# facebookresearch/momentum

Measured on NVIDIA H100. Metric: GN iterations/sec (batched 72-joint IK), higher is better.
Workload: dtype f32

## Files before the change

momentum_b200/csrc/ik_capi.cu:

```cuda
#include "../../include/momentum_b200.h"

#include <cuda_runtime.h>
#include <nvtx3/nvToolsExt.h>

#include <algorithm>
#include <cfloat>
#include <cmath>
#include <cstdio>
#include <cstdlib>
#include <cstring>
#include <memory>
#include <string>
#include <vector>

#include "ik_chol_sched.h"
#include "ik_fused.cuh"
#include "ik_jtj_tc.cuh"
#include "ik_kernels.cuh"
#include "ik_plan.h"

using namespace mb2;

namespace {

thread_local std::string g_lastError;

int fail(int code, const std::string& msg) {
  g_lastError = msg;
  return code;
}
#define MB2_CUDA(expr)                                                                                  \
  do {                                                                                                  \
    cudaError_t _e = (expr);                                                                            \
    if (_e != cudaSuccess) return fail(MB2_ERR_CUDA, std::string(#expr) + ": " + cudaGetErrorString(_e)); \
  } while (0)
#define MB2_CHECK(cond, msg)                                   \
  do {                                                         \
    if (!(cond)) return fail(MB2_ERR_INVALID_ARGUMENT, (msg)); \
  } while (0)

template <class T>
struct DeviceBuffer {
  T* p{nullptr};
  size_t n{0};
  ~DeviceBuffer() { release(); }
  void release() {
    if (p) cudaFree(p);
    p = nullptr;
    n = 0;
  }
  cudaError_t resize(size_t count) {
    if (count <= n && p) return cudaSuccess;
    release();
    if (count == 0) return cudaSuccess;
    cudaError_t e = cudaMalloc(&p, count * sizeof(T));
    if (e == cudaSuccess) n = count;
    return e;
  }
  cudaError_t upload(const std::vector<T>& v, cudaStream_t s) {
    cudaError_t e = resize(std::max<size_t>(v.size(), 1));
    if (e != cudaSuccess || v.empty()) return e;
    return cudaMemcpyAsync(p, v.data(), v.size() * sizeof(T), cudaMemcpyHostToDevice, s);
  }
};

int roundUp(int v, int m) { return (v + m - 1) / m * m; }

int usableDevices();

struct DeviceGuard {
  int prev{-1};
  bool switched{false};
  cudaError_t err{cudaSuccess};
  explicit DeviceGuard(int device) {
    err = cudaGetDevice(&prev);
    if (err == cudaSuccess && prev != device) { err = cudaSetDevice(device); switched = err == cudaSuccess; }
  }
  ~DeviceGuard() { if (switched) cudaSetDevice(prev); }
  DeviceGuard(const DeviceGuard&) = delete;
  DeviceGuard& operator=(const DeviceGuard&) = delete;
};
#define MB2_DEVICE_GUARD(device)                                                                                      \
  if (usableDevices() <= 0) return fail(MB2_ERR_CUDA, "no usable sm_90 CUDA device: momentum_b200 has no CPU fallback"); \
  DeviceGuard _guard(device);                                                                                         \
  MB2_CUDA(_guard.err)

struct NvtxRange {
  explicit NvtxRange(const char* name) { nvtxRangePushA(name); }
  ~NvtxRange() { nvtxRangePop(); }
};

}

struct mb2_character {
  int device{0};
  HostCharacter host;
  DeviceBuffer<int32_t> parent, ptOuter, ptInner, levelStart, levelJoints;
  DeviceBuffer<float> offset, prerot, ptVals, ptOffsets;
  uint64_t limitsVersion{0};
};

struct DeviceSchedule {
  CholSchedule host;
  CholSchedDev dev{};
  DeviceBuffer<int32_t> blob;
  GramPlan gram;
  DeviceBuffer<int32_t> gBlob;
  int32_t gBlobInts{0}, gOffsets[8]{};
  DeviceBuffer<int32_t> fBlob;
  FusedBlobLayout fLayout{};
  FusedConfig fConfig{};
};

struct mb2_solver_function {
  const mb2_character* ch{nullptr};
  int B{0};
  cudaStream_t stream{nullptr};
  HostFunction host;
  bool planDirty{true};
  int planMode{0};
  bool planSchedDense{false};
  bool planAlignRows{false};
  uint64_t planLimitsVersion{~0ull};
  Plan plan;
  int ldJ{32};
  DeviceBuffer<EfDesc> dEfs;
  DeviceBuffer<UnitDesc> dUnits;
  DeviceBuffer<CellDesc> dCells;
  DeviceBuffer<ContribDesc> dContribs;
  DeviceBuffer<float> dLimitData;
  DeviceBuffer<int32_t> dEnabledList, dIdentity, dDeviceCols;
  DeviceBuffer<float> dTargets, dWeights, dJ, dTheta, dState, dH, dTargetStage;
  DeviceBuffer<double> dErrors;
  std::unique_ptr<DeviceSchedule> sched;
  FunctionTables tables() const;
};

struct PhaseEvent {
  cudaEvent_t start, stop;
  int phase;
};

struct mb2_solver {
  mb2_solver_function* fn{nullptr};
  mb2_gauss_newton_options opt{};
  DeviceBuffer<float> dH, dDelta, dThetaOrig, dTheta0, dScale, dGradDotDelta, dThetaStage, dGrad, dTiles, dRadius, dRSaved;
  DeviceBuffer<double> dLastErrors, dTrialErrors, dHistory;
  DeviceBuffer<int32_t> dActive, dIterations, dStatus, dSearching, dActiveCount, dWorkCounter, dQrChunks;
  DeviceBuffer<unsigned long long> dPhaseCycles;
  bool lastFused{false}, lastGramChol{false};
  int lastFusedGroups{0};
  cudaEvent_t fusedStart{nullptr}, fusedStop{nullptr};
  double fusedMs{0};
  int* hActiveCount{nullptr};
  char* hResults{nullptr};
  size_t hResultsBytes{0};
  bool resultsStaged{false};
  uint64_t totalIterations{0}, kernelLaunches{0};
  bool profiling{false};
  bool inKernelProfile{false};
  std::vector<PhaseEvent> events;
  double phaseMs[4]{0, 0, 0, 0};
  uint64_t phaseLaunches[4]{0, 0, 0, 0};
  size_t historyStride{0};
  ~mb2_solver() {
    if (hActiveCount) cudaFreeHost(hActiveCount);
    if (hResults) cudaFreeHost(hResults);
    if (fusedStart) cudaEventDestroy(fusedStart);
    if (fusedStop) cudaEventDestroy(fusedStop);
    for (auto& e : events) { cudaEventDestroy(e.start); cudaEventDestroy(e.stop); }
  }
};

FunctionTables mb2_solver_function::tables() const {
  FunctionTables T{};
  const HostCharacter& h = ch->host;
  T.numJoints = h.numJoints;
  T.numParams = h.numParams;
  T.parent = ch->parent.p;
  T.offset = ch->offset.p;
  T.prerot = ch->prerot.p;
  T.ptOuter = ch->ptOuter.p;
  T.ptInner = ch->ptInner.p;
  T.ptVals = ch->ptVals.p;
  T.ptOffsets = ch->ptOffsets.p;
  T.numLevels = int(h.levelStart.size()) - 1;
  T.levelStart = ch->levelStart.p;
  T.levelJoints = ch->levelJoints.p;
  T.numEf = int(plan.efs.size());
  T.numUnits = int(plan.units.size());
  T.numCells = int(plan.cells.size());
  T.efs = dEfs.p;
  T.units = dUnits.p;
  T.cells = dCells.p;
  T.contribs = dContribs.p;
  T.limitData = dLimitData.p;
  T.targetStride = host.targetStride;
  T.recStride = plan.recStride;
  T.numRows = plan.numRows;
  T.ldJ = ldJ;
  T.numCols = plan.numCols;
  T.weightsPerInstance = host.weightsPerInstance ? 1 : 0;
  T.numWeights = host.numWeights;
  T.ptNnz = int(h.ptInner.size());
  T.numContribs = int(plan.contribs.size());
  T.numLimitData = int(plan.limitData.size());
  const bool strips = planMode == 2 && planAlignRows && sched;
  T.stripMode = strips ? 1 : 0;
  T.residOff = strips ? sched->gram.residOff : 0;
  T.jacobianStride = strips ? size_t(sched->gram.stride) : size_t(plan.numCols + 1) * ldJ;
  return T;
}

namespace {

bool g_deviceChecked = false;
int g_usableDevices = 0;
}
namespace {
int usableDevices() {
  if (!g_deviceChecked) {
    int n = 0;
    if (cudaGetDeviceCount(&n) != cudaSuccess) { n = 0; cudaGetLastError(); }
    int ok = 0;
    for (int d = 0; d < n; ++d) {
      int major = 0;
      if (cudaDeviceGetAttribute(&major, cudaDevAttrComputeCapabilityMajor, d) == cudaSuccess && major == 9) ++ok;
    }
    g_usableDevices = ok;
    g_deviceChecked = true;
  }
  return g_usableDevices;
}

int requireDevice(int device) {
  if (usableDevices() <= 0) return fail(MB2_ERR_CUDA, "no usable sm_90 CUDA device: momentum_b200 has no CPU fallback");
  MB2_CUDA(cudaSetDevice(device));
  MB2_CUDA(initKernelAttributes());
  return MB2_OK;
}

int ensureTargets(mb2_solver_function* f) {
  const size_t need = size_t(f->B) * std::max(f->host.targetStride, 1);
  if (f->dTargets.n < need) {
    DeviceBuffer<float> old;
    std::swap(old.p, f->dTargets.p);
    std::swap(old.n, f->dTargets.n);
    MB2_CUDA(f->dTargets.resize(need));
    MB2_CUDA(cudaMemsetAsync(f->dTargets.p, 0, need * sizeof(float), f->stream));
    MB2_CUDA(cudaStreamSynchronize(f->stream));
    (void)old;
  }
  return MB2_OK;
}

int uploadWeights(mb2_solver_function* f) {
  if (!f->host.weightsPerInstance) {
    std::vector<float> w = f->host.weights;
    if (w.empty()) w.push_back(0.f);
    MB2_CUDA(f->dWeights.upload(w, f->stream));
  }
  return MB2_OK;
}

int buildFusedBlob(mb2_solver_function* f, DeviceSchedule& ds, const std::vector<int32_t>& gramBlob, const std::vector<int32_t>& schedBlob, cudaStream_t s) {
  std::vector<int32_t> blob;
  auto add = [&](const void* data, size_t bytes) {
    const int32_t off = int32_t(blob.size());
    const size_t words = (bytes + 3) / 4;
    blob.resize(blob.size() + words, 0);
    if (bytes) std::memcpy(blob.data() + off, data, bytes);
    while (blob.size() % 4) blob.push_back(0);
    return off;
  };
  const HostCharacter& h = f->ch->host;
  const Plan& p = f->plan;
  FusedBlobLayout& L = ds.fLayout;
  L.parent = add(h.parent.data(), h.parent.size() * 4);
  L.offset = add(h.offset.data(), h.offset.size() * 4);
  L.prerot = add(h.prerot.data(), h.prerot.size() * 4);
  L.ptOuter = add(h.ptOuter.data(), h.ptOuter.size() * 4);
  L.ptInner = add(h.ptInner.data(), h.ptInner.size() * 4);
  L.ptVals = add(h.ptVals.data(), h.ptVals.size() * 4);
  L.ptOffsets = add(h.ptOffsets.data(), h.ptOffsets.size() * 4);
  L.levelStart = add(h.levelStart.data(), h.levelStart.size() * 4);
  L.levelJoints = add(h.levelJoints.data(), h.levelJoints.size() * 4);
  L.efs = add(p.efs.data(), p.efs.size() * sizeof(EfDesc));
  L.units = add(p.units.data(), p.units.size() * sizeof(UnitDesc));
  L.cells = add(p.cells.data(), p.cells.size() * sizeof(CellDesc));
  L.contribs = add(p.contribs.data(), p.contribs.size() * sizeof(ContribDesc));
  L.limitData = add(p.limitData.data(), p.limitData.size() * 4);
  L.cols = add(p.deviceCols.data(), p.deviceCols.size() * 4);
  L.gram = add(gramBlob.data(), gramBlob.size() * 4);
  L.sched = add(schedBlob.data(), schedBlob.size() * 4);
  if (blob.empty()) blob.push_back(0);
  while (blob.size() % 4) blob.push_back(0);
  L.words = int32_t(blob.size());
  MB2_CUDA(ds.fBlob.upload(blob, s));
  return MB2_OK;
}

int ensurePlan(mb2_solver_function* f, int mode, bool schedDense = false, bool alignRows = false) {
  bool allEnabled = true;
  for (uint8_t e : f->host.enabled) allEnabled = allEnabled && e;
  if (allEnabled && mode == 1) mode = 0;
  if (mode != 2) alignRows = false;
  if (!f->planDirty && f->planLimitsVersion == f->ch->limitsVersion && f->planMode == mode && (mode != 2 || (f->planSchedDense == schedDense && f->planAlignRows == alignRows)))
    return MB2_OK;
  MB2_DEVICE_GUARD(f->ch->device);
  cudaStream_t s = f->stream;
  f->sched.reset();
  std::unique_ptr<DeviceSchedule> ds;
  std::string err;
  if (mode == 2) {
    ds = std::make_unique<DeviceSchedule>();
    err = planSolverPath(f->ch->host, f->host.efs, f->host.enabled, schedDense, alignRows, f->plan, ds->host, ds->gram);
  } else {
    err = buildPlan(f->ch->host, f->host.efs, f->host.enabled, mode != 0, f->plan);
  }
  if (!err.empty()) return fail(MB2_ERR_INVALID_ARGUMENT, err);
  if (ds) {
    std::vector<int32_t> sblob, gblob;
    CholSchedDev hostView;
    makeScheduleBlob(ds->host, sblob, hostView);
    MB2_CUDA(ds->blob.upload(sblob, s));
    ds->dev = rebaseSchedule(hostView, ds->blob.p);
    if (alignRows) {
      makeGramBlob(ds->gram, ds->host, gblob, ds->gOffsets);
      ds->gBlobInts = int32_t(gblob.size());
      MB2_CUDA(ds->gBlob.upload(gblob, s));
      const int rc = buildFusedBlob(f, *ds, gblob, sblob, s);
      if (rc != MB2_OK) return rc;
    }
    f->sched = std::move(ds);
  }
  f->planMode = mode;
  f->planSchedDense = schedDense;
  f->planAlignRows = alignRows;
  MB2_CUDA(f->dEfs.upload(f->plan.efs, s));
  MB2_CUDA(f->dUnits.upload(f->plan.units, s));
  MB2_CUDA(f->dCells.upload(f->plan.cells, s));
  MB2_CUDA(f->dContribs.upload(f->plan.contribs, s));
  MB2_CUDA(f->dLimitData.upload(f->plan.limitData, s));
  MB2_CUDA(f->dEnabledList.upload(f->plan.enabledList, s));
  MB2_CUDA(f->dDeviceCols.upload(f->plan.deviceCols, s));
  std::vector<int32_t> ident(f->ch->host.numParams);
  for (size_t i = 0; i < ident.size(); ++i) ident[i] = int32_t(i);
  MB2_CUDA(f->dIdentity.upload(ident, s));
  f->ldJ = std::max(32, roundUp(f->plan.numRows, 32));
  const bool stripLayout = mode == 2 && alignRows;
  const size_t jElems = stripLayout ? size_t(f->B) * size_t(f->sched->gram.stride) : size_t(f->B) * (f->plan.numCols + 1) * f->ldJ;
  MB2_CUDA(f->dJ.resize(jElems));
  MB2_CUDA(cudaMemsetAsync(f->dJ.p, 0, jElems * sizeof(float), s));
  MB2_CUDA(f->dErrors.resize(f->B));
  MB2_CUDA(f->dTheta.resize(size_t(f->B) * f->ch->host.numParams));
  int rc = ensureTargets(f);
  if (rc != MB2_OK) return rc;
  rc = uploadWeights(f);
  if (rc != MB2_OK) return rc;
  if (stripLayout) {
    int dev = 0, optin = 0;
    MB2_CUDA(cudaGetDevice(&dev));
    MB2_CUDA(cudaDeviceGetAttribute(&optin, cudaDevAttrMaxSharedMemoryPerBlockOptin, dev));
    f->sched->fConfig = fusedConfigure(f->tables(), f->sched->fLayout, f->sched->dev, f->sched->gram.stride, int(f->sched->gram.tileOrder.size()) / kGramWarps, optin);
  }
  MB2_CUDA(cudaStreamSynchronize(s));
  f->planDirty = false;
  f->planLimitsVersion = f->ch->limitsVersion;
  return MB2_OK;
}

SweepArgs sweepArgs(mb2_solver_function* f, const float* theta, const int32_t* active) {
  SweepArgs a{};
  a.T = f->tables();
  a.batch = f->B;
  a.theta = theta;
  a.ldTheta = f->ch->host.numParams;
  a.targets = f->dTargets.p;
  a.cweights = f->dWeights.p;
  a.jacobian = f->dJ.p;
  a.errors = f->dErrors.p;
  a.active = active;
  a.stateOut = nullptr;
  return a;
}

int addBlock(mb2_solver_function* f, const std::string& buildError, const HostErrorFunction& ef, int32_t* outIndex) {
  if (!buildError.empty()) return fail(MB2_ERR_INVALID_ARGUMENT, buildError);
  const std::string err = f->host.add(ef, outIndex);
  if (!err.empty()) return fail(MB2_ERR_UNSUPPORTED, err);
  f->planDirty = true;
  return MB2_OK;
}

void bitsToEnabled(const uint64_t* bits, int n, std::vector<uint8_t>& out) {
  out.assign(n, 0);
  for (int i = 0; i < n; ++i) out[i] = (bits[i >> 6] >> (i & 63)) & 1ull ? 1 : 0;
}

void recordPhaseStart(mb2_solver* s, int phase, cudaStream_t st) {
  s->kernelLaunches++;
  if (!s->profiling) return;
  PhaseEvent e;
  cudaEventCreate(&e.start);
  cudaEventCreate(&e.stop);
  e.phase = phase;
  cudaEventRecord(e.start, st);
  s->events.push_back(e);
}
void recordPhaseStop(mb2_solver* s, cudaStream_t st) {
  if (!s->profiling) return;
  cudaEventRecord(s->events.back().stop, st);
}

__global__ void initSolveStateKernel(int batch, int32_t* active, int32_t* iterations, int32_t* status, double* lastErrors, double* errors) {
  const int b = blockIdx.x * blockDim.x + threadIdx.x;
  if (b >= batch) return;
  active[b] = 1;
  iterations[b] = 0;
  status[b] = 0;
  lastErrors[b] = DBL_MAX;
  errors[b] = DBL_MAX;
}
__global__ void initLineSearchKernel(int batch, const int32_t* active, int32_t* searching, float* scale) {
  const int b = blockIdx.x * blockDim.x + threadIdx.x;
  if (b >= batch) return;
  searching[b] = active[b];
  scale[b] = 1.f;
}
__global__ void finalizeKernel(int batch, int n, float* theta, const float* theta0, int32_t* status) {
  const int b = blockIdx.x;
  __shared__ int bad;
  if (threadIdx.x == 0) bad = 0;
  __syncthreads();
  for (int i = threadIdx.x; i < n; i += blockDim.x)
    if (!isfinite(theta[size_t(b) * n + i])) bad = 1;
  __syncthreads();
  if (bad) {
    for (int i = threadIdx.x; i < n; i += blockDim.x) theta[size_t(b) * n + i] = theta0[size_t(b) * n + i];
    if (threadIdx.x == 0) status[b] = MB2_INSTANCE_NON_FINITE;
  }
}

int resolveJtjMode(const mb2_solver_function* f, int requested, int ns) {
  if (requested == MB2_JTJ_FP32_SIMT) return MB2_JTJ_FP32_SIMT;
  const bool ok = jtjTensorSupported(ns, f->plan.numCols, f->ldJ);
  if (requested == MB2_JTJ_AUTO) return ok ? MB2_JTJ_TF32X3 : MB2_JTJ_FP32_SIMT;
  return ok ? requested : -1;
}

int runJtJ(mb2_solver_function* f, int mode, int ns, float* H, int ldH, size_t hStride, const int32_t* active, cudaStream_t st, float* g = nullptr, int ldG = 0) {
  JtJArgs a{};
  a.batch = f->B;
  a.jacobian = f->dJ.p;
  a.numCols = f->plan.numCols;
  a.ldJ = f->ldJ;
  a.kRows = roundUp(std::max(f->plan.numRows, 1), 4);
  a.ns = ns;
  a.H = H;
  a.ldH = ldH;
  a.hStride = hStride;
  a.active = active;
  a.g = g;
  a.ldG = ldG;
  if (mode == MB2_JTJ_FP32_SIMT) { MB2_CUDA(launchJtJSimt(a, st)); }
  else { MB2_CUDA(launchJtJTensor(a, mode == MB2_JTJ_TF32X3 ? 3 : 1, st)); }
  return MB2_OK;
}

}

extern "C" {

const char* mb2_last_error(void) { return g_lastError.c_str(); }
int mb2_device_count(void) { return usableDevices(); }

void mb2_default_gauss_newton_options(mb2_gauss_newton_options* o) {
  if (!o) return;
  std::memset(o, 0, sizeof(*o));
  o->min_iterations = 1;
  o->max_iterations = 2;
  o->threshold = 1.0f;
  o->verbose = 0;
  o->regularization = 0.05f;
  o->do_line_search = 0;
  o->use_block_jtj = 0;
  o->target_rows_per_chunk = ~0ull;
  o->subset_line_search = 0;
  o->jtj_mode = MB2_JTJ_AUTO;
  o->store_error_history = 0;
  o->cholesky_mode = MB2_CHOLESKY_AUTO;
  o->fused_mode = MB2_FUSED_AUTO;
  o->linear_solver = MB2_LINEAR_SOLVER_CHOLESKY;
  o->trust_region_radius = 1.0f;
}

int mb2_character_create(int device, int32_t J, const int32_t* parents, const float* offsets, const float* prerot, int32_t n,
                         const int32_t* outer, const int32_t* inner, const float* vals, const float* ptoffsets, mb2_character** out) {
  MB2_CHECK(out != nullptr, "null argument");
  auto c = std::make_unique<mb2_character>();
  HostCharacter& h = c->host;
  const std::string err = makeCharacter(J, parents, offsets, prerot, n, outer, inner, vals, ptoffsets, h);
  if (!err.empty()) return fail(MB2_ERR_INVALID_ARGUMENT, err);
  MB2_DEVICE_GUARD(device);
  int rc = requireDevice(device);
  if (rc != MB2_OK) return rc;
  c->device = device;
  MB2_CUDA(c->parent.upload(h.parent, nullptr));
  MB2_CUDA(c->offset.upload(h.offset, nullptr));
  MB2_CUDA(c->prerot.upload(h.prerot, nullptr));
  MB2_CUDA(c->ptOuter.upload(h.ptOuter, nullptr));
  MB2_CUDA(c->ptInner.upload(h.ptInner, nullptr));
  MB2_CUDA(c->ptVals.upload(h.ptVals, nullptr));
  MB2_CUDA(c->ptOffsets.upload(h.ptOffsets, nullptr));
  MB2_CUDA(c->levelStart.upload(h.levelStart, nullptr));
  MB2_CUDA(c->levelJoints.upload(h.levelJoints, nullptr));
  MB2_CUDA(cudaStreamSynchronize(nullptr));
  *out = c.release();
  return MB2_OK;
}

int mb2_character_set_parameter_limits(mb2_character* c, int32_t count, const mb2_parameter_limit* limits) {
  MB2_CHECK(c != nullptr, "invalid limits");
  const std::string err = setParameterLimits(c->host, count, limits);
  if (!err.empty()) return fail(MB2_ERR_INVALID_ARGUMENT, err);
  c->limitsVersion++;
  return MB2_OK;
}

void mb2_character_destroy(mb2_character* c) { delete c; }

int mb2_solver_function_create(const mb2_character* c, int32_t batch, mb2_solver_function** out) {
  MB2_CHECK(c != nullptr && out != nullptr, "null argument");
  MB2_CHECK(batch > 0, "batch must be positive");
  MB2_DEVICE_GUARD(c->device);
  int rc = requireDevice(c->device);
  if (rc != MB2_OK) return rc;
  auto f = std::make_unique<mb2_solver_function>();
  f->ch = c;
  f->B = batch;
  f->host.enabled.assign(c->host.numParams, 1);
  MB2_CUDA(cudaStreamCreateWithFlags(&f->stream, cudaStreamNonBlocking));
  *out = f.release();
  return MB2_OK;
}

void mb2_solver_function_destroy(mb2_solver_function* f) {
  if (!f) return;
  if (f->stream) cudaStreamDestroy(f->stream);
  delete f;
}

int mb2_character_clone(const mb2_character* c, int device, mb2_character** out) {
  MB2_CHECK(c != nullptr && out != nullptr, "null argument");
  const HostCharacter& h = c->host;
  mb2_character* copy = nullptr;
  int rc = mb2_character_create(device, h.numJoints, h.parent.data(), h.offset.data(), h.prerot.data(), h.numParams, h.ptOuter.data(), h.ptInner.data(), h.ptVals.data(),
                                h.ptOffsets.data(), &copy);
  if (rc != MB2_OK) return rc;
  copy->host.limits = h.limits;
  copy->limitsVersion = 1;
  *out = copy;
  return MB2_OK;
}
int mb2_solver_function_clone(const mb2_solver_function* f, const mb2_character* c, int32_t batch, mb2_solver_function** out) {
  MB2_CHECK(f != nullptr && c != nullptr && out != nullptr, "null argument");
  MB2_CHECK(c->host.numJoints == f->ch->host.numJoints && c->host.numParams == f->ch->host.numParams, "clone target character has a different shape");
  MB2_CHECK(!f->host.weightsPerInstance, "a function with per-instance constraint weights cannot be cloned (set them on the clone)");
  mb2_solver_function* g = nullptr;
  int rc = mb2_solver_function_create(c, batch, &g);
  if (rc != MB2_OK) return rc;
  g->host = f->host;
  g->planDirty = true;
  *out = g;
  return MB2_OK;
}
int mb2_character_device(const mb2_character* c) { return c ? c->device : -1; }
const mb2_character* mb2_solver_function_character(const mb2_solver_function* f) { return f ? f->ch : nullptr; }
int32_t mb2_solver_function_num_error_functions(const mb2_solver_function* f) { return f ? int32_t(f->host.efs.size()) : 0; }
int32_t mb2_solver_function_target_size(const mb2_solver_function* f, int32_t index) {
  return (f && index >= 0 && index < int32_t(f->host.efs.size())) ? f->host.efs[index].targetSize : -1;
}

int32_t mb2_solver_function_num_parameters(const mb2_solver_function* f) { return f ? f->ch->host.numParams : 0; }
int32_t mb2_solver_function_batch(const mb2_solver_function* f) { return f ? f->B : 0; }
int32_t mb2_solver_function_actual_parameters(const mb2_solver_function* f) { return f ? f->host.actualParameters() : 0; }
int32_t mb2_solver_function_jacobian_rows(const mb2_solver_function* f) { return f ? f->host.jacobianRows(f->ch->host) : 0; }
int32_t mb2_solver_function_jacobian_stride(const mb2_solver_function* f) { return f ? f->host.jacobianStride(f->ch->host) : 0; }

int mb2_add_position_error_function(mb2_solver_function* f, float weight, float alpha, float c, int32_t nc, const int32_t* parents,
                                    const float* offsets, const float* weights, int32_t* outIndex) {
  MB2_CHECK(f != nullptr, "null solver function");
  HostErrorFunction ef;
  return addBlock(f, positionErrorFunction(f->ch->host, weight, alpha, c, nc, parents, offsets, weights, ef), ef, outIndex);
}

int mb2_add_position_error_function_instanced(mb2_solver_function* f, float weight, float alpha, float c, int32_t nc, const int32_t* parents, const float* weights,
                                              int32_t* outIndex) {
  MB2_CHECK(f != nullptr, "null solver function");
  HostErrorFunction ef;
  return addBlock(f, instancedPositionErrorFunction(f->ch->host, weight, alpha, c, nc, parents, weights, ef), ef, outIndex);
}

int mb2_add_plane_error_function(mb2_solver_function* f, float weight, float alpha, float c, int32_t above, int32_t nc, const int32_t* parents,
                                 const float* offsets, const float* weights, int32_t* outIndex) {
  MB2_CHECK(f != nullptr, "null solver function");
  HostErrorFunction ef;
  return addBlock(f, planeErrorFunction(f->ch->host, weight, alpha, c, above, nc, parents, offsets, weights, ef), ef, outIndex);
}

int mb2_add_model_parameters_error_function(mb2_solver_function* f, float weight, const float* targetWeights, int32_t* outIndex) {
  MB2_CHECK(f != nullptr, "null solver function");
  HostErrorFunction ef;
  return addBlock(f, modelParametersErrorFunction(f->ch->host, weight, targetWeights, ef), ef, outIndex);
}

int mb2_add_orientation_error_function(mb2_solver_function* f, float weight, float alpha, float c, int32_t rotDiff, int32_t nc,
                                       const int32_t* parents, const float* offsets, const float* weights, int32_t* outIndex) {
  MB2_CHECK(f != nullptr, "null solver function");
  HostErrorFunction ef;
  return addBlock(f, orientationErrorFunction(f->ch->host, weight, alpha, c, rotDiff, nc, parents, offsets, weights, ef), ef, outIndex);
}

int mb2_add_state_error_function(mb2_solver_function* f, float weight, int32_t rotationErrorType, float posWgt, float rotWgt,
                                 const float* posW, const float* rotW, int32_t* outIndex) {
  MB2_CHECK(f != nullptr, "null solver function");
  HostErrorFunction ef;
  return addBlock(f, stateErrorFunction(f->ch->host, weight, rotationErrorType, posWgt, rotWgt, posW, rotW, ef), ef, outIndex);
}

int mb2_add_limit_error_function(mb2_solver_function* f, float weight, float alpha, float c, int32_t* outIndex) {
  MB2_CHECK(f != nullptr, "null solver function");
  HostErrorFunction ef;
  return addBlock(f, limitErrorFunction(weight, alpha, c, ef), ef, outIndex);
}

int mb2_set_error_function_weight(mb2_solver_function* f, int32_t index, float weight) {
  MB2_CHECK(f != nullptr && index >= 0 && index < int(f->host.efs.size()), "error function index out of range");
  f->host.efs[index].weight = weight;
  f->planDirty = true;
  return MB2_OK;
}

static int setTargetsImpl(mb2_solver_function* f, int32_t index, const float* targets, bool deviceSrc, cudaStream_t st) {
  MB2_CHECK(f != nullptr && index >= 0 && index < int(f->host.efs.size()) && targets, "invalid targets");
  const HostErrorFunction& ef = f->host.efs[index];
  if (ef.targetSize == 0 && ef.kind != 4) return MB2_OK;
  MB2_CHECK(ef.targetSize > 0, "this error function has no per-instance targets");
  MB2_DEVICE_GUARD(f->ch->device);
  int rc = ensureTargets(f);
  if (rc != MB2_OK) return rc;
  float* dst = f->dTargets.p + ef.targetOff;
  const float* packed = targets;
  if (!deviceSrc) {
    MB2_CUDA(f->dTargetStage.resize(size_t(f->B) * ef.targetSize));
    MB2_CUDA(cudaMemcpyAsync(f->dTargetStage.p, targets, size_t(f->B) * ef.targetSize * sizeof(float), cudaMemcpyHostToDevice, st));
    packed = f->dTargetStage.p;
  }
  MB2_CUDA(launchScatterTargets(packed, dst, ef.targetSize, f->host.targetStride, f->B, st));
  if (ef.kind == 1 || ef.kind == 2) MB2_CUDA(launchNormalizeQuats(dst, 0, f->host.targetStride, ef.numConstraints(), f->B, st));
  return MB2_OK;
}
int mb2_set_targets(mb2_solver_function* f, int32_t index, const float* targets) {
  if (!f) return fail(MB2_ERR_INVALID_ARGUMENT, "null solver function");
  int rc = setTargetsImpl(f, index, targets, false, f->stream);
  if (rc != MB2_OK) return rc;
  MB2_CUDA(cudaStreamSynchronize(f->stream));
  return MB2_OK;
}
int mb2_set_targets_device(mb2_solver_function* f, int32_t index, const float* targets, void* stream) {
  if (!f) return fail(MB2_ERR_INVALID_ARGUMENT, "null solver function");
  return setTargetsImpl(f, index, targets, true, stream ? (cudaStream_t)stream : f->stream);
}

int mb2_set_constraint_weights(mb2_solver_function* f, int32_t index, const float* weights, int32_t perInstance) {
  MB2_CHECK(f != nullptr && index >= 0 && index < int(f->host.efs.size()) && weights, "invalid constraint weights");
  HostErrorFunction& ef = f->host.efs[index];
  MB2_CHECK(ef.kind <= 2 || ef.kind == 5, "constraint weights apply to Position/Orientation/Plane error functions");
  MB2_DEVICE_GUARD(f->ch->device);
  const int nc = ef.numConstraints();
  if (!perInstance) {
    MB2_CHECK(!f->host.weightsPerInstance, "solver function already uses per-instance constraint weights");
    ef.weights.assign(weights, weights + nc);
    std::copy(weights, weights + nc, f->host.weights.begin() + ef.weightOff);
    return uploadWeights(f);
  }
  if (!f->host.weightsPerInstance) {
    std::vector<float> all(size_t(f->B) * f->host.numWeights);
    for (int b = 0; b < f->B; ++b) std::copy(f->host.weights.begin(), f->host.weights.end(), all.begin() + size_t(b) * f->host.numWeights);
    f->dWeights.release();
    MB2_CUDA(f->dWeights.upload(all, f->stream));
    f->host.weightsPerInstance = true;
  }
  MB2_CUDA(cudaMemcpy2DAsync(f->dWeights.p + ef.weightOff, size_t(f->host.numWeights) * sizeof(float), weights, size_t(nc) * sizeof(float),
                             size_t(nc) * sizeof(float), f->B, cudaMemcpyHostToDevice, f->stream));
  MB2_CUDA(cudaStreamSynchronize(f->stream));
  return MB2_OK;
}

int mb2_set_constraint_weights_device(mb2_solver_function* f, int32_t index, const float* weights_device, void* stream) {
  MB2_CHECK(f != nullptr && index >= 0 && index < int(f->host.efs.size()) && weights_device, "invalid constraint weights");
  HostErrorFunction& ef = f->host.efs[index];
  MB2_CHECK(ef.kind <= 2 || ef.kind == 5, "constraint weights apply to Position/Orientation/Plane error functions");
  MB2_DEVICE_GUARD(f->ch->device);
  const int nc = ef.numConstraints();
  if (!f->host.weightsPerInstance) {
    std::vector<float> all(size_t(f->B) * f->host.numWeights);
    for (int b = 0; b < f->B; ++b) std::copy(f->host.weights.begin(), f->host.weights.end(), all.begin() + size_t(b) * f->host.numWeights);
    f->dWeights.release();
    MB2_CUDA(f->dWeights.upload(all, f->stream));
    MB2_CUDA(cudaStreamSynchronize(f->stream));
    f->host.weightsPerInstance = true;
    f->planDirty = true;
  }
  cudaStream_t st = stream ? (cudaStream_t)stream : f->stream;
  if (nc > 0)
    MB2_CUDA(cudaMemcpy2DAsync(f->dWeights.p + ef.weightOff, size_t(f->host.numWeights) * sizeof(float), weights_device, size_t(nc) * sizeof(float), size_t(nc) * sizeof(float), f->B,
                               cudaMemcpyDeviceToDevice, st));
  return MB2_OK;
}

int mb2_solver_function_set_enabled_parameters(mb2_solver_function* f, const uint64_t* bits) {
  MB2_CHECK(f != nullptr && bits != nullptr, "null argument");
  bitsToEnabled(bits, f->ch->host.numParams, f->host.enabled);
  f->planDirty = true;
  return MB2_OK;
}

int mb2_solver_function_get_error(mb2_solver_function* f, const float* params, double* errors) {
  MB2_CHECK(f != nullptr && params && errors, "null argument");
  MB2_DEVICE_GUARD(f->ch->device);
  int rc = ensurePlan(f, f->planMode, f->planSchedDense, f->planAlignRows);
  if (rc != MB2_OK) return rc;
  const size_t n = f->ch->host.numParams;
  MB2_CUDA(cudaMemcpyAsync(f->dTheta.p, params, size_t(f->B) * n * sizeof(float), cudaMemcpyHostToDevice, f->stream));
  MB2_CUDA(launchSweep(sweepArgs(f, f->dTheta.p, nullptr), false, f->stream));
  MB2_CUDA(cudaMemcpyAsync(errors, f->dErrors.p, size_t(f->B) * sizeof(double), cudaMemcpyDeviceToHost, f->stream));
  MB2_CUDA(cudaStreamSynchronize(f->stream));
  return MB2_OK;
}

int mb2_solver_function_get_jacobian(mb2_solver_function* f, const float* params, float* jac, float* residual, double* errors, int32_t* actualRows) {
  MB2_CHECK(f != nullptr && params, "null argument");
  MB2_DEVICE_GUARD(f->ch->device);
  int rc = ensurePlan(f, 0);
  if (rc != MB2_OK) return rc;
  const size_t n = f->ch->host.numParams;
  const int rows = mb2_solver_function_jacobian_rows(f);
  MB2_CUDA(cudaMemcpyAsync(f->dTheta.p, params, size_t(f->B) * n * sizeof(float), cudaMemcpyHostToDevice, f->stream));
  MB2_CUDA(launchSweep(sweepArgs(f, f->dTheta.p, nullptr), true, f->stream));
  for (int b = 0; b < f->B && rows > 0; ++b) {
    const float* Jb = f->dJ.p + size_t(b) * (n + 1) * f->ldJ;
    if (jac)
      MB2_CUDA(cudaMemcpy2DAsync(jac + size_t(b) * n * rows, size_t(rows) * sizeof(float), Jb, size_t(f->ldJ) * sizeof(float), size_t(rows) * sizeof(float), n,
                                 cudaMemcpyDeviceToHost, f->stream));
    if (residual)
      MB2_CUDA(cudaMemcpyAsync(residual + size_t(b) * rows, Jb + n * f->ldJ, size_t(rows) * sizeof(float), cudaMemcpyDeviceToHost, f->stream));
  }
  if (errors) MB2_CUDA(cudaMemcpyAsync(errors, f->dErrors.p, size_t(f->B) * sizeof(double), cudaMemcpyDeviceToHost, f->stream));
  MB2_CUDA(cudaStreamSynchronize(f->stream));
  if (actualRows) *actualRows = rows;
  return MB2_OK;
}

int mb2_solver_function_get_jacobian_device(mb2_solver_function* f, const float* params_device, const float** jacobian_device, int32_t* ld, void* stream) {
  MB2_CHECK(f != nullptr && params_device && jacobian_device, "null argument");
  MB2_DEVICE_GUARD(f->ch->device);
  int rc = ensurePlan(f, 0);
  if (rc != MB2_OK) return rc;
  cudaStream_t st = stream ? (cudaStream_t)stream : f->stream;
  MB2_CUDA(launchSweep(sweepArgs(f, params_device, nullptr), true, st));
  *jacobian_device = f->dJ.p;
  if (ld) *ld = f->ldJ;
  return MB2_OK;
}

int mb2_solver_function_get_jtjr(mb2_solver_function* f, const float* params, int32_t jtjMode, float* jtj, float* jtr, double* errors) {
  MB2_CHECK(f != nullptr && params, "null argument");
  MB2_DEVICE_GUARD(f->ch->device);
  int rc = ensurePlan(f, 0);
  if (rc != MB2_OK) return rc;
  const size_t n = f->ch->host.numParams;
  const int ap = f->plan.actualParameters;
  MB2_CHECK(ap > 0, "no enabled parameters");
  const int mode = resolveJtjMode(f, jtjMode, ap);
  if (mode < 0) return fail(MB2_ERR_UNSUPPORTED, "tensor-core JtJ does not support this shape");
  const int ldH = roundUp(ap + 1, 16);
  const size_t hElems = size_t(f->B) * (ap + 1) * ldH;
  MB2_CUDA(f->dH.resize(hElems));
  MB2_CUDA(cudaMemcpyAsync(f->dTheta.p, params, size_t(f->B) * n * sizeof(float), cudaMemcpyHostToDevice, f->stream));
  MB2_CUDA(launchSweep(sweepArgs(f, f->dTheta.p, nullptr), true, f->stream));
  MB2_CUDA(cudaMemsetAsync(f->dH.p, 0, hElems * sizeof(float), f->stream));
  rc = runJtJ(f, mode, ap, f->dH.p, ldH, size_t(ap + 1) * ldH, nullptr, f->stream);
  if (rc != MB2_OK) return rc;
  std::vector<float> h(hElems);
  MB2_CUDA(cudaMemcpyAsync(h.data(), f->dH.p, hElems * sizeof(float), cudaMemcpyDeviceToHost, f->stream));
  if (errors) MB2_CUDA(cudaMemcpyAsync(errors, f->dErrors.p, size_t(f->B) * sizeof(double), cudaMemcpyDeviceToHost, f->stream));
  MB2_CUDA(cudaStreamSynchronize(f->stream));
  for (int b = 0; b < f->B; ++b) {
    const float* Hb = h.data() + size_t(b) * (ap + 1) * ldH;
    for (int j = 0; j < ap; ++j) {
      if (jtj) for (int i = j; i < ap; ++i) jtj[(size_t(b) * ap + i) * ap + j] = Hb[size_t(j) * ldH + i];
      if (jtr) jtr[size_t(b) * ap + j] = Hb[size_t(j) * ldH + ap];
    }
  }
  return MB2_OK;
}

int mb2_solver_function_get_skeleton_state(mb2_solver_function* f, const float* params, float* state) {
  MB2_CHECK(f != nullptr && params && state, "null argument");
  MB2_DEVICE_GUARD(f->ch->device);
  int rc = ensurePlan(f, f->planMode, f->planSchedDense, f->planAlignRows);
  if (rc != MB2_OK) return rc;
  const size_t n = f->ch->host.numParams;
  const size_t sz = size_t(f->B) * f->ch->host.numJoints * 8;
  MB2_CUDA(f->dState.resize(sz));
  MB2_CUDA(cudaMemcpyAsync(f->dTheta.p, params, size_t(f->B) * n * sizeof(float), cudaMemcpyHostToDevice, f->stream));
  SweepArgs a = sweepArgs(f, f->dTheta.p, nullptr);
  a.stateOut = f->dState.p;
  MB2_CUDA(launchSweep(a, false, f->stream));
  MB2_CUDA(cudaMemcpyAsync(state, f->dState.p, sz * sizeof(float), cudaMemcpyDeviceToHost, f->stream));
  MB2_CUDA(cudaStreamSynchronize(f->stream));
  return MB2_OK;
}

int mb2_solver_create(mb2_solver_function* f, const mb2_gauss_newton_options* opt, mb2_solver** out) {
  MB2_CHECK(f != nullptr && out != nullptr, "null argument");
  auto s = std::make_unique<mb2_solver>();
  s->fn = f;
  if (opt) s->opt = *opt; else mb2_default_gauss_newton_options(&s->opt);
  MB2_DEVICE_GUARD(f->ch->device);
  MB2_CUDA(cudaMallocHost(&s->hActiveCount, sizeof(int)));
  *out = s.release();
  return MB2_OK;
}
void mb2_solver_destroy(mb2_solver* s) { delete s; }
int mb2_solver_set_options(mb2_solver* s, const mb2_gauss_newton_options* opt) {
  MB2_CHECK(s != nullptr && opt != nullptr, "null argument");
  s->opt = *opt;
  return MB2_OK;
}
int mb2_solver_set_enabled_parameters(mb2_solver* s, const uint64_t* bits) {
  MB2_CHECK(s != nullptr, "null solver");
  return mb2_solver_function_set_enabled_parameters(s->fn, bits);
}
int mb2_solver_set_profiling(mb2_solver* s, int32_t enabled) {
  MB2_CHECK(s != nullptr, "null solver");
  s->profiling = enabled != 0;
  s->inKernelProfile = enabled >= 2;
  return MB2_OK;
}

int mb2_solver_solve_device(mb2_solver* s, float* theta, void* cudaStream) {
  MB2_CHECK(s != nullptr && theta != nullptr, "null argument");
  mb2_solver_function* f = s->fn;
  MB2_DEVICE_GUARD(f->ch->device);
  NvtxRange nvtxSolve("mb2::SolverT::solve");
  const mb2_gauss_newton_options& o = s->opt;
  int cholMode = resolveCholeskyMode(o.cholesky_mode, f->host.enabled);
  const bool useTr = o.linear_solver == MB2_LINEAR_SOLVER_TRUST_REGION_QR;
  const bool useQr = o.linear_solver == MB2_LINEAR_SOLVER_QR || useTr;
  if (useTr && !(o.trust_region_radius > 0.f)) return fail(MB2_ERR_INVALID_ARGUMENT, "trust_region_radius must be positive");
  if (useQr) {
    if (o.jtj_mode == MB2_JTJ_SPARSE_TILES || o.cholesky_mode >= 2 || o.fused_mode >= MB2_FUSED_PERSISTENT)
      return fail(MB2_ERR_UNSUPPORTED, "the QR step works on the dense Jacobian: it excludes the tile-sparse Gram, the tile Cholesky and the fused kernels");
    cholMode = 1;
  }
  bool useGram = cholMode >= 2 && (o.jtj_mode == MB2_JTJ_AUTO || o.jtj_mode == MB2_JTJ_SPARSE_TILES);
  if (o.jtj_mode == MB2_JTJ_SPARSE_TILES && cholMode < 2) return fail(MB2_ERR_UNSUPPORTED, "MB2_JTJ_SPARSE_TILES needs the tile-scheduled Cholesky");
  int rc = ensurePlan(f, cholMode >= 2 ? 2 : 1, cholMode == 2, useGram);
  if (rc != MB2_OK) return rc;
  bool useSchedule = cholMode >= 2;
  if (useSchedule && choleskyScheduledSmemBytes(f->plan.numCols, f->sched->host.nPad, f->sched->host.numTiles, f->sched->dev.blobInts) > size_t(200 * 1024)) {
    if (o.cholesky_mode >= 2) return fail(MB2_ERR_UNSUPPORTED, "tile schedule does not fit in shared memory for this system");
    useSchedule = false;
    useGram = false;
    rc = ensurePlan(f, 1);
    if (rc != MB2_OK) return rc;
  }
  cudaStream_t st = cudaStream ? (cudaStream_t)cudaStream : f->stream;
  const int B = f->B, n = f->ch->host.numParams;
  const int ns = f->plan.numCols;
  const int maxIt = int(std::min<uint64_t>(o.max_iterations, 1u << 30));
  const int minIt = int(std::min<uint64_t>(o.min_iterations, 1u << 30));
  MB2_CHECK(ns > 0, "no enabled parameters");
  if (useGram && gramTilesSmemBytes(size_t(f->sched->gram.stride), f->sched->gBlobInts) > size_t(200 * 1024)) {
    if (o.jtj_mode == MB2_JTJ_SPARSE_TILES) return fail(MB2_ERR_UNSUPPORTED, "Jacobian strips do not fit in shared memory for this system");
    useGram = false;
    rc = ensurePlan(f, 2, cholMode == 2, false);
    if (rc != MB2_OK) return rc;
  }
  s->lastFused = false;
  {
    const bool eligible = useGram && useSchedule && o.do_line_search == 0 && f->sched->fConfig.groups >= 1 && f->sched->fBlob.p != nullptr;
    if (o.fused_mode == MB2_FUSED_PERSISTENT && !eligible)
      return fail(MB2_ERR_UNSUPPORTED, "the fused kernel needs the tile-sparse Gram + tile-scheduled Cholesky path, no line search, and a plan that fits in shared memory");
    int smCount = 0;
    if (eligible && o.fused_mode == MB2_FUSED_AUTO) {
      int dev0 = 0;
      MB2_CUDA(cudaGetDevice(&dev0));
      MB2_CUDA(cudaDeviceGetAttribute(&smCount, cudaDevAttrMultiProcessorCount, dev0));
    }
    const bool oneWave = eligible && o.fused_mode == MB2_FUSED_AUTO && B <= f->sched->fConfig.groups * smCount;
    if ((o.fused_mode == MB2_FUSED_PERSISTENT || oneWave) && eligible) {
      const DeviceSchedule& ds = *f->sched;
      MB2_CUDA(s->dIterations.resize(B));
      MB2_CUDA(s->dStatus.resize(B));
      MB2_CUDA(s->dWorkCounter.resize(1));
      MB2_CUDA(cudaMemsetAsync(s->dWorkCounter.p, 0, sizeof(int32_t), st));
      if (o.store_error_history) {
        MB2_CUDA(s->dHistory.resize(size_t(B) * std::max(maxIt, 1)));
        MB2_CUDA(cudaMemsetAsync(s->dHistory.p, 0, size_t(B) * std::max(maxIt, 1) * sizeof(double), st));
        s->historyStride = size_t(std::max(maxIt, 1));
      }
      FusedArgs fa{};
      fa.batch = B;
      fa.T = f->tables();
      fa.blob = ds.fBlob.p;
      fa.L = ds.fLayout;
      fa.S = ds.dev;
      fa.schedGlobal = ds.dev.blob;
      for (int k = 0; k < 8; ++k) fa.gramOff[k] = ds.gOffsets[k];
      fa.numStrips = ds.gram.numStrips;
      fa.stripStride = ds.gram.stride;
      fa.residOff = ds.gram.residOff;
      fa.numOrder = int32_t(ds.gram.tileOrder.size());
      fa.regularization = o.regularization;
      fa.threshold = o.threshold;
      fa.minIterations = minIt;
      fa.maxIterations = maxIt;
      fa.theta = theta;
      fa.ldTheta = n;
      fa.targets = f->dTargets.p;
      fa.cweights = f->dWeights.p;
      fa.errors = f->dErrors.p;
      fa.iterations = s->dIterations.p;
      fa.status = s->dStatus.p;
      fa.history = o.store_error_history ? s->dHistory.p : nullptr;
      fa.workCounter = s->dWorkCounter.p;
      fa.phaseCycles = nullptr;
      if (s->profiling) {
        MB2_CUDA(s->dPhaseCycles.resize(16));
        MB2_CUDA(cudaMemsetAsync(s->dPhaseCycles.p, 0, 16 * sizeof(unsigned long long), st));
        fa.phaseCycles = s->inKernelProfile ? s->dPhaseCycles.p : nullptr;
        if (!s->fusedStart) { MB2_CUDA(cudaEventCreate(&s->fusedStart)); MB2_CUDA(cudaEventCreate(&s->fusedStop)); }
        MB2_CUDA(cudaEventRecord(s->fusedStart, st));
      }
      int dev = 0, sms = 0;
      MB2_CUDA(cudaGetDevice(&dev));
      MB2_CUDA(cudaDeviceGetAttribute(&sms, cudaDevAttrMultiProcessorCount, dev));
      {
        NvtxRange nvtxIt("mb2::fusedSolveKernel (GaussNewtonSolverT::doIteration x maxIterations)");
        MB2_CUDA(launchFusedSolve(fa, ds.fConfig, sms, s->inKernelProfile, st));
      }
      if (s->profiling) MB2_CUDA(cudaEventRecord(s->fusedStop, st));
      for (auto& e : s->events) { cudaEventDestroy(e.start); cudaEventDestroy(e.stop); }
      s->events.clear();
      s->kernelLaunches = 1;
      s->lastFused = true;
      s->lastFusedGroups = ds.fConfig.groups;
      return MB2_OK;
    }
  }
  bool useGramChol = false;
  if (useGram && useSchedule) {
    const DeviceSchedule& ds = *f->sched;
    const int rounds = std::max(int(ds.gram.tileOrder.size()) / kGramWarps, 1);
    const bool fits = gramCholeskySmemBytes(size_t(ds.gram.stride), ds.gBlobInts, ns, ds.host.nPad, ds.host.numTiles, ds.dev.blobInts) <= size_t(200 * 1024) && rounds <= kGramCholMaxRounds;
    if (o.fused_mode == MB2_FUSED_GRAM_CHOLESKY && !fits) return fail(MB2_ERR_UNSUPPORTED, "Gram + Cholesky fusion: strips / tiles of this plan do not fit in shared memory, or too many tiles per warp");
    useGramChol = fits && (o.fused_mode == MB2_FUSED_AUTO || o.fused_mode == MB2_FUSED_GRAM_CHOLESKY);
  } else if (o.fused_mode == MB2_FUSED_GRAM_CHOLESKY) {
    return fail(MB2_ERR_UNSUPPORTED, "Gram + Cholesky fusion needs the tile-sparse Gram + tile-scheduled Cholesky path");
  }
  s->lastGramChol = useGramChol;
  if (useGramChol && s->profiling) {
    MB2_CUDA(s->dPhaseCycles.resize(16));
    MB2_CUDA(cudaMemsetAsync(s->dPhaseCycles.p, 0, 16 * sizeof(unsigned long long), st));
  }
  const int mode = useGram ? MB2_JTJ_SPARSE_TILES : resolveJtjMode(f, o.jtj_mode == MB2_JTJ_SPARSE_TILES ? MB2_JTJ_AUTO : o.jtj_mode, ns);
  if (mode < 0) return fail(MB2_ERR_UNSUPPORTED, "tensor-core JtJ does not support this shape");
  const int ldH = roundUp(ns + 1, 16);
  const size_t hStride = size_t(ns + 1) * ldH;
  if (!useGram && !useQr) MB2_CUDA(s->dH.resize(size_t(B) * hStride));
  int qrMaxRows = 0, qrChunks = 0;
  if (useQr) {
    qrMaxRows = qrMaxChunkRows(ns, size_t(200 * 1024));
    if (qrMaxRows < 8) return fail(MB2_ERR_UNSUPPORTED, "the QR step keeps R in shared memory: too many enabled parameters for this kernel");
    if (useTr) {
      qrMaxRows = std::min(qrMaxRows, std::max(8, ns / 2));
      if (trQrSmemFloats(ns, n, f->ch->host.numJoints, qrMaxRows) * sizeof(float) > size_t(220 * 1024))
        return fail(MB2_ERR_UNSUPPORTED, "the trust-region QR kernel keeps R and the damping rows in shared memory: too many enabled parameters / joints");
    }
    std::vector<int32_t> starts{0};
    int r0 = 0, widest = 0;
    for (const auto& ef : f->host.efs) {
      if (!(ef.weight > 0.f)) continue;
      const int size = jacobianBlockSize(f->ch->host, ef);
      for (int done = 0; done < size; done += qrMaxRows) { const int p = std::min(qrMaxRows, size - done); starts.push_back(r0 + done + p); widest = std::max(widest, p); }
      r0 += size;
    }
    qrChunks = int(starts.size()) - 1;
    qrMaxRows = std::max(widest, 1);
    MB2_CUDA(s->dQrChunks.upload(starts, st));
    if (useTr) {
      MB2_CUDA(s->dRadius.upload(std::vector<float>(size_t(B), o.trust_region_radius), st));
      MB2_CUDA(s->dRSaved.resize(size_t(B) * ((size_t(ns) * (ns + 1) / 2 + 3) & ~size_t(3))));
    }
  }
  float* Hbuf = s->dH.p;
  const size_t tilesStride = useGram ? size_t(f->sched->host.numTiles) * 256 + f->sched->host.nPad : 0;
  if (useGram && !(o.fused_mode == MB2_FUSED_AUTO || o.fused_mode == MB2_FUSED_GRAM_CHOLESKY)) MB2_CUDA(s->dTiles.resize(size_t(B) * tilesStride));
  const int ldG = cholGradientLd(ns);
  MB2_CUDA(s->dGrad.resize(size_t(B) * ldG));
  MB2_CUDA(s->dDelta.resize(size_t(B) * ns));
  MB2_CUDA(s->dTheta0.resize(size_t(B) * n));
  MB2_CUDA(s->dLastErrors.resize(B));
  MB2_CUDA(s->dActive.resize(B));
  MB2_CUDA(s->dIterations.resize(B));
  MB2_CUDA(s->dStatus.resize(B));
  MB2_CUDA(s->dActiveCount.resize(1));
  const bool lineSearch = o.do_line_search != 0 && !useTr;
  if (lineSearch) {
    MB2_CUDA(s->dThetaOrig.resize(size_t(B) * n));
    MB2_CUDA(s->dTrialErrors.resize(B));
    MB2_CUDA(s->dScale.resize(B));
    MB2_CUDA(s->dSearching.resize(B));
    MB2_CUDA(s->dGradDotDelta.resize(B));
  }
  if (o.store_error_history) {
    MB2_CUDA(s->dHistory.resize(size_t(B) * std::max(maxIt, 1)));
    MB2_CUDA(cudaMemsetAsync(s->dHistory.p, 0, size_t(B) * std::max(maxIt, 1) * sizeof(double), st));
    s->historyStride = size_t(std::max(maxIt, 1));
  }
  for (auto& e : s->events) { cudaEventDestroy(e.start); cudaEventDestroy(e.stop); }
  s->events.clear();
  s->kernelLaunches = 0;

  initSolveStateKernel<<<(B + 127) / 128, 128, 0, st>>>(B, s->dActive.p, s->dIterations.p, s->dStatus.p, s->dLastErrors.p, f->dErrors.p);
  MB2_CUDA(cudaGetLastError());
  MB2_CUDA(cudaMemcpyAsync(s->dTheta0.p, theta, size_t(B) * n * sizeof(float), cudaMemcpyDeviceToDevice, st));

  static const bool cholProfile = getenv("MB2_CHOL_PROFILE") != nullptr;
  constexpr int kPollEvery = 4;
  for (int it = 0; it < maxIt; ++it) {
    MB2_CUDA(cudaMemsetAsync(s->dActiveCount.p, 0, sizeof(int), st));
    recordPhaseStart(s, 0, st);
    MB2_CUDA(launchSweep(sweepArgs(f, theta, s->dActive.p), true, st));
    recordPhaseStop(s, st);
    GramArgs g{};
    if (!useGramChol && !useQr) recordPhaseStart(s, 1, st);
    if (useQr) {
    } else if (useGram) {
      const DeviceSchedule& ds = *f->sched;
      g.batch = B;
      g.strips = f->dJ.p;
      g.stripStride = size_t(ds.gram.stride);
      g.residOff = ds.gram.residOff;
      g.active = s->dActive.p;
      g.numStrips = ds.gram.numStrips;
      g.numTiles = ds.host.numTiles;
      g.numTileCols = ds.host.numTileCols;
      g.nPad = ds.host.nPad;
      g.numOrder = int32_t(ds.gram.tileOrder.size());
      g.blob = ds.gBlob.p;
      g.blobInts = ds.gBlobInts;
      g.offTileOrder = ds.gOffsets[0]; g.offTilePairStart = ds.gOffsets[1]; g.offPairA = ds.gOffsets[2]; g.offPairB = ds.gOffsets[3];
      g.offColStripStart = ds.gOffsets[4]; g.offColStrip = ds.gOffsets[5]; g.offStripRow = ds.gOffsets[6]; g.offTileInfo = ds.gOffsets[7];
      g.regularization = o.regularization;
      g.out = s->dTiles.p;
      g.outStride = tilesStride;
      if (!useGramChol) {
        if (s->dTiles.n < size_t(B) * tilesStride) MB2_CUDA(s->dTiles.resize(size_t(B) * tilesStride));
        g.out = s->dTiles.p;
        MB2_CUDA(launchGramTiles(g, st));
      }
    } else {
      rc = runJtJ(f, mode, ns, Hbuf, ldH, hStride, s->dActive.p, st, s->dGrad.p, ldG);
      if (rc != MB2_OK) return rc;
    }
    if (!useGramChol && !useQr) recordPhaseStop(s, st);
    CholArgs c{};
    c.batch = B;
    c.H = Hbuf;
    c.ns = ns;
    c.ldH = ldH;
    c.hStride = hStride;
    c.regularization = o.regularization;
    c.cols = f->dDeviceCols.p;
    c.theta = theta;
    c.ldTheta = n;
    c.delta = s->dDelta.p;
    c.applyUpdate = lineSearch ? 0 : 1;
    c.errors = f->dErrors.p;
    c.lastErrors = s->dLastErrors.p;
    c.active = s->dActive.p;
    c.iterations = s->dIterations.p;
    c.status = s->dStatus.p;
    c.history = o.store_error_history ? s->dHistory.p : nullptr;
    c.iteration = it;
    c.minIterations = minIt;
    c.maxIterations = maxIt;
    c.threshold = o.threshold;
    c.activeCount = s->dActiveCount.p;
    c.bookkeeping = lineSearch ? 0 : 1;
    c.gradDotDelta = lineSearch ? s->dGradDotDelta.p : nullptr;
    c.g = s->dGrad.p;
    c.ldG = ldG;
    c.tilesIn = useGram ? s->dTiles.p : nullptr;
    c.tilesStride = tilesStride;
    c.profile = (it == 0 && cholProfile) ? 1 : 0;
    recordPhaseStart(s, 2, st);
    if (useQr) {
      QrArgs q{};
      q.c = c;
      q.jacobian = f->dJ.p;
      q.numCols = f->plan.numCols;
      q.ldJ = f->ldJ;
      q.chunkStart = s->dQrChunks.p;
      q.numChunks = qrChunks;
      if (useTr) {
        TrQrArgs t{};
        t.q = q;
        t.T = f->tables();
        t.targets = f->dTargets.p;
        t.cweights = f->dWeights.p;
        t.radius = s->dRadius.p;
        t.rSaved = s->dRSaved.p;
        t.maxRadius = 10.f;
        t.maxChunkRows = qrMaxRows;
        MB2_CUDA(launchTrustRegionQr(t, st));
      } else {
        MB2_CUDA(launchQrSolve(q, qrMaxRows, st));
      }
    } else if (useGramChol) {
      GramCholArgs gc{};
      gc.g = g;
      gc.c = c;
      gc.c.tilesIn = nullptr;
      gc.phaseCycles = s->inKernelProfile ? s->dPhaseCycles.p : nullptr;
      MB2_CUDA(launchGramCholesky(gc, f->sched->dev, s->inKernelProfile, st));
    } else if (useSchedule) MB2_CUDA(launchCholeskyScheduled(c, f->sched->dev, st));
    else MB2_CUDA(launchCholesky(c, st));
    recordPhaseStop(s, st);
    if (lineSearch) {
      MB2_CUDA(cudaMemcpyAsync(s->dThetaOrig.p, theta, size_t(B) * n * sizeof(float), cudaMemcpyDeviceToDevice, st));
      initLineSearchKernel<<<(B + 127) / 128, 128, 0, st>>>(B, s->dActive.p, s->dSearching.p, s->dScale.p);
      MB2_CUDA(cudaGetLastError());
      for (int step = 0; step < 10; ++step) {
        MB2_CUDA(launchTrialUpdate(B, s->dThetaOrig.p, n, s->dDelta.p, ns, f->dDeviceCols.p, s->dScale.p, theta, s->dSearching.p, st));
        SweepArgs ea = sweepArgs(f, theta, s->dSearching.p);
        ea.errors = s->dTrialErrors.p;
        recordPhaseStart(s, 3, st);
        MB2_CUDA(launchSweep(ea, false, st));
        recordPhaseStop(s, st);
        LineSearchArgs la{};
        la.batch = B; la.ns = ns; la.numParams = n; la.ldTheta = n;
        la.errors = f->dErrors.p;
        la.trialErrors = s->dTrialErrors.p;
        la.gradDotDelta = s->dGradDotDelta.p;
        la.scale = s->dScale.p;
        la.searching = s->dSearching.p;
        la.step = step;
        la.subsetVariant = o.subset_line_search;
        la.active = s->dActive.p;
        MB2_CUDA(launchLineSearchStep(la, st));
        s->kernelLaunches += 2;
      }
      BookkeepingArgs ba{};
      ba.batch = B;
      ba.errors = f->dErrors.p; ba.lastErrors = s->dLastErrors.p; ba.active = s->dActive.p; ba.iterations = s->dIterations.p;
      ba.status = s->dStatus.p; ba.history = o.store_error_history ? s->dHistory.p : nullptr;
      ba.theta = theta; ba.ldTheta = n; ba.numParams = n;
      ba.iteration = it; ba.minIterations = minIt; ba.maxIterations = maxIt; ba.threshold = o.threshold; ba.activeCount = s->dActiveCount.p;
      MB2_CUDA(launchBookkeeping(ba, st));
      s->kernelLaunches += 1;
    }
    if (it + 1 < maxIt && it >= minIt && (it - minIt) % kPollEvery == kPollEvery - 1) {
      MB2_CUDA(cudaMemcpyAsync(s->hActiveCount, s->dActiveCount.p, sizeof(int), cudaMemcpyDeviceToHost, st));
      MB2_CUDA(cudaStreamSynchronize(st));
      if (*s->hActiveCount == 0) break;
    }
  }
  finalizeKernel<<<B, 128, 0, st>>>(B, n, theta, s->dTheta0.p, s->dStatus.p);
  MB2_CUDA(cudaGetLastError());
  s->kernelLaunches += 2;
  return MB2_OK;
}

static void collectProfile(mb2_solver* s) {
  if (s->profiling && s->lastFused && s->fusedStart) {
    float ms = 0.f;
    s->fusedMs = cudaEventElapsedTime(&ms, s->fusedStart, s->fusedStop) == cudaSuccess ? double(ms) : 0.0;
  }
  if (s->profiling) {
    for (int k = 0; k < 4; ++k) { s->phaseMs[k] = 0; s->phaseLaunches[k] = 0; }
    for (auto& e : s->events) {
      float ms = 0.f;
      if (cudaEventElapsedTime(&ms, e.start, e.stop) == cudaSuccess) { s->phaseMs[e.phase] += ms; s->phaseLaunches[e.phase]++; }
    }
  }
}

int mb2_solver_get_results(mb2_solver* s, double* errors, int32_t* iterations, int32_t* status) {
  MB2_CHECK(s != nullptr, "null solver");
  mb2_solver_function* f = s->fn;
  const int B = f->B;
  MB2_DEVICE_GUARD(f->ch->device);
  MB2_CUDA(cudaDeviceSynchronize());
  if (errors) MB2_CUDA(cudaMemcpy(errors, f->dErrors.p, size_t(B) * sizeof(double), cudaMemcpyDeviceToHost));
  std::vector<int32_t> its(B);
  MB2_CUDA(cudaMemcpy(its.data(), s->dIterations.p, size_t(B) * sizeof(int32_t), cudaMemcpyDeviceToHost));
  s->totalIterations = 0;
  for (int v : its) s->totalIterations += uint64_t(v);
  if (iterations) std::copy(its.begin(), its.end(), iterations);
  if (status) MB2_CUDA(cudaMemcpy(status, s->dStatus.p, size_t(B) * sizeof(int32_t), cudaMemcpyDeviceToHost));
  collectProfile(s);
  return MB2_OK;
}

int mb2_solver_solve_async(mb2_solver* s, float* params) {
  MB2_CHECK(s != nullptr && params != nullptr, "null argument");
  mb2_solver_function* f = s->fn;
  MB2_DEVICE_GUARD(f->ch->device);
  const size_t B = size_t(f->B);
  const size_t bytes = B * f->ch->host.numParams * sizeof(float);
  MB2_CUDA(s->dThetaStage.resize(B * f->ch->host.numParams));
  MB2_CUDA(cudaMemcpyAsync(s->dThetaStage.p, params, bytes, cudaMemcpyHostToDevice, f->stream));
  s->resultsStaged = false;
  int rc = mb2_solver_solve_device(s, s->dThetaStage.p, f->stream);
  if (rc != MB2_OK) return rc;
  MB2_CUDA(cudaMemcpyAsync(params, s->dThetaStage.p, bytes, cudaMemcpyDeviceToHost, f->stream));
  const size_t need = B * (sizeof(double) + 2 * sizeof(int32_t));
  if (s->hResultsBytes < need) {
    if (s->hResults) cudaFreeHost(s->hResults);
    s->hResults = nullptr;
    s->hResultsBytes = 0;
    MB2_CUDA(cudaMallocHost(reinterpret_cast<void**>(&s->hResults), need));
    s->hResultsBytes = need;
  }
  MB2_CUDA(cudaMemcpyAsync(s->hResults, f->dErrors.p, B * sizeof(double), cudaMemcpyDeviceToHost, f->stream));
  MB2_CUDA(cudaMemcpyAsync(s->hResults + B * sizeof(double), s->dIterations.p, B * sizeof(int32_t), cudaMemcpyDeviceToHost, f->stream));
  MB2_CUDA(cudaMemcpyAsync(s->hResults + B * (sizeof(double) + sizeof(int32_t)), s->dStatus.p, B * sizeof(int32_t), cudaMemcpyDeviceToHost, f->stream));
  s->resultsStaged = true;
  return MB2_OK;
}

int mb2_solver_wait(mb2_solver* s, double* errors, int32_t* iterations, int32_t* status) {
  MB2_CHECK(s != nullptr, "null solver");
  MB2_DEVICE_GUARD(s->fn->ch->device);
  MB2_CUDA(cudaStreamSynchronize(s->fn->stream));
  if (!s->resultsStaged) return mb2_solver_get_results(s, errors, iterations, status);
  const size_t B = size_t(s->fn->B);
  const int32_t* its = reinterpret_cast<const int32_t*>(s->hResults + B * sizeof(double));
  if (errors) std::memcpy(errors, s->hResults, B * sizeof(double));
  s->totalIterations = 0;
  for (size_t b = 0; b < B; ++b) s->totalIterations += uint64_t(its[b]);
  if (iterations) std::memcpy(iterations, its, B * sizeof(int32_t));
  if (status) std::memcpy(status, s->hResults + B * (sizeof(double) + sizeof(int32_t)), B * sizeof(int32_t));
  s->resultsStaged = false;
  collectProfile(s);
  return MB2_OK;
}

int mb2_solver_solve(mb2_solver* s, float* params, double* errors, int32_t* iterations, int32_t* status) {
  const int rc = mb2_solver_solve_async(s, params);
  if (rc != MB2_OK) return rc;
  return mb2_solver_wait(s, errors, iterations, status);
}

int mb2_solver_get_error_history(mb2_solver* s, double* history) {
  MB2_CHECK(s != nullptr && history != nullptr, "null argument");
  MB2_CHECK(s->opt.store_error_history && s->dHistory.p, "error history was not stored (set store_error_history)");
  MB2_CUDA(cudaMemcpy(history, s->dHistory.p, size_t(s->fn->B) * s->historyStride * sizeof(double), cudaMemcpyDeviceToHost));
  return MB2_OK;
}

int mb2_solver_get_counters(mb2_solver* s, uint64_t* totalIterations, uint64_t* kernelLaunches) {
  MB2_CHECK(s != nullptr, "null solver");
  if (totalIterations) *totalIterations = s->totalIterations;
  if (kernelLaunches) *kernelLaunches = s->kernelLaunches;
  return MB2_OK;
}

int mb2_solver_get_plan_stats(mb2_solver* s, int64_t stats[12]) {
  MB2_CHECK(s != nullptr && stats != nullptr, "null argument");
  const mb2_solver_function* f = s->fn;
  int64_t nnz = 0;
  for (const CellDesc& c : f->plan.cells) nnz += f->plan.units[c.unit].numRows;
  const bool tiles = f->planMode == 2 && f->sched;
  stats[0] = nnz;
  stats[1] = f->plan.numCols;
  stats[2] = f->ldJ;
  stats[3] = f->planMode == 0 ? int64_t(f->plan.enabledList.size()) : int64_t(f->plan.numCols);
  stats[4] = tiles ? f->sched->host.numTiles : 0;
  stats[5] = tiles ? f->sched->host.tileOps : 0;
  stats[6] = tiles ? f->sched->host.numLevels : 0;
  stats[7] = f->plan.numRows;
  const bool gram = tiles && f->planAlignRows;
  stats[8] = gram ? f->sched->gram.stride : 0;
  stats[9] = gram ? f->sched->gram.macs : 0;
  stats[10] = gram ? int64_t(f->sched->gram.pairA.size()) : 0;
  stats[11] = gram ? f->sched->fConfig.groups : 0;
  return MB2_OK;
}

int mb2_solver_get_fused_profile(mb2_solver* s, int32_t* fused, int32_t* groups, double* kernelMs, uint64_t phaseCycles[12]) {
  MB2_CHECK(s != nullptr, "null solver");
  if (fused) *fused = s->lastFused ? 1 : (s->lastGramChol ? 2 : 0);
  if (groups) *groups = s->lastFused ? s->lastFusedGroups : 0;
  if (kernelMs) *kernelMs = s->lastFused ? s->fusedMs : (s->lastGramChol ? s->phaseMs[2] : 0.0);
  if (phaseCycles) {
    for (int k = 0; k < 12; ++k) phaseCycles[k] = 0;
    if ((s->lastFused || s->lastGramChol) && s->profiling && s->dPhaseCycles.p) {
      MB2_DEVICE_GUARD(s->fn->ch->device);
      unsigned long long h[12];
      MB2_CUDA(cudaMemcpy(h, s->dPhaseCycles.p, sizeof(h), cudaMemcpyDeviceToHost));
      if (s->lastFused) {
        for (int k = 0; k < 12; ++k) phaseCycles[k] = h[k];
      } else {
        phaseCycles[0] = h[0];
        for (int k = 1; k < 8; ++k) phaseCycles[4 + k] = h[k];
      }
    }
  }
  return MB2_OK;
}

int mb2_solver_get_phase_times(mb2_solver* s, double ms[4], uint64_t launches[4]) {
  MB2_CHECK(s != nullptr, "null solver");
  for (int k = 0; k < 4; ++k) {
    if (ms) ms[k] = s->phaseMs[k];
    if (launches) launches[k] = s->phaseLaunches[k];
  }
  return MB2_OK;
}

}
```

momentum_b200/csrc/ik_chol_sched.cpp:

```cpp
#include "ik_chol_sched.h"

#include "ik_chol_sched.cuh"

#include <algorithm>
#include <cstdio>
#include <cstdlib>
#include <map>
#include <set>
#include <tuple>

namespace mb2 {

namespace {

struct BitRows {
  int n, words;
  std::vector<uint64_t> b;
  BitRows(int n_) : n(n_), words((n_ + 63) / 64), b(size_t(n_) * ((n_ + 63) / 64), 0) {}
  uint64_t* row(int i) { return b.data() + size_t(i) * words; }
  const uint64_t* row(int i) const { return b.data() + size_t(i) * words; }
  void set(int i, int j) { row(i)[j >> 6] |= 1ull << (j & 63); }
  void clear(int i, int j) { row(i)[j >> 6] &= ~(1ull << (j & 63)); }
  bool test(int i, int j) const { return (row(i)[j >> 6] >> (j & 63)) & 1ull; }
  int count(int i) const {
    int c = 0;
    for (int w = 0; w < words; ++w) c += __builtin_popcountll(row(i)[w]);
    return c;
  }
};

std::vector<int> minimumDegreeOrder(BitRows& adj, const std::vector<int>* priority) {
  const int n = adj.n;
  std::vector<int> order;
  order.reserve(n);
  std::vector<uint8_t> done(n, 0);
  std::vector<int> degree(n);
  for (int i = 0; i < n; ++i) degree[i] = adj.count(i);
  int last = -1;
  for (int step = 0; step < n; ++step) {
    int best = -1;
    for (int i = 0; i < n; ++i) {
      if (done[i]) continue;
      if (best < 0 || degree[i] < degree[best]) { best = i; continue; }
      if (degree[i] != degree[best]) continue;
      const int pi = priority ? (*priority)[i] : 0, pb = priority ? (*priority)[best] : 0;
      if (pi > pb) best = i;
      else if (pi == pb && last >= 0 && adj.test(last, i) && !adj.test(last, best)) best = i;
    }
    std::vector<int> nb;
    for (int j = 0; j < n; ++j)
      if (!done[j] && j != best && adj.test(best, j)) nb.push_back(j);
    for (int u : nb) {
      uint64_t* ru = adj.row(u);
      const uint64_t* rv = adj.row(best);
      for (int w = 0; w < adj.words; ++w) ru[w] |= rv[w];
      adj.clear(u, u);
      adj.clear(u, best);
    }
    for (int u : nb) {
      int c = 0;
      for (int j : nb) c += (j != u) ? 1 : 0;
      (void)c;
      int d = 0;
      const uint64_t* ru = adj.row(u);
      for (int j = 0; j < n; ++j)
        if (!done[j] && j != best && ((ru[j >> 6] >> (j & 63)) & 1ull)) ++d;
      degree[u] = d;
    }
    done[best] = 1;
    order.push_back(best);
    last = best;
  }
  return order;
}

}

std::string buildCholSchedule(int n, const std::vector<std::vector<int>>& cliques, bool forceDense, CholSchedule& out, const std::vector<int>* priority) {
  out = CholSchedule();
  if (n <= 0) return "empty system";
  out.n = n;
  out.nParams = n;

  std::vector<int> order(n);
  BitRows pattern(n);
  for (int i = 0; i < n; ++i) pattern.set(i, i);
  if (forceDense) {
    for (int i = 0; i < n; ++i) order[i] = i;
  } else {
    for (const auto& c : cliques)
      for (int a : c) {
        if (a < 0 || a >= n) continue;
        for (int b : c)
          if (b >= 0 && b < n) pattern.set(a, b);
      }
    BitRows work = pattern;
    for (int i = 0; i < n; ++i) work.clear(i, i);
    if (priority != nullptr && int(priority->size()) != n) return "priority must have one entry per column";
    order = minimumDegreeOrder(work, priority);
  }
  std::vector<int> slot(n);
  {
    std::vector<int> rank(n);
    for (int i = 0; i < n; ++i) rank[order[i]] = i;
    BitRows F(n);
    for (int a = 0; a < n; ++a)
      for (int b = 0; b < n; ++b)
        if (a != b && (forceDense || pattern.test(a, b))) { const int i = rank[a], j = rank[b]; if (i > j) F.set(i, j); }
    std::vector<int> parent(n, -1), cnt(n, 0);
    std::vector<std::vector<int>> col(n);
    for (int j = 0; j < n; ++j) {
      for (int i = j + 1; i < n; ++i) if (F.test(i, j)) col[j].push_back(i);
      cnt[j] = int(col[j].size());
      if (!col[j].empty()) {
        const int pj = col[j][0];
        parent[j] = pj;
        for (size_t k = 1; k < col[j].size(); ++k) F.set(col[j][k], pj);
      }
    }
    int fill = 0, start = 0;
    int padded = 0;
    auto closeTile = [&]() { if (fill != 0) { padded += kCholTile - fill; fill = 0; } };
    auto flushSupernode = [&](int first, int lastExcl) {
      const int sz = lastExcl - first;
      if (sz <= kCholTile) {
        if (fill + sz > kCholTile) closeTile();
      } else {
        closeTile();
        const int head = sz % kCholTile;
        for (int j = first; j < first + head; ++j) { slot[j] = padded++; fill = (fill + 1) % kCholTile; }
        closeTile();
        first += head;
      }
      for (int j = first; j < lastExcl; ++j) { slot[j] = padded++; fill = (fill + 1) % kCholTile; }
    };
    for (int j = 1; j <= n; ++j) {
      const bool joins = j < n && parent[j - 1] == j && cnt[j - 1] == cnt[j] + 1;
      if (!joins) { flushSupernode(start, j); start = j; }
    }
    (void)fill;
    const int T0 = (padded + kCholTile - 1) / kCholTile;
    out.numTileCols = T0;
    out.nPad = T0 * kCholTile;
  }
  const int T = out.numTileCols;
  if (T > 512) return "system too large for the tile schedule";
  out.perm.assign(out.nPad, int16_t(-1));
  std::vector<int> pos(n);
  for (int i = 0; i < n; ++i) { out.perm[slot[i]] = int16_t(order[i]); pos[order[i]] = slot[i]; }

  std::vector<std::vector<uint8_t>> S(T, std::vector<uint8_t>(T, 0));
  for (int I = 0; I < T; ++I) S[I][I] = 1;
  if (forceDense) {
    for (int I = 0; I < T; ++I) for (int J = 0; J <= I; ++J) S[I][J] = 1;
  } else {
    for (int a = 0; a < n; ++a)
      for (int b = 0; b < n; ++b)
        if (pattern.test(a, b)) {
          const int I = pos[a] / kCholTile, J = pos[b] / kCholTile;
          if (I >= J) S[I][J] = 1;
        }
    for (int K = 0; K < T; ++K) {
      std::vector<int> st;
      for (int I = K + 1; I < T; ++I) if (S[I][K]) st.push_back(I);
      for (size_t a = 0; a < st.size(); ++a)
        for (size_t b = 0; b <= a; ++b) S[st[a]][st[b]] = 1;
    }
  }
  std::vector<std::vector<int>> tileId(T, std::vector<int>(T, -1));
  out.diagTile.assign(T, -1);
  for (int J = 0; J < T; ++J)
    for (int I = J; I < T; ++I)
      if (S[I][J]) {
        tileId[I][J] = int(out.tileRow.size());
        out.tileRow.push_back(int16_t(I));
        out.tileCol.push_back(int16_t(J));
        if (I == J) out.diagTile[J] = tileId[I][J];
      }
  out.numTiles = int(out.tileRow.size());
  out.tileIdTable.assign(size_t(T) * T, int16_t(-1));
  for (int I = 0; I < T; ++I) for (int J = 0; J <= I; ++J) out.tileIdTable[size_t(I) * T + J] = int16_t(tileId[I][J]);
  out.pos.resize(n);
  for (int i = 0; i < n; ++i) out.pos[i] = int16_t(pos[i]);
  std::vector<int> level(T, 0);
  std::vector<std::vector<int>> st(T);
  for (int K = 0; K < T; ++K) {
    for (int I = K + 1; I < T; ++I) if (S[I][K]) st[K].push_back(I);
    if (!st[K].empty()) level[st[K][0]] = std::max(level[st[K][0]], level[K] + 1);
  }
  int numLevels = 0;
  for (int K = 0; K < T; ++K) numLevels = std::max(numLevels, level[K] + 1);
  out.numLevels = numLevels;

  out.levelColStart.assign(1, 0);
  out.levelPanelStart.assign(1, 0);
  out.levelTaskStart.assign(1, 0);
  out.levelVTaskStart.assign(1, 0);
  out.taskPairStart.assign(1, 0);
  out.vtaskSrcStart.assign(1, 0);
  for (int L = 0; L < numLevels; ++L) {
    std::map<int, std::vector<std::pair<int, int>>> tasks;
    std::map<int, std::vector<std::pair<int, int>>> vtasks;
    for (int K = 0; K < T; ++K) {
      if (level[K] != L) continue;
      out.levelCols.push_back(K);
      for (int I : st[K]) {
        out.panelTile.push_back(tileId[I][K]);
        out.panelDiag.push_back(out.diagTile[K]);
        out.panelRow.push_back(I);
        vtasks[I].push_back({tileId[I][K], K});
      }
      for (size_t a = 0; a < st[K].size(); ++a)
        for (size_t b = 0; b <= a; ++b) {
          const int I = st[K][a], J = st[K][b];
          tasks[tileId[I][J]].push_back({tileId[I][K], tileId[J][K]});
          out.tileOps++;
        }
    }
    for (auto& kv : tasks) {
      out.taskDst.push_back(kv.first);
      for (auto& pr : kv.second) { out.pairA.push_back(pr.first); out.pairB.push_back(pr.second); }
      out.taskPairStart.push_back(int(out.pairA.size()));
    }
    for (auto& kv : vtasks) {
      out.vtaskRow.push_back(kv.first);
      for (auto& pr : kv.second) { out.vsrcTile.push_back(pr.first); out.vsrcCol.push_back(pr.second); }
      out.vtaskSrcStart.push_back(int(out.vsrcTile.size()));
    }
    out.levelColStart.push_back(int(out.levelCols.size()));
    out.levelPanelStart.push_back(int(out.panelTile.size()));
    out.levelTaskStart.push_back(int(out.taskDst.size()));
    out.levelVTaskStart.push_back(int(out.vtaskRow.size()));
  }
  for (int W : {8, 16}) {
    std::vector<int32_t>& start = W == 8 ? out.levelOrderStart8 : out.levelOrderStart16;
    std::vector<int32_t>& order = W == 8 ? out.taskOrder8 : out.taskOrder16;
    start.assign(1, 0);
    for (int L = 0; L < numLevels; ++L) {
      std::vector<int> ids;
      for (int t = out.levelTaskStart[L]; t < out.levelTaskStart[L + 1]; ++t) ids.push_back(t);
      std::stable_sort(ids.begin(), ids.end(), [&](int a, int b) { return out.taskPairStart[a + 1] - out.taskPairStart[a] > out.taskPairStart[b + 1] - out.taskPairStart[b]; });
      std::vector<std::vector<int>> ofWarp(W);
      std::vector<int64_t> load(W, 0);
      for (int t : ids) {
        int w = 0;
        for (int k = 1; k < W; ++k) if (load[k] < load[w]) w = k;
        ofWarp[w].push_back(t);
        load[w] += 2 * (out.taskPairStart[t + 1] - out.taskPairStart[t]) + 1;
      }
      size_t rounds = 0;
      for (const auto& v : ofWarp) rounds = std::max(rounds, v.size());
      const size_t base = order.size();
      order.resize(base + rounds * W, -1);
      for (int w = 0; w < W; ++w)
        for (size_t r = 0; r < ofWarp[w].size(); ++r) order[base + r * W + w] = ofWarp[w][r];
      start.push_back(int32_t(order.size()));
    }
  }
  out.colPanelStart.assign(1, 0);
  for (int K = 0; K < T; ++K) {
    for (int I : st[K]) { out.colPanelTile.push_back(tileId[I][K]); out.colPanelRow.push_back(I); }
    out.colPanelStart.push_back(int(out.colPanelTile.size()));
  }
  for (int K = 0; K < T; ++K) { const int64_t r = T - 1 - K; out.denseTileOps += r * (r + 1) / 2; }
  out.order = order;
  if (getenv("MB2_SCHED_DUMP") != nullptr) {
    fprintf(stderr, "chol schedule: n %d nPad %d tile columns %d tiles %d levels %d tile ops %lld (dense %lld)\n", n, out.nPad, T, out.numTiles, numLevels, (long long)out.tileOps, (long long)out.denseTileOps);
    for (int L = 0; L < numLevels; ++L) {
      int maxPairs = 0, pairs = 0;
      for (int t = out.levelTaskStart[L]; t < out.levelTaskStart[L + 1]; ++t) { const int p = out.taskPairStart[t + 1] - out.taskPairStart[t]; pairs += p; maxPairs = std::max(maxPairs, p); }
      fprintf(stderr, "  level %d: %d diagonal tiles, %d panel tiles, %d update tasks (%d pairs, longest %d), %d vector tasks; columns:", L, out.levelColStart[L + 1] - out.levelColStart[L],
              out.levelPanelStart[L + 1] - out.levelPanelStart[L], out.levelTaskStart[L + 1] - out.levelTaskStart[L], pairs, maxPairs, out.levelVTaskStart[L + 1] - out.levelVTaskStart[L]);
      for (int ci = out.levelColStart[L]; ci < out.levelColStart[L + 1]; ++ci) fprintf(stderr, " %d(%d)", out.levelCols[ci], int(st[out.levelCols[ci]].size()));
      fprintf(stderr, "\n");
    }
  }
  return "";
}

std::string buildGramPlan(const CholSchedule& s, const std::vector<int32_t>& cellRow0, const std::vector<int32_t>& cellRows, const std::vector<int32_t>& cellCol,
                          int numRows, GramPlan& out) {
  out = GramPlan();
  out.numTiles = s.numTiles;
  out.numTileCols = s.numTileCols;
  const int T = s.numTileCols;
  std::map<std::pair<int, int>, int> stripId;
  for (size_t i = 0; i < cellCol.size(); ++i) {
    const int d = cellCol[i];
    if (d < 0 || d >= s.n || s.pos[d] < 0) return "Jacobian cell in a column outside the schedule";
    const int K = s.pos[d] >> 4;
    for (int q = cellRow0[i] >> 2; q <= (cellRow0[i] + cellRows[i] - 1) >> 2; ++q) stripId[{q, K}] = 0;
  }
  int next = 0;
  for (auto& kv : stripId) kv.second = next++;
  out.numStrips = next;
  out.stripCoord.resize(size_t(next) * 2);
  std::vector<std::vector<int>> ofCol(T);
  for (const auto& kv : stripId) {
    const int q = kv.first.first, K = kv.first.second;
    out.stripCoord[2 * kv.second] = 4 * q;
    out.stripCoord[2 * kv.second + 1] = s.perm[16 * K];
    ofCol[K].push_back(kv.second);
  }
  std::map<int, std::set<int>> colsOfUnit;
  std::map<int, int> rowsOfUnit;
  for (size_t i = 0; i < cellCol.size(); ++i) { colsOfUnit[cellRow0[i]].insert(s.pos[cellCol[i]] >> 4); rowsOfUnit[cellRow0[i]] = cellRows[i]; }
  std::set<std::tuple<int, int, int>> quadPairs;
  for (const auto& kv : colsOfUnit) {
    const int r0 = kv.first, r1 = r0 + rowsOfUnit[r0] - 1;
    for (int q = r0 >> 2; q <= r1 >> 2; ++q)
      for (int I : kv.second)
        for (int J : kv.second)
          if (I >= J) quadPairs.insert(std::make_tuple(q, I, J));
  }
  std::vector<std::vector<std::pair<int, int>>> pairs(s.numTiles);
  for (const auto& qp : quadPairs) {
    const int q = std::get<0>(qp), I = std::get<1>(qp), J = std::get<2>(qp);
    const int t = s.tileIdTable[size_t(I) * T + J];
    if (t < 0) return "Gram plan: a Jacobian row couples two tile columns whose tile is not in the schedule";
    pairs[t].push_back({stripId[{q, I}], stripId[{q, J}]});
  }
  out.residOff = out.numStrips * 64;
  out.stride = (out.residOff + ((numRows + 3) & ~3) + 63) / 64 * 64;
  const int zeroStrip = out.stride / 64;
  out.tilePairStart.assign(s.numTiles + 1, 0);
  for (int t = 0; t < s.numTiles; ++t) {
    out.macs += int64_t(pairs[t].size()) * 16 * 16 * 4;
    if (pairs[t].size() % 2) pairs[t].push_back({zeroStrip, zeroStrip});
    out.tilePairStart[t + 1] = out.tilePairStart[t] + int(pairs[t].size());
    for (const auto& pr : pairs[t]) { out.pairA.push_back(pr.first); out.pairB.push_back(pr.second); }
  }
  out.tileQuadStart.assign(s.numTiles + 1, 0);
  for (int t = 0; t < s.numTiles; ++t) {
    out.tileQuadStart[t + 1] = out.tileQuadStart[t] + (out.tilePairStart[t + 1] - out.tilePairStart[t]) / 2;
    for (int p = out.tilePairStart[t]; p < out.tilePairStart[t + 1]; p += 2) {
      out.quad.push_back(out.pairA[p] * 64); out.quad.push_back(out.pairB[p] * 64);
      out.quad.push_back(out.pairA[p + 1] * 64); out.quad.push_back(out.pairB[p + 1] * 64);
    }
  }
  {
    std::vector<int> byLoad(s.numTiles);
    for (int t = 0; t < s.numTiles; ++t) byLoad[t] = t;
    std::stable_sort(byLoad.begin(), byLoad.end(), [&](int a, int b) { return pairs[a].size() > pairs[b].size(); });
    std::vector<std::vector<int>> ofWarp(kGramWarps);
    std::vector<int64_t> load(kGramWarps, 0);
    for (int t : byLoad) {
      int w = 0;
      for (int k = 1; k < kGramWarps; ++k) if (load[k] < load[w]) w = k;
      ofWarp[w].push_back(t);
      load[w] += int64_t(pairs[t].size()) / 2 + 2;
    }
    size_t rounds = 0;
    for (const auto& v : ofWarp) rounds = std::max(rounds, v.size());
    out.tileOrder.assign(rounds * kGramWarps, -1);
    for (int w = 0; w < kGramWarps; ++w)
      for (size_t r = 0; r < ofWarp[w].size(); ++r) out.tileOrder[r * kGramWarps + w] = ofWarp[w][r];
  }
  std::map<int, int> stripsOfQuad;
  for (const auto& kv : stripId) ++stripsOfQuad[kv.first.first];
  out.cellStripOff.resize(cellCol.size());
  out.cellQuadStride.resize(cellCol.size());
  for (size_t i = 0; i < cellCol.size(); ++i) {
    const int d = cellCol[i], K = s.pos[d] >> 4, q0 = cellRow0[i] >> 2;
    out.cellStripOff[i] = uint32_t(stripId[{q0, K}]) * 64u + uint32_t(d - s.perm[16 * K]) * 4u;
    out.cellQuadStride[i] = uint16_t(stripsOfQuad[q0]);
    for (int q = q0 + 1; q <= (cellRow0[i] + cellRows[i] - 1) >> 2; ++q)
      if (stripsOfQuad[q] != stripsOfQuad[q0] || stripId[{q, K}] != stripId[{q0, K}] + (q - q0) * stripsOfQuad[q0]) return "Gram plan: row quads of one unit are not laid out uniformly";
  }
  out.colStripStart.assign(T + 1, 0);
  for (int K = 0; K < T; ++K) {
    out.colStripStart[K + 1] = out.colStripStart[K] + int(ofCol[K].size());
    out.colStrip.insert(out.colStrip.end(), ofCol[K].begin(), ofCol[K].end());
  }
  return "";
}

void makeGramBlob(const GramPlan& g, const CholSchedule& s, std::vector<int32_t>& blob, int32_t offsets[8]) {
  blob.clear();
  int k = 0;
  auto add = [&](const std::vector<int32_t>& v) { offsets[k++] = int32_t(blob.size()); blob.insert(blob.end(), v.begin(), v.end()); while (blob.size() % 4) blob.push_back(0); };
  add(g.tileOrder); add(g.tileQuadStart); add(g.quad); add(std::vector<int32_t>()); add(g.colStripStart); add(g.colStrip);
  std::vector<int32_t> stripRow(g.numStrips), info(s.numTiles);
  for (int i = 0; i < g.numStrips; ++i) stripRow[i] = g.stripCoord[2 * i];
  auto validOf = [&](int K) { int v = 0; while (v < kCholTile && s.perm[16 * K + v] >= 0) ++v; return v; };
  for (int t = 0; t < s.numTiles; ++t) info[t] = validOf(s.tileRow[t]) | (validOf(s.tileCol[t]) << 8) | ((s.tileRow[t] == s.tileCol[t] ? 1 : 0) << 16);
  add(stripRow); add(info);
  if (blob.empty()) blob.push_back(0);
}

void layoutDeviceColumns(CholSchedule& s, std::vector<int32_t>& deviceColumnOrder) {
  deviceColumnOrder.clear();
  s.nParams = s.n;
  for (int K = 0; K < s.numTileCols; ++K) {
    while (deviceColumnOrder.size() % 4 != 0) deviceColumnOrder.push_back(-1);
    for (int j = 0; j < kCholTile; ++j) {
      int16_t& p = s.perm[16 * K + j];
      if (p < 0) continue;
      const int dev = int(deviceColumnOrder.size());
      deviceColumnOrder.push_back(p);
      p = int16_t(dev);
    }
  }
  s.n = int32_t(deviceColumnOrder.size());
  s.pos.assign(s.n, int16_t(-1));
  for (int slot = 0; slot < s.nPad; ++slot) if (s.perm[slot] >= 0) s.pos[s.perm[slot]] = int16_t(slot);
  s.order.assign(deviceColumnOrder.begin(), deviceColumnOrder.end());
}

}

namespace mb2 {

void makeScheduleBlob(const CholSchedule& s, std::vector<int32_t>& blob, CholSchedDev& dev) {
  blob.clear();
  std::vector<size_t> offs;
  auto add16 = [&](const std::vector<int16_t>& v) { offs.push_back(blob.size()); for (int16_t x : v) blob.push_back(int32_t(x)); while (blob.size() % 4) blob.push_back(0); };
  auto add32 = [&](const std::vector<int32_t>& v) { offs.push_back(blob.size()); blob.insert(blob.end(), v.begin(), v.end()); while (blob.size() % 4) blob.push_back(0); };
  add16(s.perm); add16(s.pos); add16(s.tileIdTable); add16(s.tileRow); add16(s.tileCol);
  add32(s.diagTile); add32(s.levelColStart); add32(s.levelCols); add32(s.levelPanelStart); add32(s.panelTile); add32(s.panelDiag);
  add32(s.levelTaskStart); add32(s.taskDst); add32(s.taskPairStart); add32(s.pairA); add32(s.pairB); add32(s.levelVTaskStart); add32(s.vtaskRow);
  add32(s.vtaskSrcStart); add32(s.vsrcTile); add32(s.vsrcCol); add32(s.colPanelStart); add32(s.colPanelTile); add32(s.colPanelRow);
  add32(s.levelOrderStart8); add32(s.taskOrder8); add32(s.levelOrderStart16); add32(s.taskOrder16);
  {
    std::vector<int32_t> info(size_t(s.numTiles) * 3, 0);
    auto validOf = [&](int K) { int v = 0; while (v < kCholTile && s.perm[16 * K + v] >= 0) ++v; return v; };
    for (int t = 0; t < s.numTiles; ++t) {
      const int I = s.tileRow[t], J = s.tileCol[t];
      const int vI = validOf(I), vJ = validOf(J);
      info[3 * t] = vI > 0 ? s.perm[16 * I] : 0;
      info[3 * t + 1] = vJ > 0 ? s.perm[16 * J] : 0;
      info[3 * t + 2] = vI | (vJ << 8) | ((I == J ? 1 : 0) << 16);
    }
    add32(info);
  }
  if (blob.empty()) blob.push_back(0);
  dev = CholSchedDev();
  dev.n = s.n; dev.nPad = s.nPad; dev.numTileCols = s.numTileCols; dev.numTiles = s.numTiles; dev.numLevels = s.numLevels;
  const int32_t* b = blob.data();
  dev.blob = b;
  dev.blobInts = int32_t(blob.size());
  int k = 0;
  dev.perm = b + offs[k++]; dev.pos = b + offs[k++]; dev.tileIdTable = b + offs[k++]; dev.tileRow = b + offs[k++]; dev.tileCol = b + offs[k++];
  dev.diagTile = b + offs[k++]; dev.levelColStart = b + offs[k++]; dev.levelCols = b + offs[k++]; dev.levelPanelStart = b + offs[k++];
  dev.panelTile = b + offs[k++]; dev.panelDiag = b + offs[k++]; dev.levelTaskStart = b + offs[k++]; dev.taskDst = b + offs[k++];
  dev.taskPairStart = b + offs[k++]; dev.pairA = b + offs[k++]; dev.pairB = b + offs[k++]; dev.levelVTaskStart = b + offs[k++]; dev.vtaskRow = b + offs[k++];
  dev.vtaskSrcStart = b + offs[k++]; dev.vsrcTile = b + offs[k++]; dev.vsrcCol = b + offs[k++]; dev.colPanelStart = b + offs[k++];
  dev.colPanelTile = b + offs[k++]; dev.colPanelRow = b + offs[k++];
  dev.levelOrderStart8 = b + offs[k++]; dev.taskOrder8 = b + offs[k++]; dev.levelOrderStart16 = b + offs[k++]; dev.taskOrder16 = b + offs[k++];
  dev.tileInfo = b + offs[k++];
}

}
```

momentum_b200/csrc/ik_chol_sched.cuh:

```cuda
#pragma once

#include <cmath>
#include <cstring>

#include "ik_types.h"

#include <vector_types.h>

namespace mb2 {

struct CholSchedDev {
  int32_t n, nPad, numTileCols, numTiles, numLevels;
  const int32_t* blob;
  int32_t blobInts;
  const int32_t* perm;
  const int32_t* pos;
  const int32_t* tileIdTable;
  const int32_t* tileRow;
  const int32_t* tileCol;
  const int32_t* diagTile;
  const int32_t* levelColStart;
  const int32_t* levelCols;
  const int32_t* levelPanelStart;
  const int32_t* panelTile;
  const int32_t* panelDiag;
  const int32_t* levelTaskStart;
  const int32_t* taskDst;
  const int32_t* taskPairStart;
  const int32_t* pairA;
  const int32_t* pairB;
  const int32_t* levelVTaskStart;
  const int32_t* vtaskRow;
  const int32_t* vtaskSrcStart;
  const int32_t* vsrcTile;
  const int32_t* vsrcCol;
  const int32_t* colPanelStart;
  const int32_t* colPanelTile;
  const int32_t* colPanelRow;
  const int32_t* levelOrderStart8;
  const int32_t* taskOrder8;
  const int32_t* levelOrderStart16;
  const int32_t* taskOrder16;
  const int32_t* tileInfo;
};
MB2_HD CholSchedDev rebaseSchedule(const CholSchedDev& S, const int32_t* newBlob) {
  CholSchedDev R = S;
  const int32_t* o = S.blob;
  R.blob = newBlob;
#define MB2_RB(f) R.f = newBlob + (S.f - o);
  MB2_RB(perm) MB2_RB(pos) MB2_RB(tileIdTable) MB2_RB(tileRow) MB2_RB(tileCol) MB2_RB(diagTile) MB2_RB(levelColStart) MB2_RB(levelCols)
  MB2_RB(levelPanelStart) MB2_RB(panelTile) MB2_RB(panelDiag) MB2_RB(levelTaskStart) MB2_RB(taskDst) MB2_RB(taskPairStart) MB2_RB(pairA) MB2_RB(pairB)
  MB2_RB(levelVTaskStart) MB2_RB(vtaskRow) MB2_RB(vtaskSrcStart) MB2_RB(vsrcTile) MB2_RB(vsrcCol) MB2_RB(colPanelStart) MB2_RB(colPanelTile)
  MB2_RB(colPanelRow) MB2_RB(levelOrderStart8) MB2_RB(taskOrder8) MB2_RB(levelOrderStart16) MB2_RB(taskOrder16) MB2_RB(tileInfo)
#undef MB2_RB
  return R;
}

MB2_HD int tileSlotOffset(int lane) { return (lane ^ (lane >> 3)) << 2; }
MB2_HD int tileIdx(int r, int c) {
  const int lane = ((r & 7) << 2) | ((c & 7) >> 1);
  return ((c >> 3) << 7) + ((lane ^ (lane >> 3)) << 2) + (((r >> 3) << 1) | (c & 1));
}
MB2_HD int fragRow(int lane, int e) { return (lane >> 2) + 8 * (e >> 1); }
MB2_HD int fragCol(int lane, int h, int e) { return 8 * h + 2 * (lane & 3) + (e & 1); }
MB2_HD void tileLoadFrag(const float* tile, int lane, float d[2][4]) {
  const int so = tileSlotOffset(lane);
#if defined(__CUDA_ARCH__)
  const float4 v0 = *reinterpret_cast<const float4*>(tile + so), v1 = *reinterpret_cast<const float4*>(tile + 128 + so);
  d[0][0] = v0.x; d[0][1] = v0.y; d[0][2] = v0.z; d[0][3] = v0.w; d[1][0] = v1.x; d[1][1] = v1.y; d[1][2] = v1.z; d[1][3] = v1.w;
#else
  for (int h = 0; h < 2; ++h) for (int e = 0; e < 4; ++e) d[h][e] = tile[128 * h + so + e];
#endif
}
MB2_HD void tileStoreFrag(float* tile, int lane, const float d[2][4]) {
  const int so = tileSlotOffset(lane);
#if defined(__CUDA_ARCH__)
  *reinterpret_cast<float4*>(tile + so) = make_float4(d[0][0], d[0][1], d[0][2], d[0][3]);
  *reinterpret_cast<float4*>(tile + 128 + so) = make_float4(d[1][0], d[1][1], d[1][2], d[1][3]);
#else
  for (int h = 0; h < 2; ++h) for (int e = 0; e < 4; ++e) tile[128 * h + so + e] = d[h][e];
#endif
}

MB2_HD float cholPadElement(float v, int info, int r, int c) {
  const int vI = info & 0xFF, vJ = (info >> 8) & 0xFF, diag = (info >> 16) & 1;
  if (r < vI && c < vJ) return v;
  return (diag && r == c) ? 1.f : 0.f;
}
MB2_HD int tmaBoxIdx(int c, int r) { return c * 16 + ((((r >> 2) ^ ((c >> 1) & 3)) << 2) | (r & 3)); }
MB2_HD void cholConvertBox(float* tile, int info, int lane) {
  float v[2][4];
#pragma unroll
  for (int h = 0; h < 2; ++h)
#pragma unroll
    for (int e = 0; e < 4; ++e) {
      const int r = fragRow(lane, e), c = fragCol(lane, h, e);
      const bool mirror = ((info >> 16) & 1) != 0 && c > r;
      v[h][e] = cholPadElement(tile[mirror ? tmaBoxIdx(r, c) : tmaBoxIdx(c, r)], info, r, c);
    }
#if defined(__CUDA_ARCH__)
  __syncwarp();
#endif
  tileStoreFrag(tile, lane, v);
}

MB2_HD float tf32High(float x) {
#if defined(__CUDA_ARCH__)
  return __uint_as_float((__float_as_uint(x) + 0x1000u) & 0xFFFFE000u);
#else
  uint32_t u;
  std::memcpy(&u, &x, 4);
  u = (u + 0x1000u) & 0xFFFFE000u;
  float r;
  std::memcpy(&r, &u, 4);
  return r;
#endif
}
#if defined(__CUDA_ARCH__)
__device__ __forceinline__ void mmaTf32K8(float d[4], float a0, float a1, float a2, float a3, float b0, float b1) {
  asm volatile("mma.sync.aligned.m16n8k8.row.col.f32.tf32.tf32.f32 {%0, %1, %2, %3}, {%4, %5, %6, %7}, {%8, %9}, {%0, %1, %2, %3};"
               : "+f"(d[0]), "+f"(d[1]), "+f"(d[2]), "+f"(d[3])
               : "r"(__float_as_uint(a0)), "r"(__float_as_uint(a1)), "r"(__float_as_uint(a2)), "r"(__float_as_uint(a3)), "r"(__float_as_uint(b0)),
                 "r"(__float_as_uint(b1)));
}
__device__ __forceinline__ void mma3xTf32Step(float d[2][4], float small[2][4], float a0, float a1, float a2, float a3, float b00, float b01, float b10, float b11) {
  const float a0h = tf32High(a0), a1h = tf32High(a1), a2h = tf32High(a2), a3h = tf32High(a3);
  const float b00h = tf32High(b00), b01h = tf32High(b01), b10h = tf32High(b10), b11h = tf32High(b11);
  const float a0l = a0 - a0h, a1l = a1 - a1h, a2l = a2 - a2h, a3l = a3 - a3h;
  const float b00l = b00 - b00h, b01l = b01 - b01h, b10l = b10 - b10h, b11l = b11 - b11h;
  mmaTf32K8(small[0], a0l, a1l, a2l, a3l, b00h, b01h); mmaTf32K8(small[1], a0l, a1l, a2l, a3l, b10h, b11h);
  mmaTf32K8(small[0], a0h, a1h, a2h, a3h, b00l, b01l); mmaTf32K8(small[1], a0h, a1h, a2h, a3h, b10l, b11l);
  float t0[4] = {0.f, 0.f, 0.f, 0.f}, t1[4] = {0.f, 0.f, 0.f, 0.f};
  mmaTf32K8(t0, a0h, a1h, a2h, a3h, b00h, b01h); mmaTf32K8(t1, a0h, a1h, a2h, a3h, b10h, b11h);
#pragma unroll
  for (int e = 0; e < 4; ++e) { d[0][e] += t0[e]; d[1][e] += t1[e]; }
}
#endif
MB2_HD void mma3xEmulate(float& d, float& small, const float av[8], const float bv[8]) {
  float lo = 0.f, mid = 0.f, hi = 0.f;
  for (int k = 0; k < 8; ++k) {
    const float ah = tf32High(av[k]), bh = tf32High(bv[k]), al = av[k] - ah, bl = bv[k] - bh;
    lo += al * bh; mid += ah * bl; hi += ah * bh;
  }
  small += lo + mid;
  d += hi;
}

MB2_HD void gramTilePairs(const float* strips, int oa0, int ob0, int oa1, int ob1, int lane, float d[2][4], float small[2][4]) {
  const float* A0 = strips + oa0;
  const float* B0 = strips + ob0;
  const float* A1 = strips + oa1;
  const float* B1 = strips + ob1;
#if defined(__CUDA_ARCH__)
  mma3xTf32Step(d, small, A0[lane], A0[32 + lane], A1[lane], A1[32 + lane], B0[lane], B1[lane], B0[32 + lane], B1[32 + lane]);
#else
  for (int h = 0; h < 2; ++h)
    for (int e = 0; e < 4; ++e) {
      const int r = fragRow(lane, e), c = fragCol(lane, h, e);
      float av[8], bv[8];
      for (int k = 0; k < 8; ++k) { av[k] = k < 4 ? A0[4 * r + k] : A1[4 * r + k - 4]; bv[k] = k < 4 ? B0[4 * c + k] : B1[4 * c + k - 4]; }
      mma3xEmulate(d[h][e], small[h][e], av, bv);
    }
#endif
}
MB2_HD void gramTileAccumulate(const float* strips, const int32_t* quads, int q0, int q1, int lane, float d[2][4]) {
  float small[2][4] = {{0.f, 0.f, 0.f, 0.f}, {0.f, 0.f, 0.f, 0.f}};
  for (int q = q0; q < q1; ++q) {
#if defined(__CUDA_ARCH__)
    const int4 o = *reinterpret_cast<const int4*>(quads + 4 * q);
    gramTilePairs(strips, o.x, o.y, o.z, o.w, lane, d, small);
#else
    gramTilePairs(strips, quads[4 * q], quads[4 * q + 1], quads[4 * q + 2], quads[4 * q + 3], lane, d, small);
#endif
  }
#pragma unroll
  for (int h = 0; h < 2; ++h)
#pragma unroll
    for (int e = 0; e < 4; ++e) d[h][e] += small[h][e];
}
MB2_HD void gramTileStore(float* tile, const float d[2][4], int info, float lambda, int lane) {
  const int vI = info & 0xFF, vJ = (info >> 8) & 0xFF, diag = (info >> 16) & 1;
  if (vI == 16 && vJ == 16 && !diag) { tileStoreFrag(tile, lane, d); return; }
  float v[2][4];
#pragma unroll
  for (int h = 0; h < 2; ++h)
#pragma unroll
    for (int e = 0; e < 4; ++e) {
      const int r = fragRow(lane, e), c = fragCol(lane, h, e);
      v[h][e] = cholPadElement((diag && r == c) ? d[h][e] + lambda : d[h][e], info, r, c);
    }
  tileStoreFrag(tile, lane, v);
}
MB2_HD float gramVectorEntry(const float* strips, const float* resid, const int32_t* colStrip, const int32_t* stripRow, int s0, int s1, int hl) {
  float g0 = 0.f, g1 = 0.f;
  for (int k = s0; k < s1; ++k) {
    const int sidx = colStrip[k];
    const float4 sv = *reinterpret_cast<const float4*>(strips + size_t(sidx) * 64 + 4 * hl);
    const float4 rv = *reinterpret_cast<const float4*>(resid + stripRow[sidx]);
    g0 += sv.x * rv.x + sv.y * rv.y;
    g1 += sv.z * rv.z + sv.w * rv.w;
  }
  return g0 + g1;
}

MB2_HD void tileLoadRow(const float* tile, int r, float* a) {
#pragma unroll
  for (int j = 0; j < 16; j += 2) {
    const float2 v = *reinterpret_cast<const float2*>(tile + tileIdx(r, j));
    a[j] = v.x; a[j + 1] = v.y;
  }
}
MB2_HD void tileStoreRow(float* tile, int r, const float* a) {
#pragma unroll
  for (int j = 0; j < 16; j += 2) {
    float2 v;
    v.x = a[j]; v.y = a[j + 1];
    *reinterpret_cast<float2*>(tile + tileIdx(r, j)) = v;
  }
}

MB2_HD void cholDiagTile(float* tile, float* y16, int lane, float fallback, int* fail) {
#if defined(__CUDA_ARCH__)
  const int hl = lane & 15;
  const bool isE = lane >= 16;
  float v[16];
#pragma unroll
  for (int k = 0; k < 16; ++k) v[k] = isE ? (k == hl ? 1.f : 0.f) : tile[tileIdx(k, hl)];
  float z = isE ? 0.f : y16[hl], rdSelf = 0.f;
  __syncwarp();
#pragma unroll
  for (int k = 0; k < 16; ++k) {
    float* blk = tile + 32 * (k & 1);
    if (!isE) { blk[hl] = v[k]; blk[16 + hl] = z; }
    __syncwarp();
    float c[16];
#pragma unroll
    for (int g4 = (k >> 2); g4 < 4; ++g4) {
      const float4 q = *reinterpret_cast<const float4*>(blk + 4 * g4);
      c[4 * g4] = q.x; c[4 * g4 + 1] = q.y; c[4 * g4 + 2] = q.z; c[4 * g4 + 3] = q.w;
    }
    float piv = c[k];
    const float zk = blk[16 + k];
    if (!(piv > 0.f)) { piv = fallback; if (lane == k) *fail = 1; }
    float inv;
    asm("rcp.approx.ftz.f32 %0, %1;" : "=f"(inv) : "f"(piv));
    const float rdk = rsqrtf(piv);
    if (lane == k) rdSelf = rdk;
    const float m = v[k] * inv;
    const float tm = (!isE && hl > k) ? m : 0.f;
#pragma unroll
    for (int j = k + 1; j < 16; ++j) v[j] -= m * c[j];
    z -= tm * zk;
    v[k] *= rdk;
  }
  __syncwarp();
  if (!isE) y16[hl] = z * rdSelf;
  else {
#pragma unroll
    for (int i = 0; i < 16; ++i) tile[tileIdx(i, hl)] = v[i];
  }
#else
  if (lane != 0) return;
  float A[16][16], E[16][16], z[16], rd[16];
  for (int l = 0; l < 16; ++l) { for (int k = 0; k < 16; ++k) { A[l][k] = tile[tileIdx(k, l)]; E[k][l] = (k == l) ? 1.f : 0.f; } z[l] = y16[l]; }
  for (int k = 0; k < 16; ++k) {
    float piv = A[k][k];
    if (!(piv > 0.f)) { piv = fallback; *fail = 1; }
    const float inv = 1.f / piv;
    rd[k] = 1.f / sqrtf(piv);
    const float zk = z[k];
    float c[16];
    for (int j = 0; j < 16; ++j) c[j] = A[j][k];
    for (int l = 0; l < 16; ++l) {
      const float m = c[l] * inv;
      for (int j = k + 1; j < 16; ++j) A[l][j] -= m * c[j];
      if (l > k) z[l] -= m * zk;
    }
    for (int l = 0; l < 16; ++l) {
      const float m = E[k][l] * inv;
      for (int j = k + 1; j < 16; ++j) E[j][l] -= m * c[j];
      E[k][l] *= rd[k];
    }
  }
  for (int l = 0; l < 16; ++l) {
    y16[l] = z[l] * rd[l];
    for (int i = 0; i < 16; ++i) tile[tileIdx(i, l)] = E[i][l];
  }
#endif
}

MB2_HD void tileProduct(const float* TA, const float* TB, int lane, float d[2][4], float small[2][4]) {
#if defined(__CUDA_ARCH__)
  const int so = tileSlotOffset(lane);
  const float4 a0 = *reinterpret_cast<const float4*>(TA + so), a1 = *reinterpret_cast<const float4*>(TA + 128 + so);
  const float4 b0 = *reinterpret_cast<const float4*>(TB + so), b1 = *reinterpret_cast<const float4*>(TB + 128 + so);
  mma3xTf32Step(d, small, a0.x, a0.z, a0.y, a0.w, b0.x, b0.y, b0.z, b0.w);
  mma3xTf32Step(d, small, a1.x, a1.z, a1.y, a1.w, b1.x, b1.y, b1.z, b1.w);
#else
  for (int h = 0; h < 2; ++h)
    for (int e = 0; e < 4; ++e) {
      const int r = fragRow(lane, e), c = fragCol(lane, h, e);
      for (int ks = 0; ks < 2; ++ks) {
        float av[8], bv[8];
        for (int k = 0; k < 8; ++k) { av[k] = TA[tileIdx(r, 8 * ks + k)]; bv[k] = TB[tileIdx(c, 8 * ks + k)]; }
        mma3xEmulate(d[h][e], small[h][e], av, bv);
      }
    }
#endif
}

MB2_HD void cholPanelProduct(const float* tile, const float* diagW, int lane, float out[2][4]) {
  float small[2][4];
#pragma unroll
  for (int h = 0; h < 2; ++h)
#pragma unroll
    for (int e = 0; e < 4; ++e) { out[h][e] = 0.f; small[h][e] = 0.f; }
  tileProduct(tile, diagW, lane, out, small);
#pragma unroll
  for (int h = 0; h < 2; ++h)
#pragma unroll
    for (int e = 0; e < 4; ++e) out[h][e] += small[h][e];
}
MB2_HD void cholPanelStore(float* tile, int lane, const float out[2][4]) { tileStoreFrag(tile, lane, out); }

MB2_HD void cholUpdateTask(float* tiles, const CholSchedDev& S, int task, int lane) {
  float d[2][4], small[2][4];
#pragma unroll
  for (int h = 0; h < 2; ++h)
#pragma unroll
    for (int e = 0; e < 4; ++e) { d[h][e] = 0.f; small[h][e] = 0.f; }
  for (int p = S.taskPairStart[task]; p < S.taskPairStart[task + 1]; ++p)
    tileProduct(tiles + size_t(S.pairA[p]) * 256, tiles + size_t(S.pairB[p]) * 256, lane, d, small);
  float* D = tiles + size_t(S.taskDst[task]) * 256;
  float v[2][4];
  tileLoadFrag(D, lane, v);
#pragma unroll
  for (int h = 0; h < 2; ++h)
#pragma unroll
    for (int e = 0; e < 4; ++e) v[h][e] -= d[h][e] + small[h][e];
  tileStoreFrag(D, lane, v);
}

MB2_HD void cholVectorTask(const float* tiles, float* y, const CholSchedDev& S, int vtask, int hl) {
  float s0 = 0.f, s1 = 0.f, s2 = 0.f, s3 = 0.f;
  for (int p = S.vtaskSrcStart[vtask]; p < S.vtaskSrcStart[vtask + 1]; ++p) {
    float t[16];
    tileLoadRow(tiles + size_t(S.vsrcTile[p]) * 256, hl, t);
    const float* yk = y + S.vsrcCol[p] * 16;
#pragma unroll
    for (int c = 0; c < 16; c += 4) { s0 += t[c] * yk[c]; s1 += t[c + 1] * yk[c + 1]; s2 += t[c + 2] * yk[c + 2]; s3 += t[c + 3] * yk[c + 3]; }
  }
  y[S.vtaskRow[vtask] * 16 + hl] -= (s0 + s1) + (s2 + s3);
}

MB2_HD void cholBackwardColumn(const float* tiles, float* y, const CholSchedDev& S, int K, int lane) {
#if defined(__CUDA_ARCH__)
  const int g = lane >> 2, t = lane & 3, so = tileSlotOffset(lane);
  float c0 = 0.f, c1 = 0.f, c2 = 0.f, c3 = 0.f;
  for (int p = S.colPanelStart[K]; p < S.colPanelStart[K + 1]; ++p) {
    const float* T = tiles + size_t(S.colPanelTile[p]) * 256;
    const float* yi = y + S.colPanelRow[p] * 16;
    const float4 v0 = *reinterpret_cast<const float4*>(T + so), v1 = *reinterpret_cast<const float4*>(T + 128 + so);
    const float ya = yi[g], yb = yi[g + 8];
    c0 = fmaf(v0.x, ya, fmaf(v0.z, yb, c0)); c1 = fmaf(v0.y, ya, fmaf(v0.w, yb, c1));
    c2 = fmaf(v1.x, ya, fmaf(v1.z, yb, c2)); c3 = fmaf(v1.y, ya, fmaf(v1.w, yb, c3));
  }
#pragma unroll
  for (int o = 4; o < 32; o <<= 1) {
    c0 += __shfl_xor_sync(0xffffffffu, c0, o); c1 += __shfl_xor_sync(0xffffffffu, c1, o);
    c2 += __shfl_xor_sync(0xffffffffu, c2, o); c3 += __shfl_xor_sync(0xffffffffu, c3, o);
  }
  float* yk = y + K * 16;
  if (g == 0) { yk[2 * t] -= c0; yk[2 * t + 1] -= c1; yk[8 + 2 * t] -= c2; yk[9 + 2 * t] -= c3; }
  __syncwarp();
  const float* W = tiles + size_t(S.diagTile[K]) * 256;
  const float4 w0 = *reinterpret_cast<const float4*>(W + so), w1 = *reinterpret_cast<const float4*>(W + 128 + so);
  const float sa = yk[g], sb = yk[g + 8];
  float x0 = fmaf(w0.x, sa, w0.z * sb), x1 = fmaf(w0.y, sa, w0.w * sb), x2 = fmaf(w1.x, sa, w1.z * sb), x3 = fmaf(w1.y, sa, w1.w * sb);
#pragma unroll
  for (int o = 4; o < 32; o <<= 1) {
    x0 += __shfl_xor_sync(0xffffffffu, x0, o); x1 += __shfl_xor_sync(0xffffffffu, x1, o);
    x2 += __shfl_xor_sync(0xffffffffu, x2, o); x3 += __shfl_xor_sync(0xffffffffu, x3, o);
  }
  __syncwarp();
  if (g == 0) { yk[2 * t] = x0; yk[2 * t + 1] = x1; yk[8 + 2 * t] = x2; yk[9 + 2 * t] = x3; }
#else
  if (lane != 0) return;
  float s[16];
  for (int c = 0; c < 16; ++c) s[c] = 0.f;
  for (int p = S.colPanelStart[K]; p < S.colPanelStart[K + 1]; ++p) {
    const float* T = tiles + size_t(S.colPanelTile[p]) * 256;
    const float* yi = y + S.colPanelRow[p] * 16;
    for (int c = 0; c < 16; ++c) for (int r = 0; r < 16; ++r) s[c] += T[tileIdx(r, c)] * yi[r];
  }
  float* yk = y + K * 16;
  for (int c = 0; c < 16; ++c) s[c] = yk[c] - s[c];
  const float* W = tiles + size_t(S.diagTile[K]) * 256;
  for (int c = 0; c < 16; ++c) {
    float x = 0.f;
    for (int r = 0; r < 16; ++r) x += W[tileIdx(r, c)] * s[r];
    yk[c] = x;
  }
#endif
}

}
```

momentum_b200/csrc/ik_chol_sched.h:

```cpp
#pragma once

#include <cstdint>
#include <string>
#include <vector>

namespace mb2 {

constexpr int kCholTile = 16;

struct CholSchedule {
  int32_t n{0}, nPad{0}, numTileCols{0}, numTiles{0}, numLevels{0};
  int32_t nParams{0};
  std::vector<int16_t> perm;
  std::vector<int16_t> pos;
  std::vector<int16_t> tileIdTable;
  std::vector<int16_t> tileRow, tileCol;
  std::vector<int32_t> diagTile;
  std::vector<int32_t> levelColStart, levelCols;
  std::vector<int32_t> levelPanelStart, panelTile, panelDiag, panelRow;
  std::vector<int32_t> levelTaskStart, taskDst, taskPairStart, pairA, pairB;
  std::vector<int32_t> levelOrderStart8, taskOrder8, levelOrderStart16, taskOrder16;
  std::vector<int32_t> levelVTaskStart, vtaskRow, vtaskSrcStart, vsrcTile, vsrcCol;
  std::vector<int32_t> colPanelStart, colPanelTile, colPanelRow;
  std::vector<int> order;
  int64_t tileOps{0};
  int64_t denseTileOps{0};
};

std::string buildCholSchedule(int n, const std::vector<std::vector<int>>& cliques, bool forceDense, CholSchedule& out, const std::vector<int>* priority = nullptr);
void layoutDeviceColumns(CholSchedule& s, std::vector<int32_t>& deviceColumnOrder);

inline int cholSchedLdH(int n) { return (n + 1 + 15) / 16 * 16; }
constexpr int kGramWarps = 8;
constexpr int kGramCholMaxRounds = 8;
struct GramPlan {
  int32_t numStrips{0}, numTiles{0}, numTileCols{0};
  std::vector<int32_t> stripCoord;
  std::vector<int32_t> tileOrder;
  std::vector<int32_t> tilePairStart;
  std::vector<int32_t> pairA, pairB;
  std::vector<int32_t> tileQuadStart;
  std::vector<int32_t> quad;
  std::vector<int32_t> colStripStart;
  std::vector<int32_t> colStrip;
  std::vector<uint32_t> cellStripOff;
  std::vector<uint16_t> cellQuadStride;
  int32_t residOff{0};
  int32_t stride{0};
  int64_t macs{0};
};
std::string buildGramPlan(const CholSchedule& s, const std::vector<int32_t>& cellRow0, const std::vector<int32_t>& cellRows, const std::vector<int32_t>& cellCol,
                          int numRows, GramPlan& out);

void makeGramBlob(const GramPlan& g, const CholSchedule& s, std::vector<int32_t>& blob, int32_t offsets[8]);

struct CholSchedDev;
void makeScheduleBlob(const CholSchedule& s, std::vector<int32_t>& blob, CholSchedDev& dev);

}
```

momentum_b200/csrc/ik_kernels.cu:

```cuda
#include "ik_kernels.cuh"

#include <algorithm>
#include <cstdio>
#include <type_traits>

#include "ik_chol.cuh"
#include "ik_chol_sched.h"
#include "ik_jtj_tc.cuh"
#include "ik_ptx.cuh"
#include "ik_device.cuh"

namespace mb2 {

__device__ __forceinline__ double warpSum(double v) {
  for (int o = 16; o > 0; o >>= 1) v += __shfl_xor_sync(0xffffffffu, v, o);
  return v;
}

size_t sweepSmemPerInstance(const FunctionTables& T, int warpsPerInstance) {
  const size_t nPad = (T.numParams + 3) & ~3;
  const size_t jp = warpsPerInstance > 1 ? size_t((T.numJoints * kParametersPerJoint + 1) & ~1) : 0;
  return sizeof(float) * (nPad + jp + size_t((T.numJoints * kJointStateStride + 1) & ~1) + size_t((T.recStride + 1) & ~1) + 4 + 2 * size_t(warpsPerInstance));
}

MB2_HD size_t tableWords(size_t count, size_t elemBytes) { return (count * elemBytes + 15) / 16 * 4; }
size_t sweepTableBytes(const FunctionTables& T, int mode) {
  if (mode == 0) return 0;
  const size_t J = T.numJoints;
  size_t w = 0;
  w += tableWords(J, 4) + tableWords(3 * J, 4) + tableWords(4 * J, 4);
  w += tableWords(7 * J + 1, 4) + tableWords(T.ptNnz, 4) * 2 + tableWords(7 * J, 4);
  w += tableWords(T.numLevels + 1, 4) + tableWords(J, 4);
  w += tableWords(T.numEf, sizeof(EfDesc)) + tableWords(T.numUnits, sizeof(UnitDesc)) + tableWords(T.numLimitData, 4);
  if (mode == 1) w += tableWords(T.numCells, sizeof(CellDesc)) + tableWords(T.numContribs, sizeof(ContribDesc));
  return w * 4;
}

template <class E>
__device__ __forceinline__ void stageTable(const E*& table, size_t count, uint32_t*& cursor) {
  static_assert(sizeof(E) % 4 == 0, "tables are staged word by word");
  const uint32_t* src = reinterpret_cast<const uint32_t*>(table);
  const size_t words = count * (sizeof(E) / 4);
  const int nt = int(blockDim.x);
  size_t i = threadIdx.x;
  for (; i + 7 * size_t(nt) < words; i += 8 * size_t(nt)) {
    uint32_t v[8];
#pragma unroll
    for (int k = 0; k < 8; ++k) v[k] = src[i + size_t(k) * nt];
#pragma unroll
    for (int k = 0; k < 8; ++k) cursor[i + size_t(k) * nt] = v[k];
  }
  for (; i < words; i += nt) cursor[i] = src[i];
  table = reinterpret_cast<const E*>(cursor);
  cursor += tableWords(count, sizeof(E));
}

constexpr int kSweepMaxWarps = 24;
template <bool kJacobian, int W, int kStage>
__global__ void __launch_bounds__(32 * kSweepMaxWarps) sweepKernel(const SweepArgs a) {
  extern __shared__ __align__(16) float smem[];
  FunctionTables T = a.T;
  const int warp = threadIdx.x >> 5, lane = threadIdx.x & 31;
  const int group = warp / W, gl = (warp % W) * 32 + lane;
  constexpr int gs = 32 * W;
  const int groupsPerCta = (blockDim.x >> 5) / W;
  const int nPad = (T.numParams + 3) & ~3;
  const int jpFloats = W > 1 ? ((T.numJoints * kParametersPerJoint + 1) & ~1) : 0;
  const int perGroup = nPad + jpFloats + ((T.numJoints * kJointStateStride + 1) & ~1) + ((T.recStride + 1) & ~1) + 4 + 2 * W;
  float* th = smem + size_t(group) * perGroup;
  float* jp = W > 1 ? th + nPad : nullptr;
  float* js = th + nPad + jpFloats;
  float* rec = js + ((T.numJoints * kJointStateStride + 1) & ~1);
  double* errSlots = reinterpret_cast<double*>(rec + ((T.recStride + 1) & ~1));
  auto groupSync = [&]() {
    if (W == 1) __syncwarp();
    else asm volatile("bar.sync %0, %1;" ::"r"(1 + group), "r"(gs) : "memory");
  };
  if constexpr (kStage != 0) {
    uint32_t* cursor = reinterpret_cast<uint32_t*>(smem + ((size_t(groupsPerCta) * perGroup + 3) & ~size_t(3)));
    const size_t J = T.numJoints;
    stageTable(T.parent, J, cursor); stageTable(T.offset, 3 * J, cursor); stageTable(T.prerot, 4 * J, cursor);
    stageTable(T.ptOuter, 7 * J + 1, cursor); stageTable(T.ptInner, T.ptNnz, cursor); stageTable(T.ptVals, T.ptNnz, cursor);
    stageTable(T.ptOffsets, 7 * J, cursor);
    stageTable(T.levelStart, T.numLevels + 1, cursor); stageTable(T.levelJoints, J, cursor);
    stageTable(T.efs, T.numEf, cursor); stageTable(T.units, T.numUnits, cursor); stageTable(T.limitData, T.numLimitData, cursor);
    if constexpr (kStage == 1) { stageTable(T.cells, T.numCells, cursor); stageTable(T.contribs, T.numContribs, cursor); }
    __syncthreads();
  }

  for (int b = blockIdx.x * groupsPerCta + group; b < a.batch; b += gridDim.x * groupsPerCta) {
    if (a.active != nullptr && a.active[b] == 0) continue;
    const float* theta = a.theta + size_t(b) * a.ldTheta;
    for (int i = gl; i < T.numParams; i += gs) th[i] = theta[i];
    groupSync();
    if (W == 1) {
      const int bn = b + gridDim.x * groupsPerCta;
      if (bn < a.batch) { const float* tn = a.theta + size_t(bn) * a.ldTheta; for (int i = gl * 8; i < T.numParams; i += gs * 8) asm volatile("prefetch.global.L2 [%0];" ::"l"(tn + i)); }
    }
    if constexpr (W > 1) {
      for (int row = gl; row < T.numJoints * kParametersPerJoint; row += gs) jp[row] = jointParameterRow(T, row, th);
      groupSync();
      for (int j = gl; j < T.numJoints; j += gs) fkLocal<kJacobian>(T, j, jp, js);
    } else {
      for (int j = gl; j < T.numJoints; j += gs) fkLocalFromTheta<kJacobian>(T, j, th, js);
    }
    groupSync();
    for (int lvl = 1; lvl < T.numLevels; ++lvl) {
      const int end = T.levelStart[lvl + 1];
      for (int k = T.levelStart[lvl] + gl; k < end; k += gs) fkCompose(T, T.levelJoints[k], js);
      groupSync();
    }
    if (kJacobian) {
      for (int i = gl; i < 3 * T.numJoints; i += gs) fkAxis(T, i / 3, i % 3, js);
      groupSync();
    }
    if (a.stateOut != nullptr) {
      float* so = a.stateOut + size_t(b) * T.numJoints * 8;
      for (int i = gl; i < T.numJoints * 8; i += gs) so[i] = js[(i >> 3) * kJointStateStride + (i & 7)];
    }
    const float* targets = a.targets + size_t(b) * T.targetStride;
    const float* cw = a.cweights + (T.weightsPerInstance ? size_t(b) * T.numWeights : 0);
    float* J = kJacobian ? a.jacobian + size_t(b) * T.jacobianStride : nullptr;
    float* residual = kJacobian ? J + (T.stripMode ? size_t(T.residOff) : size_t(T.numCols) * T.ldJ) : nullptr;
    double err = 0.0;
    for (int u = gl; u < T.numUnits; u += gs) err += (double)evalUnit<kJacobian>(T, u, th, jp, js, targets, cw, rec, residual);
    err = warpSum(err);
    if (W > 1 && lane == 0) errSlots[warp % W] = err;
    groupSync();
    if (kJacobian)
      for (int c = gl; c < T.numCells; c += gs) jacobianCell(T, c, js, rec, targets, J);
    if (gl == 0) {
      if (W > 1) { err = 0.0; for (int w = 0; w < W; ++w) err += errSlots[w]; }
      a.errors[b] = kJacobian ? err : (double)(float)err;
    }
    groupSync();
  }
}

static int g_numSms = 0;
static int g_maxSmemOptin = 0;
static int g_maxSmemPerSm = 0;

cudaError_t launchSweep(const SweepArgs& a0, bool jacobian, cudaStream_t stream) {
  SweepArgs a = a0;
  const size_t budget = size_t(g_maxSmemOptin);
  const size_t per1 = sweepSmemPerInstance(a.T, 8);
  a.stageTables = (2 * per1 + sweepTableBytes(a.T, 1) + 16 <= budget) ? 1 : (2 * per1 + sweepTableBytes(a.T, 2) + 16 <= budget) ? 2 : 0;
  const size_t tableBytes = sweepTableBytes(a.T, a.stageTables) + 16;
  int groups = int((budget - tableBytes) / per1);
  if (groups < 1) return cudaErrorInvalidConfiguration;
  const int groupsOneWarp = int((budget - tableBytes) / sweepSmemPerInstance(a.T, 1));
  int W = 1;
  if (groupsOneWarp >= 16) {
    const int sms = std::max(g_numSms, 1);
    const int maxG = std::min(groupsOneWarp, kSweepMaxWarps), minG = std::min(12, maxG);
    long best = -1;
    if (a.batch < sms * minG) { groups = std::max(1, (a.batch + sms - 1) / sms); best = 0; }
    for (int gcand = maxG; gcand >= minG && best != 0; --gcand) {
      const long rounds = (a.batch + long(sms) * gcand - 1) / (long(sms) * gcand);
      if (best < 0 || rounds * gcand < best) { best = rounds * gcand; groups = gcand; }
    }
  } else {
    if (groups > 15) groups = 15;
    while (W < 8 && groups * W * 2 <= kSweepMaxWarps) W *= 2;
  }
  a.warpsPerInstance = W;
  const int warps = groups * W;
  const size_t per = sweepSmemPerInstance(a.T, W);
  const size_t smem = per * groups + tableBytes;
  if (smem > budget) return cudaErrorInvalidConfiguration;
  const int ctasNeeded = (a.batch + groups - 1) / groups;
  int ctasPerSm = (int)((size_t(g_maxSmemPerSm)) / (smem + 1024));
  if (ctasPerSm < 1) ctasPerSm = 1;
  if (ctasPerSm * warps > 32) ctasPerSm = 32 / warps > 0 ? 32 / warps : 1;
  int grid = g_numSms * ctasPerSm;
  if (grid > ctasNeeded) grid = ctasNeeded;
  if (grid < 1) grid = 1;
  auto launch = [&](auto kernel) -> cudaError_t {
    const cudaError_t e = cudaFuncSetAttribute(kernel, cudaFuncAttributeMaxDynamicSharedMemorySize, int(smem));
    if (e != cudaSuccess) return e;
    kernel<<<grid, warps * 32, smem, stream>>>(a);
    return cudaGetLastError();
  };
  auto pick = [&](auto jac, auto staged) -> cudaError_t {
    constexpr bool kJ = decltype(jac)::value;
    constexpr int kS = decltype(staged)::value;
    switch (W) {
      case 1: return launch(sweepKernel<kJ, 1, kS>);
      case 2: return launch(sweepKernel<kJ, 2, kS>);
      case 4: return launch(sweepKernel<kJ, 4, kS>);
      default: return launch(sweepKernel<kJ, 8, kS>);
    }
  };
  auto pickStage = [&](auto jac) -> cudaError_t {
    switch (a.stageTables) {
      case 1: return pick(jac, std::integral_constant<int, 1>{});
      case 2: return pick(jac, std::integral_constant<int, 2>{});
      default: return pick(jac, std::integral_constant<int, 0>{});
    }
  };
  return jacobian ? pickStage(std::true_type{}) : pickStage(std::false_type{});
}


constexpr int kJtjTile = 64;
constexpr int kJtjKc = 32;

__global__ void __launch_bounds__(256) jtjSimtKernel(const JtJArgs a) {
  const int b = blockIdx.y;
  if (a.active != nullptr && a.active[b] == 0) return;
  int t = blockIdx.x, ti = 0;
  while ((ti + 1) * (ti + 2) / 2 <= t) ++ti;
  const int tj = t - ti * (ti + 1) / 2;
  __shared__ float As[kJtjTile][kJtjKc + 1];
  __shared__ float Bs[kJtjTile][kJtjKc + 1];
  __shared__ float rs[kJtjKc];
  const float* J = a.jacobian + size_t(b) * (a.numCols + 1) * a.ldJ;
  const float* r = J + size_t(a.numCols) * a.ldJ;
  const int tx = threadIdx.x & 15, ty = threadIdx.x >> 4;
  float acc[4][4];
#pragma unroll
  for (int i = 0; i < 4; ++i)
#pragma unroll
    for (int j = 0; j < 4; ++j) acc[i][j] = 0.f;
  float gacc = 0.f;
  const bool diag = (ti == tj);
  for (int k0 = 0; k0 < a.kRows; k0 += kJtjKc) {
    for (int idx = threadIdx.x; idx < kJtjTile * kJtjKc; idx += 256) {
      const int c = idx / kJtjKc, kk = idx % kJtjKc;
      const int ia = ti * kJtjTile + c, ib = tj * kJtjTile + c;
      const int k = k0 + kk;
      As[c][kk] = (ia < a.ns && k < a.kRows) ? J[size_t(ia) * a.ldJ + k] : 0.f;
      Bs[c][kk] = (ib < a.ns && k < a.kRows) ? J[size_t(ib) * a.ldJ + k] : 0.f;
    }
    if (threadIdx.x < kJtjKc) rs[threadIdx.x] = (k0 + threadIdx.x < a.kRows) ? r[k0 + threadIdx.x] : 0.f;
    __syncthreads();
#pragma unroll 8
    for (int kk = 0; kk < kJtjKc; ++kk) {
      float av[4], bv[4];
#pragma unroll
      for (int i = 0; i < 4; ++i) av[i] = As[ty * 4 + i][kk];
#pragma unroll
      for (int j = 0; j < 4; ++j) bv[j] = Bs[tx * 4 + j][kk];
#pragma unroll
      for (int i = 0; i < 4; ++i)
#pragma unroll
        for (int j = 0; j < 4; ++j) acc[i][j] = fmaf(av[i], bv[j], acc[i][j]);
    }
    if (diag && threadIdx.x < kJtjTile)
      for (int kk = 0; kk < kJtjKc; ++kk) gacc = fmaf(As[threadIdx.x][kk], rs[kk], gacc);
    __syncthreads();
  }
  float* H = a.H + size_t(b) * a.hStride;
#pragma unroll
  for (int i = 0; i < 4; ++i)
#pragma unroll
    for (int j = 0; j < 4; ++j) {
      const int gi = ti * kJtjTile + ty * 4 + i, gj = tj * kJtjTile + tx * 4 + j;
      if (gi < a.ns && gj <= gi) { H[size_t(gj) * a.ldH + gi] = acc[i][j]; H[size_t(gi) * a.ldH + gj] = acc[i][j]; }
    }
  if (diag && threadIdx.x < kJtjTile) {
    const int gi = ti * kJtjTile + threadIdx.x;
    if (gi < a.ns) {
      H[size_t(gi) * a.ldH + a.ns] = gacc; H[size_t(a.ns) * a.ldH + gi] = gacc;
      if (a.g != nullptr) a.g[size_t(b) * a.ldG + gi] = gacc;
    }
  }
}

cudaError_t launchJtJSimt(const JtJArgs& a, cudaStream_t stream) {
  const int tiles = (a.ns + kJtjTile - 1) / kJtjTile;
  dim3 grid(tiles * (tiles + 1) / 2, a.batch);
  jtjSimtKernel<<<grid, 256, 0, stream>>>(a);
  return cudaGetLastError();
}

__device__ void cholFinish(const CholArgs& a, int b, int n, const float* dsub, const float* gsub, bool failed, const int32_t* slotOf = nullptr) {
  const int tid = threadIdx.x;
  float* theta = a.theta + size_t(b) * a.ldTheta;
  float part = 0.f;
  for (int i = tid; i < n; i += blockDim.x) {
    const int c = a.cols[i];
    const float d = c >= 0 ? dsub[slotOf != nullptr ? slotOf[i] : i] : 0.f;
    a.delta[size_t(b) * n + i] = d;
    if (c >= 0) part += gsub[i] * d;
    if (a.applyUpdate && c >= 0) theta[c] -= d;
  }
  if (a.gradDotDelta != nullptr) {
    __shared__ float red[32];
    for (int o = 16; o > 0; o >>= 1) part += __shfl_xor_sync(0xffffffffu, part, o);
    if ((tid & 31) == 0) red[tid >> 5] = part;
    __syncthreads();
    if (tid == 0) {
      float s = 0.f;
      for (int w = 0; w < int(blockDim.x >> 5); ++w) s += red[w];
      a.gradDotDelta[b] = s;
    }
  }
  if (tid == 0) {
    if (failed && a.status[b] == 0) a.status[b] = 1;
    if (a.bookkeeping) {
      const double error = a.errors[b], last = a.lastErrors[b];
      if (a.history != nullptr) a.history[size_t(b) * a.maxIterations + a.iteration] = error;
      const bool converged = fabs(last - error) / (fabs(error) + (double)FLT_MIN) <= (double)(a.threshold * FLT_EPSILON);
      a.iterations[b] = a.iteration + 1;
      if ((a.iteration >= a.minIterations && converged) || a.iteration + 1 >= a.maxIterations) a.active[b] = 0;
      else { a.lastErrors[b] = error; atomicAdd(a.activeCount, 1); }
    }
  }
}

template <int NB>
__global__ void __launch_bounds__(kCholThreads) choleskyKernel(const CholArgs a, const int useSmemMatrix) {
  extern __shared__ float smem[];
  const int b = blockIdx.x;
  if (a.active[b] == 0) return;
  const int n = a.ns;
  const int tid = threadIdx.x;
  float* Hg = a.H + size_t(b) * a.hStride;
  CholCtx ctx;
  ctx.n = n;
  int ldp = ((n + 1 + 3) & ~3) + 4;
  float* P = smem;
  float* gsave = P + NB * ldp;
  int* flags = reinterpret_cast<int*>(gsave + ((n + 3) & ~3));
  float* As = reinterpret_cast<float*>(flags + 4);
  if (useSmemMatrix) {
    ctx.lda = n | 1;
    ctx.A = As;
    for (int idx = tid; idx < (n + 1) * n; idx += kCholThreads) {
      const int j = idx / (n + 1), i = idx - j * (n + 1);
      if (i >= j) {
        float v = Hg[size_t(j) * a.ldH + i];
        if (i == j) v += a.regularization;
        As[i * ctx.lda + j] = v;
      }
    }
  } else {
    ctx.lda = a.ldH;
    ctx.A = Hg;
    for (int idx = tid; idx < (n + 1) * n; idx += kCholThreads) {
      const int j = idx / (n + 1), i = idx - j * (n + 1);
      if (i > j) Hg[size_t(i) * a.ldH + j] = Hg[size_t(j) * a.ldH + i];
    }
    for (int i = tid; i < n; i += kCholThreads) Hg[size_t(i) * a.ldH + i] += a.regularization;
  }
  ctx.P = P;
  ctx.ldp = ldp;
  ctx.fail = flags;
  if (tid == 0) flags[0] = 0;
  for (int i = tid; i < n; i += kCholThreads) gsave[i] = Hg[size_t(i) * a.ldH + n];
  __syncthreads();

  const int blockSize = cholBlockSize(n, NB);
  for (int k = 0; k < n; k += blockSize) {
    const int bs = min(blockSize, n - k);
    if (tid < 32) {
      for (int jj = 0; jj < bs; ++jj) {
        const float x = cholDiagPivot(ctx, k, jj);
        __syncwarp();
        if (!(x > 0.f)) { if (tid == 0) flags[0] = k + jj + 1; break; }
        cholDiagColumn(ctx, k, bs, jj, x, tid);
        __syncwarp();
      }
    }
    __syncthreads();
    if (flags[0] != 0) break;
    cholPanelSolve<NB>(ctx, k, bs, tid, kCholThreads);
    __syncthreads();
    cholTrailingUpdate<NB>(ctx, k, bs, tid, kCholThreads);
    __syncthreads();
  }
  float* y = ctx.A + size_t(n) * ctx.lda;
  if (flags[0] != 0) {
    if (tid == 0) cholForwardFrom(ctx, cholCompletedColumns(flags[0] - 1, blockSize), y);
    __syncthreads();
  }
  for (int i0 = ((n - 1) / 32) * 32; i0 >= 0; i0 -= 32) {
    const int nb = min(32, n - i0);
    if (tid < 32) {
      float yv = tid < nb ? y[i0 + tid] : 0.f;
      float dinv = tid < nb ? 1.f / ctx.A[size_t(i0 + tid) * ctx.lda + i0 + tid] : 0.f;
      for (int kk = nb - 1; kk >= 0; --kk) {
        const float xk = __shfl_sync(0xffffffffu, yv, kk) * __shfl_sync(0xffffffffu, dinv, kk);
        if (tid == kk) yv = xk;
        else if (tid < kk) yv -= ctx.A[size_t(i0 + kk) * ctx.lda + i0 + tid] * xk;
      }
      if (tid < nb) y[i0 + tid] = yv;
    }
    __syncthreads();
    for (int i = tid; i < i0; i += kCholThreads) {
      float s = y[i];
      for (int kk = 0; kk < nb; ++kk) s -= ctx.A[size_t(i0 + kk) * ctx.lda + i] * y[i0 + kk];
      y[i] = s;
    }
    __syncthreads();
  }
  cholFinish(a, b, n, y, gsave, flags[0] != 0);
}

static size_t cholSmemBytes(int n, int NB, bool matrixInSmem) {
  const size_t ldp = ((n + 1 + 3) & ~3) + 4;
  size_t s = sizeof(float) * (NB * ldp + ((n + 3) & ~3)) + 4 * sizeof(int);
  if (matrixInSmem) s += sizeof(float) * size_t(n + 1) * (n | 1);
  return s;
}

cudaError_t launchCholesky(const CholArgs& a, cudaStream_t stream) {
  const int n = a.ns;
  const int eig = cholBlockSize(n, 32);
  const int NB = eig <= 8 ? 8 : (eig <= 16 ? 16 : 32);
  bool inSmem = cholSmemBytes(n, NB, true) <= size_t(g_maxSmemOptin);
  const size_t smem = cholSmemBytes(n, NB, inSmem);
  cudaError_t e = cudaSuccess;
#define MB2_LAUNCH_CHOL(NBV)                                                                                   \
  e = cudaFuncSetAttribute(choleskyKernel<NBV>, cudaFuncAttributeMaxDynamicSharedMemorySize, int(smem));       \
  if (e != cudaSuccess) return e;                                                                              \
  choleskyKernel<NBV><<<a.batch, kCholThreads, smem, stream>>>(a, inSmem ? 1 : 0);
  if (NB == 8) { MB2_LAUNCH_CHOL(8) } else if (NB == 16) { MB2_LAUNCH_CHOL(16) } else { MB2_LAUNCH_CHOL(32) }
#undef MB2_LAUNCH_CHOL
  return cudaGetLastError();
}

constexpr int kGramThreads = 32 * kGramWarps;

size_t gramTilesSmemBytes(size_t stripStride, int blobInts) { return 128 + sizeof(float) * (stripStride + 64) + 16 + sizeof(int32_t) * size_t((blobInts + 3) & ~3); }

template <int kThreads>
__global__ void __launch_bounds__(kThreads) gramTilesKernel(const GramArgs a) {
  extern __shared__ __align__(16) float gramSmem[];
  const int b = blockIdx.x;
  if (a.active != nullptr && a.active[b] == 0) return;
  const int tid = threadIdx.x, warp = tid >> 5, lane = tid & 31, hw = tid >> 4, hl = tid & 15;
  float* strips = gramSmem + (((128u - (smemAddr(gramSmem) & 127u)) & 127u) >> 2);
  float* resid = strips + a.residOff;
  float* zero = strips + a.stripStride;
  unsigned long long* bar = reinterpret_cast<unsigned long long*>(zero + 64);
  const uint32_t barAddr = smemAddr(bar);
  const uint32_t total = uint32_t(a.stripStride) * 4u;
  if (tid < 64) zero[tid] = 0.f;
  if (tid == 0) {
    mbarInit(barAddr, 1);
    fenceBarrierInit();
    mbarExpectTx(barAddr, total);
    const char* src = reinterpret_cast<const char*>(a.strips + size_t(b) * a.stripStride);
    for (uint32_t off = 0; off < total; off += 16384u) bulkLoad(smemAddr(strips) + off, src + off, total - off < 16384u ? total - off : 16384u, barAddr);
  }
  int32_t* tab = reinterpret_cast<int32_t*>(bar + 2);
  for (int i = tid; i < a.blobInts; i += kThreads) tab[i] = __ldg(a.blob + i);
  __syncthreads();
  mbarWaitRelaxed(barAddr, 0);
  const int32_t* tileOrder = tab + a.offTileOrder, *tileQuadStart = tab + a.offTilePairStart, *quads = tab + a.offPairA;
  const int32_t* colStripStart = tab + a.offColStripStart, *colStrip = tab + a.offColStrip, *stripRow = tab + a.offStripRow, *tileInfo = tab + a.offTileInfo;
  float* out = a.out + size_t(b) * a.outStride;
  for (int ti = warp; ti < a.numOrder; ti += kThreads / 32) {
    const int t = tileOrder[ti];
    if (t < 0) continue;
    float acc[2][4];
#pragma unroll
    for (int i = 0; i < 2; ++i)
#pragma unroll
      for (int j = 0; j < 4; ++j) acc[i][j] = 0.f;
    gramTileAccumulate(strips, quads, tileQuadStart[t], tileQuadStart[t + 1], lane, acc);
    gramTileStore(out + size_t(t) * 256, acc, tileInfo[t], a.regularization, lane);
  }
  float* y = out + size_t(a.numTiles) * 256;
  for (int K = hw; K < a.numTileCols; K += kThreads / 16)
    y[16 * K + hl] = gramVectorEntry(strips, resid, colStrip, stripRow, colStripStart[K], colStripStart[K + 1], hl);
}

cudaError_t launchGramTiles(const GramArgs& a, cudaStream_t stream) {
  const size_t smem = gramTilesSmemBytes(a.stripStride, a.blobInts);
  if (smem > size_t(g_maxSmemOptin) || (a.stripStride & 3) != 0) return cudaErrorInvalidConfiguration;
  const bool wide = 2 * (smem + 1024) > size_t(g_maxSmemPerSm);
  cudaError_t e = wide ? cudaFuncSetAttribute(gramTilesKernel<512>, cudaFuncAttributeMaxDynamicSharedMemorySize, int(smem))
                       : cudaFuncSetAttribute(gramTilesKernel<kGramThreads>, cudaFuncAttributeMaxDynamicSharedMemorySize, int(smem));
  if (e != cudaSuccess) return e;
  if (wide) gramTilesKernel<512><<<a.batch, 512, smem, stream>>>(a);
  else gramTilesKernel<kGramThreads><<<a.batch, kGramThreads, smem, stream>>>(a);
  return cudaGetLastError();
}


size_t choleskyScheduledSmemBytes(int n, int nPad, int numTiles, int blobInts) {
  return 1024  + sizeof(float) * (size_t(numTiles) * 256 + size_t(nPad) + 2 * size_t((n + 3) & ~3)) +
         sizeof(int32_t) * size_t((blobInts + 3) & ~3) + 32;
}

template <int kSchedThreads, bool kProfile>
__global__ void __launch_bounds__(kSchedThreads, kSchedThreads == 256 ? 3 : 1) choleskyScheduledKernel(const __grid_constant__ CUtensorMap hmap, const CholArgs a, const CholSchedDev Sg) {
  extern __shared__ __align__(16) float smemRaw[];
  const int b = blockIdx.x;
  if (a.active[b] == 0) return;
  const int n = a.ns, tid = threadIdx.x;
  const int warp = tid >> 5, lane = tid & 31, hw = tid >> 4, hl = tid & 15;
  const unsigned hmask = 0xFFFFu << (16 * ((tid >> 4) & 1));
  float* tiles = smemRaw + (((1024u - (smemAddr(smemRaw) & 1023u)) & 1023u) >> 2);
  float* y = tiles + size_t(Sg.numTiles) * 256;
  float* gsub = y + Sg.nPad;
  float* dsub = gsub + ((n + 3) & ~3);
  int32_t* blob = reinterpret_cast<int32_t*>(dsub + ((n + 3) & ~3));
  int* flags = reinterpret_cast<int*>(blob + ((Sg.blobInts + 3) & ~3));
  unsigned long long* bar = reinterpret_cast<unsigned long long*>(flags + 2);
  long long pc[9] = {0, 0, 0, 0, 0, 0, 0, 0, 0}, pt = clock64();
#define MB2_PROF(k) if constexpr (kProfile) { const long long now = clock64(); pc[k] += now - pt; pt = now; }
  const uint32_t barAddr = smemAddr(bar);
  const uint32_t blobBytes = uint32_t((Sg.blobInts + 3) & ~3) * 4u, gBytes = uint32_t(a.ldG) * 4u;
  const bool fromGram = a.tilesIn != nullptr;
  const uint32_t tileBytes = uint32_t(Sg.numTiles) * 1024u, yBytes = uint32_t(Sg.nPad) * 4u;
  if (tid == 0) {
    flags[0] = 0;
    mbarInit(barAddr, 1);
    fenceBarrierInit();
    mbarExpectTx(barAddr, blobBytes + tileBytes + (fromGram ? yBytes : gBytes));
  }
  __syncthreads();
  if (fromGram) {
    if (tid == 0) {
      bulkLoad(smemAddr(blob), Sg.blob, blobBytes, barAddr);
      const float* src = a.tilesIn + size_t(b) * a.tilesStride;
      const uint32_t total = tileBytes + yBytes;
      for (uint32_t off = 0; off < total; off += 16384u)
        bulkLoad(smemAddr(tiles) + off, reinterpret_cast<const char*>(src) + off, total - off < 16384u ? total - off : 16384u, barAddr);
    }
  } else {
    if (tid == 0) {
      bulkLoad(smemAddr(blob), Sg.blob, blobBytes, barAddr);
      bulkLoad(smemAddr(gsub), a.g + size_t(b) * a.ldG, gBytes, barAddr);
    }
    for (int t = tid; t < Sg.numTiles; t += kSchedThreads) {
      const int gi0 = __ldg(Sg.tileInfo + 3 * t), gj0 = __ldg(Sg.tileInfo + 3 * t + 1);
      tmaLoad3d(smemAddr(tiles + size_t(t) * 256), &hmap, gi0, gj0, b, barAddr);
    }
  }
  MB2_PROF(6)
  mbarWaitRelaxed(barAddr, 0);
  MB2_PROF(7)
  const CholSchedDev S = rebaseSchedule(Sg, blob);
  if (fromGram) {
    for (int s = tid; s < S.nPad; s += kSchedThreads) {
      const int p = S.perm[s];
      if (p >= 0) gsub[p] = y[s];
    }
  } else {
    for (int t = warp; t < S.numTiles; t += kSchedThreads / 32) cholConvertBox(tiles + size_t(t) * 256, S.tileInfo[3 * t + 2], lane);
    for (int s = tid; s < S.nPad; s += kSchedThreads) {
      const int p = S.perm[s];
      y[s] = p >= 0 ? gsub[p] : 0.f;
    }
  }
  __syncthreads();
  MB2_PROF(8)
  if (!fromGram)
    for (int s = tid; s < S.nPad; s += kSchedThreads)
      if (S.perm[s] >= 0) tiles[size_t(S.diagTile[s >> 4]) * 256 + tileIdx(s & 15, s & 15)] += a.regularization;
  __syncthreads();
  MB2_PROF(0)

  for (int L = 0; L < S.numLevels; ++L) {
    for (int ci = S.levelColStart[L] + warp; ci < S.levelColStart[L + 1]; ci += kSchedThreads / 32) {
      const int K = S.levelCols[ci];
      cholDiagTile(tiles + size_t(S.diagTile[K]) * 256, y + 16 * K, lane, a.regularization, flags);
    }
    __syncthreads();
    MB2_PROF(1)
    for (int pi = S.levelPanelStart[L] + warp; pi < S.levelPanelStart[L + 1]; pi += kSchedThreads / 32) {
      float* ptile = tiles + size_t(S.panelTile[pi]) * 256;
      float x[2][4];
      cholPanelProduct(ptile, tiles + size_t(S.panelDiag[pi]) * 256, lane, x);
      cholPanelStore(ptile, lane, x);
    }
    __syncthreads();
    MB2_PROF(2)
    {
      const int32_t* oStart = kSchedThreads == 256 ? S.levelOrderStart8 : S.levelOrderStart16, *order = kSchedThreads == 256 ? S.taskOrder8 : S.taskOrder16;
      for (int oi = oStart[L] + warp; oi < oStart[L + 1]; oi += kSchedThreads / 32) { const int ti = order[oi]; if (ti >= 0) cholUpdateTask(tiles, S, ti, lane); }
    }
    for (int vi = S.levelVTaskStart[L] + hw; vi < S.levelVTaskStart[L + 1]; vi += kSchedThreads / 16) cholVectorTask(tiles, y, S, vi, hl);
    __syncthreads();
    MB2_PROF(3)
  }
  for (int L = S.numLevels - 1; L >= 0; --L) {
    for (int ci = S.levelColStart[L] + warp; ci < S.levelColStart[L + 1]; ci += kSchedThreads / 32) cholBackwardColumn(tiles, y, S, S.levelCols[ci], lane);
    __syncthreads();
  }
  MB2_PROF(4)
  for (int i = tid; i < S.nPad; i += kSchedThreads) { const int p = S.perm[i]; if (p >= 0) dsub[p] = y[i]; }
  __syncthreads();
  cholFinish(a, b, n, dsub, gsub, flags[0] != 0);
  MB2_PROF(5)
  if (kProfile && b == 0 && tid == 0)
    printf("chol-profile (cycles, block 0): blob %lld issue %lld wait %lld lambda %lld diag %lld panel %lld update %lld backward %lld finish %lld | levels %d tiles %d\n", pc[6], pc[7],
           pc[8], pc[0], pc[1], pc[2], pc[3], pc[4], pc[5], S.numLevels, S.numTiles);
#undef MB2_PROF
}

cudaError_t launchCholeskyScheduled(const CholArgs& a, const CholSchedDev& sched, cudaStream_t stream) {
  const size_t smem = choleskyScheduledSmemBytes(a.ns, sched.nPad, sched.numTiles, sched.blobInts);
  if (smem > size_t(g_maxSmemOptin)) return cudaErrorInvalidConfiguration;
  const bool wide = 2 * (smem + 1024) > size_t(g_maxSmemPerSm);
  const bool prof = (a.profile & 1) != 0;
  cudaError_t e;
  if (wide) e = prof ? cudaFuncSetAttribute(choleskyScheduledKernel<512, true>, cudaFuncAttributeMaxDynamicSharedMemorySize, int(smem))
                     : cudaFuncSetAttribute(choleskyScheduledKernel<512, false>, cudaFuncAttributeMaxDynamicSharedMemorySize, int(smem));
  else e = prof ? cudaFuncSetAttribute(choleskyScheduledKernel<256, true>, cudaFuncAttributeMaxDynamicSharedMemorySize, int(smem))
                : cudaFuncSetAttribute(choleskyScheduledKernel<256, false>, cudaFuncAttributeMaxDynamicSharedMemorySize, int(smem));
  if (e != cudaSuccess) return e;
  if (a.tilesIn == nullptr && (a.g == nullptr || a.ldG != cholGradientLd(a.ns))) return cudaErrorInvalidValue;
  if ((a.ldH & 3) != 0 || (a.hStride & 3) != 0 || (a.tilesStride & 3) != 0) return cudaErrorInvalidValue;
  CUtensorMap hmap;
  const bool fromGram = a.tilesIn != nullptr;
  const uint64_t dims[3] = {uint64_t(fromGram ? 256 : a.ldH), uint64_t(fromGram ? sched.numTiles : a.ns + 1), uint64_t(a.batch)};
  const uint64_t strides[2] = {uint64_t(fromGram ? 256 : a.ldH) * sizeof(float), uint64_t(fromGram ? a.tilesStride : a.hStride) * sizeof(float)};
  const uint32_t box[3] = {16u, 16u, 1u};
  e = makeTensorMap3d(&hmap, fromGram ? a.tilesIn : a.H, dims, strides, box, 64);
  if (e != cudaSuccess) return e;
  if (wide && prof) choleskyScheduledKernel<512, true><<<a.batch, 512, smem, stream>>>(hmap, a, sched);
  else if (wide) choleskyScheduledKernel<512, false><<<a.batch, 512, smem, stream>>>(hmap, a, sched);
  else if (prof) choleskyScheduledKernel<256, true><<<a.batch, 256, smem, stream>>>(hmap, a, sched);
  else choleskyScheduledKernel<256, false><<<a.batch, 256, smem, stream>>>(hmap, a, sched);
  return cudaGetLastError();
}

size_t gramCholeskySmemBytes(size_t stripStride, int gramBlobInts, int n, int nPad, int numTiles, int schedBlobInts) {
  (void)gramBlobInts; (void)schedBlobInts;
  const size_t uni = std::max<size_t>(size_t(numTiles) * 256, stripStride + 64);
  return 128 + sizeof(float) * (((uni + 3) & ~size_t(3)) + size_t(nPad) + size_t((n + 3) & ~3)) + 32;
}

template <bool kProfile>
__global__ void __launch_bounds__(kGramThreads, 4) gramCholeskyKernel(const GramCholArgs a, const CholSchedDev S) {
  extern __shared__ __align__(16) float gcSmem[];
  const GramArgs& g = a.g;
  const CholArgs& c = a.c;
  const int b = blockIdx.x;
  if (c.active[b] == 0) return;
  const int n = c.ns, tid = threadIdx.x;
  const int warp = tid >> 5, lane = tid & 31, hw = tid >> 4, hl = tid & 15;
  const unsigned hmask = 0xFFFFu << (16 * ((tid >> 4) & 1));
  float* U = gcSmem + (((128u - (smemAddr(gcSmem) & 127u)) & 127u) >> 2);
  const size_t tileFloats = size_t(S.numTiles) * 256, sweepFloats = g.stripStride + 64;
  const size_t uni = ((tileFloats > sweepFloats ? tileFloats : sweepFloats) + 3) & ~size_t(3);
  float* strips = U;
  float* resid = U + g.residOff;
  float* tiles = U;
  float* y = U + uni;
  float* gsub = y + S.nPad;
  int* flags = reinterpret_cast<int*>(gsub + ((n + 3) & ~3));
  unsigned long long* bar = reinterpret_cast<unsigned long long*>(flags + 4);
  long long pc[8] = {0, 0, 0, 0, 0, 0, 0, 0}, pt = 0;
  if constexpr (kProfile) pt = clock64();
#define MB2_GC(k) if constexpr (kProfile) { const long long now = clock64(); pc[k] += now - pt; pt = now; }
  const uint32_t barAddr = smemAddr(bar);
  const uint32_t stripBytes = uint32_t(g.stripStride) * 4u;
  if (tid == 0) {
    flags[0] = 0;
    mbarInit(barAddr, 1);
    fenceBarrierInit();
    mbarExpectTx(barAddr, stripBytes);
    const char* src = reinterpret_cast<const char*>(g.strips + size_t(b) * g.stripStride);
    for (uint32_t off = 0; off < stripBytes; off += 16384u) bulkLoad(smemAddr(strips) + off, src + off, stripBytes - off < 16384u ? stripBytes - off : 16384u, barAddr);
  }
  if (tid >= 64 && tid < 128) strips[g.stripStride + (tid - 64)] = 0.f;
  __syncthreads();
  mbarWaitRelaxed(barAddr, 0);
  MB2_GC(0)
  const int32_t* __restrict__ gtab = g.blob;
  const int32_t* tileOrder = gtab + g.offTileOrder, *tileQuadStart = gtab + g.offTilePairStart, *quads = gtab + g.offPairA;
  const int32_t* colStripStart = gtab + g.offColStripStart, *colStrip = gtab + g.offColStrip, *stripRow = gtab + g.offStripRow, *tileInfo = gtab + g.offTileInfo;
  float parked[kGramCholMaxRounds][8];
  {
    int slot = 0;
    for (int ti = warp; ti < g.numOrder; ti += kGramThreads / 32, ++slot) {
      const int t = tileOrder[ti];
      if (t < 0) continue;
      float acc[2][4];
#pragma unroll
      for (int i = 0; i < 2; ++i)
#pragma unroll
        for (int j = 0; j < 4; ++j) acc[i][j] = 0.f;
      gramTileAccumulate(strips, quads, tileQuadStart[t], tileQuadStart[t + 1], lane, acc);
      if (size_t(t) * 256 >= sweepFloats) gramTileStore(tiles + size_t(t) * 256, acc, tileInfo[t], g.regularization, lane);
      else {
#pragma unroll
        for (int i = 0; i < 8; ++i) parked[slot][i] = acc[i >> 2][i & 3];
      }
    }
    for (int K = hw; K < S.numTileCols; K += kGramThreads / 16)
      y[16 * K + hl] = gramVectorEntry(strips, resid, colStrip, stripRow, colStripStart[K], colStripStart[K + 1], hl);
  }
  __syncthreads();
  MB2_GC(1)
  {
    int slot = 0;
    for (int ti = warp; ti < g.numOrder; ti += kGramThreads / 32, ++slot) {
      const int t = tileOrder[ti];
      if (t < 0 || size_t(t) * 256 >= sweepFloats) continue;
      float acc[2][4];
#pragma unroll
      for (int i = 0; i < 8; ++i) acc[i >> 2][i & 3] = parked[slot][i];
      gramTileStore(tiles + size_t(t) * 256, acc, tileInfo[t], g.regularization, lane);
    }
    for (int s2 = tid; s2 < S.nPad; s2 += kGramThreads) {
      const int p = S.perm[s2];
      if (p >= 0) gsub[p] = y[s2];
    }
  }
  __syncthreads();
  MB2_GC(2)
  for (int L = 0; L < S.numLevels; ++L) {
    for (int ci = S.levelColStart[L] + warp; ci < S.levelColStart[L + 1]; ci += kGramThreads / 32) {
      const int K = S.levelCols[ci];
      cholDiagTile(tiles + size_t(S.diagTile[K]) * 256, y + 16 * K, lane, c.regularization, flags);
    }
    __syncthreads();
    MB2_GC(3)
    for (int pi = S.levelPanelStart[L] + warp; pi < S.levelPanelStart[L + 1]; pi += kGramThreads / 32) {
      float* ptile = tiles + size_t(S.panelTile[pi]) * 256;
      float x[2][4];
      cholPanelProduct(ptile, tiles + size_t(S.panelDiag[pi]) * 256, lane, x);
      cholPanelStore(ptile, lane, x);
    }
    __syncthreads();
    MB2_GC(4)
    for (int oi = S.levelOrderStart8[L] + warp; oi < S.levelOrderStart8[L + 1]; oi += kGramThreads / 32) { const int ti = S.taskOrder8[oi]; if (ti >= 0) cholUpdateTask(tiles, S, ti, lane); }
    for (int vi = S.levelVTaskStart[L] + hw; vi < S.levelVTaskStart[L + 1]; vi += kGramThreads / 16) cholVectorTask(tiles, y, S, vi, hl);
    __syncthreads();
    MB2_GC(5)
  }
  for (int L = S.numLevels - 1; L >= 0; --L) {
    for (int ci = S.levelColStart[L] + warp; ci < S.levelColStart[L + 1]; ci += kGramThreads / 32) cholBackwardColumn(tiles, y, S, S.levelCols[ci], lane);
    __syncthreads();
  }
  MB2_GC(6)
  cholFinish(c, b, n, y, gsub, flags[0] != 0, S.pos);
  MB2_GC(7)
  if constexpr (kProfile) {
    if (b == int(gridDim.x >> 1) && tid == 0 && a.phaseCycles != nullptr)
      for (int k = 0; k < 8; ++k) a.phaseCycles[k] += (unsigned long long)pc[k];
  }
#undef MB2_GC
}

cudaError_t launchGramCholesky(const GramCholArgs& a, const CholSchedDev& sched, bool profile, cudaStream_t stream) {
  const size_t smem = gramCholeskySmemBytes(a.g.stripStride, a.g.blobInts, a.c.ns, sched.nPad, sched.numTiles, sched.blobInts);
  if (smem > size_t(g_maxSmemOptin) || (a.g.stripStride & 3) != 0) return cudaErrorInvalidConfiguration;
  if (a.g.numOrder > kGramCholMaxRounds * (kGramThreads / 32)) return cudaErrorInvalidConfiguration;
  cudaError_t e = profile ? cudaFuncSetAttribute(gramCholeskyKernel<true>, cudaFuncAttributeMaxDynamicSharedMemorySize, int(smem))
                          : cudaFuncSetAttribute(gramCholeskyKernel<false>, cudaFuncAttributeMaxDynamicSharedMemorySize, int(smem));
  if (e != cudaSuccess) return e;
  e = profile ? cudaFuncSetAttribute(gramCholeskyKernel<true>, cudaFuncAttributePreferredSharedMemoryCarveout, int(cudaSharedmemCarveoutMaxShared))
              : cudaFuncSetAttribute(gramCholeskyKernel<false>, cudaFuncAttributePreferredSharedMemoryCarveout, int(cudaSharedmemCarveoutMaxShared));
  if (e != cudaSuccess) return e;
  if (profile) gramCholeskyKernel<true><<<a.c.batch, kGramThreads, smem, stream>>>(a, sched);
  else gramCholeskyKernel<false><<<a.c.batch, kGramThreads, smem, stream>>>(a, sched);
  return cudaGetLastError();
}

}
#include "ik_qr.cuh"
#include "ik_tr_qr.cuh"
namespace mb2 {

cudaError_t initKernelAttributes() {
  int dev = 0;
  cudaError_t e = cudaGetDevice(&dev);
  if (e != cudaSuccess) return e;
  e = cudaDeviceGetAttribute(&g_numSms, cudaDevAttrMultiProcessorCount, dev);
  if (e != cudaSuccess) return e;
  e = cudaDeviceGetAttribute(&g_maxSmemPerSm, cudaDevAttrMaxSharedMemoryPerMultiprocessor, dev);
  if (e != cudaSuccess) return e;
  return cudaDeviceGetAttribute(&g_maxSmemOptin, cudaDevAttrMaxSharedMemoryPerBlockOptin, dev);
}

__global__ void trialUpdateKernel(int batch, const float* thetaOrig, int ldTheta, const float* delta, int ns, const int32_t* cols, const float* scale,
                                  float* thetaTrial, const int32_t* active) {
  const int b = blockIdx.x;
  if (active[b] == 0) return;
  const float s = scale[b];
  for (int i = threadIdx.x; i < ns; i += blockDim.x) {
    const int c = cols[i];
    if (c >= 0) thetaTrial[size_t(b) * ldTheta + c] = thetaOrig[size_t(b) * ldTheta + c] - s * delta[size_t(b) * ns + i];
  }
}
cudaError_t launchTrialUpdate(int batch, const float* thetaOrig, int ldTheta, const float* delta, int ns, const int32_t* cols, const float* scale,
                              float* thetaTrial, const int32_t* active, cudaStream_t stream) {
  trialUpdateKernel<<<batch, 128, 0, stream>>>(batch, thetaOrig, ldTheta, delta, ns, cols, scale, thetaTrial, active);
  return cudaGetLastError();
}

__global__ void lineSearchStepKernel(const LineSearchArgs a) {
  const int b = blockIdx.x * blockDim.x + threadIdx.x;
  if (b >= a.batch || a.searching[b] == 0) return;
  const double error = a.errors[b], errorNew = a.trialErrors[b];
  const float scale = a.scale[b];
  bool accept;
  if (!a.subsetVariant) {
    const float scaledError = 1e-3f * (float)error;
    accept = (error - errorNew) >= (double)(scale * scaledError);
  } else {
    accept = (error - errorNew) >= (double)(1e-4f * scale) * (double)a.gradDotDelta[b];
  }
  if (accept || a.step >= 9) a.searching[b] = 0;
  else a.scale[b] = scale * 0.5f;
}
cudaError_t launchLineSearchStep(const LineSearchArgs& a, cudaStream_t stream) {
  lineSearchStepKernel<<<(a.batch + 127) / 128, 128, 0, stream>>>(a);
  return cudaGetLastError();
}

__global__ void commitTrialKernel(int batch, int numParams, int ldTheta, const float* thetaTrial, float* theta, const int32_t* active) {
  const int b = blockIdx.x;
  if (active[b] == 0) return;
  for (int i = threadIdx.x; i < numParams; i += blockDim.x) theta[size_t(b) * ldTheta + i] = thetaTrial[size_t(b) * ldTheta + i];
}
cudaError_t launchCommitTrial(int batch, int numParams, int ldTheta, const float* thetaTrial, float* theta, const int32_t* active, cudaStream_t stream) {
  commitTrialKernel<<<batch, 128, 0, stream>>>(batch, numParams, ldTheta, thetaTrial, theta, active);
  return cudaGetLastError();
}

__global__ void bookkeepingKernel(const BookkeepingArgs a) {
  const int b = blockIdx.x * blockDim.x + threadIdx.x;
  if (b >= a.batch || a.active[b] == 0) return;
  const double error = a.errors[b], last = a.lastErrors[b];
  if (a.history != nullptr) a.history[size_t(b) * a.maxIterations + a.iteration] = error;
  const bool converged = fabs(last - error) / (fabs(error) + (double)FLT_MIN) <= (double)(a.threshold * FLT_EPSILON);
  a.iterations[b] = a.iteration + 1;
  if ((a.iteration >= a.minIterations && converged) || a.iteration + 1 >= a.maxIterations) a.active[b] = 0;
  else { a.lastErrors[b] = error; atomicAdd(a.activeCount, 1); }
}
cudaError_t launchBookkeeping(const BookkeepingArgs& a, cudaStream_t stream) {
  bookkeepingKernel<<<(a.batch + 127) / 128, 128, 0, stream>>>(a);
  return cudaGetLastError();
}

__global__ void normalizeQuatsKernel(float* base, int count, int strideFloats, int quatsPerRecord, int batch) {
  const int idx = blockIdx.x * blockDim.x + threadIdx.x;
  if (idx >= batch * quatsPerRecord) return;
  const int b = idx / quatsPerRecord, q = idx % quatsPerRecord;
  float* p = base + size_t(b) * strideFloats + 4 * q;
  const float n = sqrtf(p[0] * p[0] + p[1] * p[1] + p[2] * p[2] + p[3] * p[3]);
  p[0] /= n; p[1] /= n; p[2] /= n; p[3] /= n;
}
__global__ void scatterTargetsKernel(const float* packed, float* dst, int size, int strideFloats, int batch) {
  const size_t idx = size_t(blockIdx.x) * blockDim.x + threadIdx.x;
  if (idx >= size_t(batch) * size) return;
  const size_t b = idx / size, k = idx % size;
  dst[b * strideFloats + k] = packed[idx];
}
cudaError_t launchScatterTargets(const float* packed, float* dst, int size, int strideFloats, int batch, cudaStream_t stream) {
  const size_t total = size_t(batch) * size;
  if (total == 0) return cudaSuccess;
  scatterTargetsKernel<<<unsigned((total + 255) / 256), 256, 0, stream>>>(packed, dst, size, strideFloats, batch);
  return cudaGetLastError();
}
cudaError_t launchNormalizeQuats(float* base, int count, int strideFloats, int quatsPerRecord, int batch, cudaStream_t stream) {
  const int total = batch * quatsPerRecord;
  if (total == 0) return cudaSuccess;
  normalizeQuatsKernel<<<(total + 127) / 128, 128, 0, stream>>>(base, count, strideFloats, quatsPerRecord, batch);
  return cudaGetLastError();
}

}
```

momentum_b200/csrc/ik_kernels.cuh:

```cuda
#pragma once

#include <cuda_runtime.h>

#include "ik_chol_sched.cuh"
#include "ik_types.h"

namespace mb2 {

struct SweepArgs {
  FunctionTables T;
  int32_t batch;
  const float* theta;
  int32_t ldTheta;
  const float* targets;
  const float* cweights;
  float* jacobian;
  double* errors;
  const int32_t* active;
  float* stateOut;
  int32_t stageTables;
  int32_t warpsPerInstance;
};

struct JtJArgs {
  int32_t batch;
  const float* jacobian;
  int32_t numCols, ldJ, kRows;
  int32_t ns;
  float* H;
  int32_t ldH;
  size_t hStride;
  const int32_t* active;
  float* g;
  int32_t ldG;
};

struct CholArgs {
  int32_t batch;
  float* H;
  size_t hStride;
  int32_t ns, ldH;
  float regularization;
  const int32_t* cols;
  float* theta;
  int32_t ldTheta;
  float* delta;
  int32_t applyUpdate;
  const double* errors;
  double* lastErrors;
  int32_t* active;
  int32_t* iterations;
  int32_t* status;
  double* history;
  int32_t iteration, minIterations, maxIterations;
  float threshold;
  int32_t* activeCount;
  int32_t bookkeeping;
  float* gradDotDelta;
  const float* g;
  int32_t ldG;
  const float* tilesIn;
  size_t tilesStride;
  int32_t profile;
};

struct GramArgs {
  int32_t batch;
  const float* strips;
  size_t stripStride;
  int32_t residOff;
  const int32_t* active;
  int32_t numStrips, numTiles, numTileCols, nPad;
  int32_t numOrder;
  const int32_t* blob;
  int32_t blobInts;
  int32_t offTileOrder, offTilePairStart, offPairA, offPairB, offColStripStart, offColStrip, offStripRow, offTileInfo;
  float regularization;
  float* out;
  size_t outStride;
};
cudaError_t launchGramTiles(const GramArgs& a, cudaStream_t stream);
size_t gramTilesSmemBytes(size_t stripStride, int blobInts);

struct GramCholArgs {
  GramArgs g;
  CholArgs c;
  unsigned long long* phaseCycles;
};
size_t gramCholeskySmemBytes(size_t stripStride, int gramBlobInts, int n, int nPad, int numTiles, int schedBlobInts);
cudaError_t launchGramCholesky(const GramCholArgs& a, const CholSchedDev& sched, bool profile, cudaStream_t stream);

struct QrArgs {
  CholArgs c;
  const float* jacobian;
  int32_t numCols, ldJ;
  const int32_t* chunkStart;
  int32_t numChunks;
};
struct TrQrArgs {
  QrArgs q;
  FunctionTables T;
  const float* targets;
  const float* cweights;
  float* radius;
  float* rSaved;
  float maxRadius;
  int32_t maxChunkRows;
};
size_t trQrSmemFloats(int n, int numParams, int numJoints, int maxChunkRows);
cudaError_t launchTrustRegionQr(const TrQrArgs& a, cudaStream_t stream);
size_t qrSmemFloats(int n, int maxChunkRows);
int qrMaxChunkRows(int n, size_t smemBytes);
cudaError_t launchQrSolve(const QrArgs& a, int maxChunkRows, cudaStream_t stream);
cudaError_t launchSweep(const SweepArgs& a, bool jacobian, cudaStream_t stream);
size_t sweepSmemPerInstance(const FunctionTables& T, int warpsPerInstance);
cudaError_t launchJtJSimt(const JtJArgs& a, cudaStream_t stream);
cudaError_t launchCholesky(const CholArgs& a, cudaStream_t stream);
cudaError_t launchCholeskyScheduled(const CholArgs& a, const CholSchedDev& sched, cudaStream_t stream);
inline int cholGradientLd(int ns) { return (ns + 3) & ~3; }
size_t choleskyScheduledSmemBytes(int n, int nPad, int numTiles, int blobInts);
cudaError_t initKernelAttributes();

cudaError_t launchTrialUpdate(int batch, const float* thetaOrig, int ldTheta, const float* delta, int ns, const int32_t* cols, const float* scale ,
                              float* thetaTrial, const int32_t* active, cudaStream_t stream);
struct LineSearchArgs {
  int32_t batch, ns, numParams, ldTheta;
  const double* errors;
  const double* trialErrors;
  const float* gradDotDelta;
  float* scale;
  int32_t* searching;
  int32_t step;
  int32_t subsetVariant;
  const int32_t* active;
};
cudaError_t launchLineSearchStep(const LineSearchArgs& a, cudaStream_t stream);
cudaError_t launchCommitTrial(int batch, int numParams, int ldTheta, const float* thetaTrial, float* theta, const int32_t* active, cudaStream_t stream);
struct BookkeepingArgs {
  int32_t batch;
  const double* errors; double* lastErrors; int32_t* active; int32_t* iterations; int32_t* status; double* history;
  const float* theta; int32_t ldTheta, numParams;
  int32_t iteration, minIterations, maxIterations; float threshold; int32_t* activeCount;
};
cudaError_t launchBookkeeping(const BookkeepingArgs& a, cudaStream_t stream);
cudaError_t launchScatterTargets(const float* packed, float* dst, int size, int strideFloats, int batch, cudaStream_t stream);
cudaError_t launchNormalizeQuats(float* base, int count, int strideFloats, int quatsPerRecord, int batch, cudaStream_t stream);

}
```

Baseline: 8.113 million.

## Pack Gram+Cholesky schedule into 16-bit kernel-param tables and park Gram tiles

Builds a compact 16-bit table holding the Gram tile order, quads, column strips and the Cholesky level, panel, task and vector schedules. When it fits, the table is passed as a __grid_constant__ kernel parameter (up to 8192 entries); otherwise it is read from global memory. It also adds a park buffer with atomic slot allocation so Gram tiles can be staged through global memory instead of occupying shared memory. The aim is fewer scattered int32 blob reads from shared or global memory, at the cost of a large parameter block, atomics, and more code-path complexity.

```diff
diff --git a/momentum_b200/csrc/ik_capi.cu b/momentum_b200/csrc/ik_capi.cu
--- a/momentum_b200/csrc/ik_capi.cu
+++ b/momentum_b200/csrc/ik_capi.cu
@@ -107,6 +107,10 @@
   GramPlan gram;
   DeviceBuffer<int32_t> gBlob;
   int32_t gBlobInts{0}, gOffsets[8]{};
+  GramCholTables gc;
+  bool gcValid{false};
+  std::unique_ptr<GramCholParamTables> gcParams;
+  DeviceBuffer<uint16_t> gcTab;
   DeviceBuffer<int32_t> fBlob;
   FusedBlobLayout fLayout{};
   FusedConfig fConfig{};
@@ -148,6 +152,8 @@
   DeviceBuffer<double> dLastErrors, dTrialErrors, dHistory;
   DeviceBuffer<int32_t> dActive, dIterations, dStatus, dSearching, dActiveCount, dWorkCounter, dQrChunks;
   DeviceBuffer<unsigned long long> dPhaseCycles;
+  DeviceBuffer<float> dPark;
+  DeviceBuffer<uint32_t> dParkSlots;
   bool lastFused{false}, lastGramChol{false};
   int lastFusedGroups{0};
   cudaEvent_t fusedStart{nullptr}, fusedStop{nullptr};
@@ -329,6 +335,14 @@
       makeGramBlob(ds->gram, ds->host, gblob, ds->gOffsets);
       ds->gBlobInts = int32_t(gblob.size());
       MB2_CUDA(ds->gBlob.upload(gblob, s));
+      ds->gcValid = makeGramCholTables(ds->gram, ds->host, ds->gc).empty();
+      if (ds->gcValid && ds->gc.tab.size() <= size_t(kGramCholParamEntries)) {
+        ds->gcParams = std::make_unique<GramCholParamTables>();
+        ds->gcParams->L = ds->gc.L;
+        std::copy(ds->gc.tab.begin(), ds->gc.tab.end(), ds->gcParams->tab);
+      } else if (ds->gcValid) {
+        MB2_CUDA(ds->gcTab.upload(ds->gc.tab, s));
+      }
       const int rc = buildFusedBlob(f, *ds, gblob, sblob, s);
       if (rc != MB2_OK) return rc;
     }
@@ -966,7 +980,8 @@
   if (useGram && useSchedule) {
     const DeviceSchedule& ds = *f->sched;
     const int rounds = std::max(int(ds.gram.tileOrder.size()) / kGramWarps, 1);
-    const bool fits = gramCholeskySmemBytes(size_t(ds.gram.stride), ds.gBlobInts, ns, ds.host.nPad, ds.host.numTiles, ds.dev.blobInts) <= size_t(200 * 1024) && rounds <= kGramCholMaxRounds;
+    const bool fits = gramCholeskySmemBytes(size_t(ds.gram.stride), ds.gBlobInts, ns, ds.host.nPad, ds.host.numTiles, ds.dev.blobInts) <= size_t(200 * 1024) && rounds <= kGramCholMaxRounds &&
+                      ds.gcValid;
     if (o.fused_mode == MB2_FUSED_GRAM_CHOLESKY && !fits) return fail(MB2_ERR_UNSUPPORTED, "Gram + Cholesky fusion: strips / tiles of this plan do not fit in shared memory, or too many tiles per warp");
     useGramChol = fits && (o.fused_mode == MB2_FUSED_AUTO || o.fused_mode == MB2_FUSED_GRAM_CHOLESKY);
   } else if (o.fused_mode == MB2_FUSED_GRAM_CHOLESKY) {
@@ -1138,7 +1153,24 @@
       gc.c = c;
       gc.c.tilesIn = nullptr;
       gc.phaseCycles = s->inKernelProfile ? s->dPhaseCycles.p : nullptr;
-      MB2_CUDA(launchGramCholesky(gc, f->sched->dev, s->inKernelProfile, st));
+      const DeviceSchedule& ds = *f->sched;
+      gc.parkTiles = ds.gc.parkTiles;
+      if (gc.parkTiles > 0) {
+        const int slots = gramCholeskyParkSlots(gc, ds.dev, ds.gcParams != nullptr);
+        if (slots < 1) return fail(MB2_ERR_CUDA, "Gram + Cholesky fusion: no resident CTA");
+        if (s->dParkSlots.n < size_t(slots / 32)) {
+          MB2_CUDA(s->dParkSlots.resize(size_t(slots / 32)));
+          MB2_CUDA(cudaMemsetAsync(s->dParkSlots.p, 0, s->dParkSlots.n * sizeof(uint32_t), st));
+        }
+        MB2_CUDA(s->dPark.resize(size_t(slots) * size_t(gc.parkTiles) * 256));
+        gc.park = s->dPark.p;
+        gc.parkSlots = s->dParkSlots.p;
+        gc.parkSlotWords = int32_t(slots / 32);
+      }
+      GramCholGlobalTables gt{};
+      gt.L = ds.gc.L;
+      gt.tab = ds.gcTab.p;
+      MB2_CUDA(launchGramCholesky(gc, ds.dev, ds.gcParams.get(), gt, s->inKernelProfile, st));
     } else if (useSchedule) MB2_CUDA(launchCholeskyScheduled(c, f->sched->dev, st));
     else MB2_CUDA(launchCholesky(c, st));
     recordPhaseStop(s, st);
diff --git a/momentum_b200/csrc/ik_chol_sched.cpp b/momentum_b200/csrc/ik_chol_sched.cpp
--- a/momentum_b200/csrc/ik_chol_sched.cpp
+++ b/momentum_b200/csrc/ik_chol_sched.cpp
@@ -388,6 +388,53 @@
   if (blob.empty()) blob.push_back(0);
 }
 
+std::string makeGramCholTables(const GramPlan& g, const CholSchedule& s, GramCholTables& out) {
+  out = GramCholTables();
+  std::vector<uint16_t>& t = out.tab;
+  bool fits = true;
+  auto put = [&](int64_t v) { fits = fits && v >= 0 && v <= 0xFFFF; t.push_back(uint16_t(v)); };
+  auto section = [&]() { while (t.size() % 4) t.push_back(0); return int32_t(t.size()); };
+  auto validOf = [&](int K) { int v = 0; while (v < kCholTile && s.perm[16 * K + v] >= 0) ++v; return v; };
+  out.L.gram = section();
+  for (int32_t tile : g.tileOrder) {
+    if (tile < 0) { put(0xFFFF); put(0); put(0); put(0); continue; }
+    fits = fits && tile < 0xFFFF;
+    put(tile);
+    put(validOf(s.tileRow[tile]) | (validOf(s.tileCol[tile]) << 8) | ((s.tileRow[tile] == s.tileCol[tile] ? 1 : 0) << 15));
+    put(g.tileQuadStart[tile]); put(g.tileQuadStart[tile + 1]);
+  }
+  out.L.quad = section();
+  for (int32_t v : g.quad) put(v);
+  out.L.col = section();
+  for (int32_t v : g.colStripStart) put(v);
+  out.L.colEnt = section();
+  for (int32_t sidx : g.colStrip) { put(int64_t(sidx) * 64); put(g.stripCoord[2 * sidx]); }
+  out.L.level = section();
+  for (int L = 0; L <= s.numLevels; ++L) { put(s.levelColStart[L]); put(s.levelPanelStart[L]); put(s.levelOrderStart8[L]); put(s.levelVTaskStart[L]); }
+  out.L.diag = section();
+  for (int32_t K : s.levelCols) { put(K); put(s.diagTile[K]); put(s.colPanelStart[K]); put(s.colPanelStart[K + 1]); }
+  out.L.panel = section();
+  for (size_t pi = 0; pi < s.panelTile.size(); ++pi) { put(s.panelTile[pi]); put(s.panelDiag[pi]); }
+  out.L.order = section();
+  for (int32_t ti : s.taskOrder8) {
+    if (ti < 0) { put(0xFFFF); put(0); put(0); put(0); continue; }
+    fits = fits && s.taskDst[ti] < 0xFFFF;
+    put(s.taskDst[ti]); put(s.taskPairStart[ti]); put(s.taskPairStart[ti + 1]); put(0);
+  }
+  out.L.pair = section();
+  for (size_t p = 0; p < s.pairA.size(); ++p) { put(s.pairA[p]); put(s.pairB[p]); }
+  out.L.vtask = section();
+  for (size_t vi = 0; vi < s.vtaskRow.size(); ++vi) { put(s.vtaskRow[vi]); put(s.vtaskSrcStart[vi]); put(s.vtaskSrcStart[vi + 1]); put(0); }
+  out.L.vsrc = section();
+  for (size_t p = 0; p < s.vsrcTile.size(); ++p) { put(s.vsrcTile[p]); put(s.vsrcCol[p]); }
+  out.L.colPanel = section();
+  for (size_t p = 0; p < s.colPanelTile.size(); ++p) { put(s.colPanelTile[p]); put(s.colPanelRow[p]); }
+  section();
+  const int64_t onStrips = (int64_t(g.stride) + 64 + 255) / 256;
+  out.parkTiles = int32_t(std::min<int64_t>(s.numTiles, onStrips));
+  return fits ? "" : "Gram + Cholesky tables: an entry does not fit in 16 bits";
+}
+
 void layoutDeviceColumns(CholSchedule& s, std::vector<int32_t>& deviceColumnOrder) {
   deviceColumnOrder.clear();
   s.nParams = s.n;
diff --git a/momentum_b200/csrc/ik_chol_sched.cuh b/momentum_b200/csrc/ik_chol_sched.cuh
--- a/momentum_b200/csrc/ik_chol_sched.cuh
+++ b/momentum_b200/csrc/ik_chol_sched.cuh
@@ -163,15 +163,40 @@
     }
 #endif
 }
-MB2_HD void gramTileAccumulate(const float* strips, const int32_t* quads, int q0, int q1, int lane, float d[2][4]) {
+MB2_HD int4 tableRecord4(const int32_t* p) {
+#if defined(__CUDA_ARCH__)
+  return *reinterpret_cast<const int4*>(p);
+#else
+  int4 r; r.x = p[0]; r.y = p[1]; r.z = p[2]; r.w = p[3];
+  return r;
+#endif
+}
+MB2_HD int4 tableRecord4(const uint16_t* p) {
+  int4 r;
+#if defined(__CUDA_ARCH__)
+  const uint2 v = *reinterpret_cast<const uint2*>(p);
+  r.x = int(v.x & 0xFFFFu); r.y = int(v.x >> 16); r.z = int(v.y & 0xFFFFu); r.w = int(v.y >> 16);
+#else
+  r.x = p[0]; r.y = p[1]; r.z = p[2]; r.w = p[3];
+#endif
+  return r;
+}
+MB2_HD int2 tableRecord2(const uint16_t* p) {
+  int2 r;
+#if defined(__CUDA_ARCH__)
+  const uint32_t v = *reinterpret_cast<const uint32_t*>(p);
+  r.x = int(v & 0xFFFFu); r.y = int(v >> 16);
+#else
+  r.x = p[0]; r.y = p[1];
+#endif
+  return r;
+}
+template <class Q>
+MB2_HD void gramTileAccumulate(const float* strips, const Q* quads, int q0, int q1, int lane, float d[2][4]) {
   float small[2][4] = {{0.f, 0.f, 0.f, 0.f}, {0.f, 0.f, 0.f, 0.f}};
   for (int q = q0; q < q1; ++q) {
-#if defined(__CUDA_ARCH__)
-    const int4 o = *reinterpret_cast<const int4*>(quads + 4 * q);
+    const int4 o = tableRecord4(quads + 4 * q);
     gramTilePairs(strips, o.x, o.y, o.z, o.w, lane, d, small);
-#else
-    gramTilePairs(strips, quads[4 * q], quads[4 * q + 1], quads[4 * q + 2], quads[4 * q + 3], lane, d, small);
-#endif
   }
 #pragma unroll
   for (int h = 0; h < 2; ++h)
@@ -191,14 +216,25 @@
     }
   tileStoreFrag(tile, lane, v);
 }
+MB2_HD void gramVectorTerm(const float* strip, const float* r4, int hl, float& g0, float& g1) {
+  const float4 sv = *reinterpret_cast<const float4*>(strip + 4 * hl);
+  const float4 rv = *reinterpret_cast<const float4*>(r4);
+  g0 += sv.x * rv.x + sv.y * rv.y;
+  g1 += sv.z * rv.z + sv.w * rv.w;
+}
 MB2_HD float gramVectorEntry(const float* strips, const float* resid, const int32_t* colStrip, const int32_t* stripRow, int s0, int s1, int hl) {
   float g0 = 0.f, g1 = 0.f;
   for (int k = s0; k < s1; ++k) {
     const int sidx = colStrip[k];
-    const float4 sv = *reinterpret_cast<const float4*>(strips + size_t(sidx) * 64 + 4 * hl);
-    const float4 rv = *reinterpret_cast<const float4*>(resid + stripRow[sidx]);
-    g0 += sv.x * rv.x + sv.y * rv.y;
-    g1 += sv.z * rv.z + sv.w * rv.w;
+    gramVectorTerm(strips + size_t(sidx) * 64, resid + stripRow[sidx], hl, g0, g1);
+  }
+  return g0 + g1;
+}
+MB2_HD float gramVectorEntry(const float* strips, const float* resid, const uint16_t* colEnt, int s0, int s1, int hl) {
+  float g0 = 0.f, g1 = 0.f;
+  for (int k = s0; k < s1; ++k) {
+    const int2 e = tableRecord2(colEnt + 2 * k);
+    gramVectorTerm(strips + e.x, resid + e.y, hl, g0, g1);
   }
   return g0 + g1;
 }
@@ -323,15 +359,16 @@
 }
 MB2_HD void cholPanelStore(float* tile, int lane, const float out[2][4]) { tileStoreFrag(tile, lane, out); }
 
-MB2_HD void cholUpdateTask(float* tiles, const CholSchedDev& S, int task, int lane) {
+template <class I>
+MB2_HD void cholUpdateTile(float* tiles, const I* pairA, const I* pairB, int stride, int p0, int p1, int dst, int lane) {
   float d[2][4], small[2][4];
 #pragma unroll
   for (int h = 0; h < 2; ++h)
 #pragma unroll
     for (int e = 0; e < 4; ++e) { d[h][e] = 0.f; small[h][e] = 0.f; }
-  for (int p = S.taskPairStart[task]; p < S.taskPairStart[task + 1]; ++p)
-    tileProduct(tiles + size_t(S.pairA[p]) * 256, tiles + size_t(S.pairB[p]) * 256, lane, d, small);
-  float* D = tiles + size_t(S.taskDst[task]) * 256;
+  for (int p = p0; p < p1; ++p)
+    tileProduct(tiles + size_t(pairA[p * stride]) * 256, tiles + size_t(pairB[p * stride]) * 256, lane, d, small);
+  float* D = tiles + size_t(dst) * 256;
   float v[2][4];
   tileLoadFrag(D, lane, v);
 #pragma unroll
@@ -340,26 +377,34 @@
     for (int e = 0; e < 4; ++e) v[h][e] -= d[h][e] + small[h][e];
   tileStoreFrag(D, lane, v);
 }
-
+MB2_HD void cholUpdateTask(float* tiles, const CholSchedDev& S, int task, int lane) {
+  cholUpdateTile(tiles, S.pairA, S.pairB, 1, S.taskPairStart[task], S.taskPairStart[task + 1], S.taskDst[task], lane);
+}
+
+template <class I>
+MB2_HD void cholVectorRows(const float* tiles, float* y, const I* srcTile, const I* srcCol, int stride, int p0, int p1, int row, int hl) {
+  float s0 = 0.f, s1 = 0.f, s2 = 0.f, s3 = 0.f;
+  for (int p = p0; p < p1; ++p) {
+    float t[16];
+    tileLoadRow(tiles + size_t(srcTile[p * stride]) * 256, hl, t);
+    const float* yk = y + srcCol[p * stride] * 16;
+#pragma unroll
+    for (int c = 0; c < 16; c += 4) { s0 += t[c] * yk[c]; s1 += t[c + 1] * yk[c + 1]; s2 += t[c + 2] * yk[c + 2]; s3 += t[c + 3] * yk[c + 3]; }
+  }
+  y[row * 16 + hl] -= (s0 + s1) + (s2 + s3);
+}
 MB2_HD void cholVectorTask(const float* tiles, float* y, const CholSchedDev& S, int vtask, int hl) {
-  float s0 = 0.f, s1 = 0.f, s2 = 0.f, s3 = 0.f;
-  for (int p = S.vtaskSrcStart[vtask]; p < S.vtaskSrcStart[vtask + 1]; ++p) {
-    float t[16];
-    tileLoadRow(tiles + size_t(S.vsrcTile[p]) * 256, hl, t);
-    const float* yk = y + S.vsrcCol[p] * 16;
-#pragma unroll
-    for (int c = 0; c < 16; c += 4) { s0 += t[c] * yk[c]; s1 += t[c + 1] * yk[c + 1]; s2 += t[c + 2] * yk[c + 2]; s3 += t[c + 3] * yk[c + 3]; }
-  }
-  y[S.vtaskRow[vtask] * 16 + hl] -= (s0 + s1) + (s2 + s3);
-}
-
-MB2_HD void cholBackwardColumn(const float* tiles, float* y, const CholSchedDev& S, int K, int lane) {
+  cholVectorRows(tiles, y, S.vsrcTile, S.vsrcCol, 1, S.vtaskSrcStart[vtask], S.vtaskSrcStart[vtask + 1], S.vtaskRow[vtask], hl);
+}
+
+template <class I>
+MB2_HD void cholBackwardPanels(const float* tiles, float* y, const I* panelTile, const I* panelRow, int stride, int p0, int p1, int K, int diag, int lane) {
 #if defined(__CUDA_ARCH__)
   const int g = lane >> 2, t = lane & 3, so = tileSlotOffset(lane);
   float c0 = 0.f, c1 = 0.f, c2 = 0.f, c3 = 0.f;
-  for (int p = S.colPanelStart[K]; p < S.colPanelStart[K + 1]; ++p) {
-    const float* T = tiles + size_t(S.colPanelTile[p]) * 256;
-    const float* yi = y + S.colPanelRow[p] * 16;
+  for (int p = p0; p < p1; ++p) {
+    const float* T = tiles + size_t(panelTile[p * stride]) * 256;
+    const float* yi = y + panelRow[p * stride] * 16;
     const float4 v0 = *reinterpret_cast<const float4*>(T + so), v1 = *reinterpret_cast<const float4*>(T + 128 + so);
     const float ya = yi[g], yb = yi[g + 8];
     c0 = fmaf(v0.x, ya, fmaf(v0.z, yb, c0)); c1 = fmaf(v0.y, ya, fmaf(v0.w, yb, c1));
@@ -373,7 +418,7 @@
   float* yk = y + K * 16;
   if (g == 0) { yk[2 * t] -= c0; yk[2 * t + 1] -= c1; yk[8 + 2 * t] -= c2; yk[9 + 2 * t] -= c3; }
   __syncwarp();
-  const float* W = tiles + size_t(S.diagTile[K]) * 256;
+  const float* W = tiles + size_t(diag) * 256;
   const float4 w0 = *reinterpret_cast<const float4*>(W + so), w1 = *reinterpret_cast<const float4*>(W + 128 + so);
   const float sa = yk[g], sb = yk[g + 8];
   float x0 = fmaf(w0.x, sa, w0.z * sb), x1 = fmaf(w0.y, sa, w0.w * sb), x2 = fmaf(w1.x, sa, w1.z * sb), x3 = fmaf(w1.y, sa, w1.w * sb);
@@ -388,14 +433,14 @@
   if (lane != 0) return;
   float s[16];
   for (int c = 0; c < 16; ++c) s[c] = 0.f;
-  for (int p = S.colPanelStart[K]; p < S.colPanelStart[K + 1]; ++p) {
-    const float* T = tiles + size_t(S.colPanelTile[p]) * 256;
-    const float* yi = y + S.colPanelRow[p] * 16;
+  for (int p = p0; p < p1; ++p) {
+    const float* T = tiles + size_t(panelTile[p * stride]) * 256;
+    const float* yi = y + panelRow[p * stride] * 16;
     for (int c = 0; c < 16; ++c) for (int r = 0; r < 16; ++r) s[c] += T[tileIdx(r, c)] * yi[r];
   }
   float* yk = y + K * 16;
   for (int c = 0; c < 16; ++c) s[c] = yk[c] - s[c];
-  const float* W = tiles + size_t(S.diagTile[K]) * 256;
+  const float* W = tiles + size_t(diag) * 256;
   for (int c = 0; c < 16; ++c) {
     float x = 0.f;
     for (int r = 0; r < 16; ++r) x += W[tileIdx(r, c)] * s[r];
@@ -403,5 +448,8 @@
   }
 #endif
 }
-
-}
+MB2_HD void cholBackwardColumn(const float* tiles, float* y, const CholSchedDev& S, int K, int lane) {
+  cholBackwardPanels(tiles, y, S.colPanelTile, S.colPanelRow, 1, S.colPanelStart[K], S.colPanelStart[K + 1], K, S.diagTile[K], lane);
+}
+
+}
diff --git a/momentum_b200/csrc/ik_chol_sched.h b/momentum_b200/csrc/ik_chol_sched.h
--- a/momentum_b200/csrc/ik_chol_sched.h
+++ b/momentum_b200/csrc/ik_chol_sched.h
@@ -57,4 +57,14 @@
 struct CholSchedDev;
 void makeScheduleBlob(const CholSchedule& s, std::vector<int32_t>& blob, CholSchedDev& dev);
 
+struct GramCholLayout {
+  int32_t gram, quad, col, colEnt, level, diag, panel, order, pair, vtask, vsrc, colPanel;
+};
+struct GramCholTables {
+  GramCholLayout L{};
+  std::vector<uint16_t> tab;
+  int32_t parkTiles{0};
+};
+std::string makeGramCholTables(const GramPlan& g, const CholSchedule& s, GramCholTables& out);
+
 }
diff --git a/momentum_b200/csrc/ik_kernels.cu b/momentum_b200/csrc/ik_kernels.cu
--- a/momentum_b200/csrc/ik_kernels.cu
+++ b/momentum_b200/csrc/ik_kernels.cu
@@ -628,8 +628,19 @@
   return 128 + sizeof(float) * (((uni + 3) & ~size_t(3)) + size_t(nPad) + size_t((n + 3) & ~3)) + 32;
 }
 
-template <bool kProfile>
-__global__ void __launch_bounds__(kGramThreads, 4) gramCholeskyKernel(const GramCholArgs a, const CholSchedDev S) {
+__device__ int acquireParkSlot(uint32_t* words, int numWords, int start) {
+  for (int w = start % numWords;; w = (w + 1 == numWords) ? 0 : w + 1) {
+    uint32_t freeBits = ~__ldcg(words + w);
+    while (freeBits != 0u) {
+      const int bit = __ffs(freeBits) - 1;
+      if ((atomicOr(words + w, 1u << bit) & (1u << bit)) == 0u) return 32 * w + bit;
+      freeBits &= freeBits - 1u;
+    }
+  }
+}
+
+template <bool kProfile, class Tables>
+__global__ void __launch_bounds__(kGramThreads, 4) gramCholeskyKernel(const GramCholArgs a, const CholSchedDev S, const __grid_constant__ Tables P) {
   extern __shared__ __align__(16) float gcSmem[];
   const GramArgs& g = a.g;
   const CholArgs& c = a.c;
@@ -637,7 +648,7 @@
   if (c.active[b] == 0) return;
   const int n = c.ns, tid = threadIdx.x;
   const int warp = tid >> 5, lane = tid & 31, hw = tid >> 4, hl = tid & 15;
-  const unsigned hmask = 0xFFFFu << (16 * ((tid >> 4) & 1));
+  constexpr int kWarps = kGramThreads / 32;
   float* U = gcSmem + (((128u - (smemAddr(gcSmem) & 127u)) & 127u) >> 2);
   const size_t tileFloats = size_t(S.numTiles) * 256, sweepFloats = g.stripStride + 64;
   const size_t uni = ((tileFloats > sweepFloats ? tileFloats : sweepFloats) + 3) & ~size_t(3);
@@ -648,6 +659,8 @@
   float* gsub = y + S.nPad;
   int* flags = reinterpret_cast<int*>(gsub + ((n + 3) & ~3));
   unsigned long long* bar = reinterpret_cast<unsigned long long*>(flags + 4);
+  const uint16_t* tab = P.tab;
+  const GramCholLayout& L = P.L;
   long long pc[8] = {0, 0, 0, 0, 0, 0, 0, 0}, pt = 0;
   if constexpr (kProfile) pt = clock64();
 #define MB2_GC(k) if constexpr (kProfile) { const long long now = clock64(); pc[k] += now - pt; pt = now; }
@@ -660,76 +673,83 @@
     mbarExpectTx(barAddr, stripBytes);
     const char* src = reinterpret_cast<const char*>(g.strips + size_t(b) * g.stripStride);
     for (uint32_t off = 0; off < stripBytes; off += 16384u) bulkLoad(smemAddr(strips) + off, src + off, stripBytes - off < 16384u ? stripBytes - off : 16384u, barAddr);
+    flags[1] = a.parkTiles > 0 ? acquireParkSlot(a.parkSlots, a.parkSlotWords, b) : 0;
   }
   if (tid >= 64 && tid < 128) strips[g.stripStride + (tid - 64)] = 0.f;
   __syncthreads();
   mbarWaitRelaxed(barAddr, 0);
   MB2_GC(0)
-  const int32_t* __restrict__ gtab = g.blob;
-  const int32_t* tileOrder = gtab + g.offTileOrder, *tileQuadStart = gtab + g.offTilePairStart, *quads = gtab + g.offPairA;
-  const int32_t* colStripStart = gtab + g.offColStripStart, *colStrip = gtab + g.offColStrip, *stripRow = gtab + g.offStripRow, *tileInfo = gtab + g.offTileInfo;
-  float parked[kGramCholMaxRounds][8];
-  {
-    int slot = 0;
-    for (int ti = warp; ti < g.numOrder; ti += kGramThreads / 32, ++slot) {
-      const int t = tileOrder[ti];
-      if (t < 0) continue;
-      float acc[2][4];
-#pragma unroll
-      for (int i = 0; i < 2; ++i)
-#pragma unroll
-        for (int j = 0; j < 4; ++j) acc[i][j] = 0.f;
-      gramTileAccumulate(strips, quads, tileQuadStart[t], tileQuadStart[t + 1], lane, acc);
-      if (size_t(t) * 256 >= sweepFloats) gramTileStore(tiles + size_t(t) * 256, acc, tileInfo[t], g.regularization, lane);
-      else {
-#pragma unroll
-        for (int i = 0; i < 8; ++i) parked[slot][i] = acc[i >> 2][i & 3];
-      }
-    }
-    for (int K = hw; K < S.numTileCols; K += kGramThreads / 16)
-      y[16 * K + hl] = gramVectorEntry(strips, resid, colStrip, stripRow, colStripStart[K], colStripStart[K + 1], hl);
-  }
+  float* park = a.park + size_t(flags[1]) * size_t(a.parkTiles) * 256 + 4 * lane;
+  const int rounds = g.numOrder / kWarps;
+  auto tileInfoOf = [](int packed) { return (packed & 0x7FFF) | ((packed >> 15) << 16); };
+  for (int r = 0; r < rounds; ++r) {
+    const int4 rec = tableRecord4(tab + L.gram + 4 * (r * kWarps + warp));
+    if (rec.x == 0xFFFF) continue;
+    float acc[2][4];
+#pragma unroll
+    for (int i = 0; i < 2; ++i)
+#pragma unroll
+      for (int j = 0; j < 4; ++j) acc[i][j] = 0.f;
+    gramTileAccumulate(strips, tab + L.quad, rec.z, rec.w, lane, acc);
+    if (rec.x >= a.parkTiles) gramTileStore(tiles + size_t(rec.x) * 256, acc, tileInfoOf(rec.y), g.regularization, lane);
+    else {
+      __stcg(reinterpret_cast<float4*>(park + size_t(rec.x) * 256), make_float4(acc[0][0], acc[0][1], acc[0][2], acc[0][3]));
+      __stcg(reinterpret_cast<float4*>(park + size_t(rec.x) * 256 + 128), make_float4(acc[1][0], acc[1][1], acc[1][2], acc[1][3]));
+    }
+  }
+  for (int K = hw; K < S.numTileCols; K += kGramThreads / 16)
+    y[16 * K + hl] = gramVectorEntry(strips, resid, tab + L.colEnt, int(tab[L.col + K]), int(tab[L.col + K + 1]), hl);
   __syncthreads();
   MB2_GC(1)
-  {
-    int slot = 0;
-    for (int ti = warp; ti < g.numOrder; ti += kGramThreads / 32, ++slot) {
-      const int t = tileOrder[ti];
-      if (t < 0 || size_t(t) * 256 >= sweepFloats) continue;
-      float acc[2][4];
-#pragma unroll
-      for (int i = 0; i < 8; ++i) acc[i >> 2][i & 3] = parked[slot][i];
-      gramTileStore(tiles + size_t(t) * 256, acc, tileInfo[t], g.regularization, lane);
-    }
-    for (int s2 = tid; s2 < S.nPad; s2 += kGramThreads) {
-      const int p = S.perm[s2];
-      if (p >= 0) gsub[p] = y[s2];
-    }
+  for (int r = 0; r < rounds; ++r) {
+    const int4 rec = tableRecord4(tab + L.gram + 4 * (r * kWarps + warp));
+    if (rec.x == 0xFFFF || rec.x >= a.parkTiles) continue;
+    const float4 v0 = __ldcg(reinterpret_cast<const float4*>(park + size_t(rec.x) * 256));
+    const float4 v1 = __ldcg(reinterpret_cast<const float4*>(park + size_t(rec.x) * 256 + 128));
+    const float acc[2][4] = {{v0.x, v0.y, v0.z, v0.w}, {v1.x, v1.y, v1.z, v1.w}};
+    gramTileStore(tiles + size_t(rec.x) * 256, acc, tileInfoOf(rec.y), g.regularization, lane);
+  }
+  for (int s2 = tid; s2 < S.nPad; s2 += kGramThreads) {
+    const int p = S.perm[s2];
+    if (p >= 0) gsub[p] = y[s2];
   }
   __syncthreads();
+  if (tid == 0 && a.parkTiles > 0) atomicAnd(a.parkSlots + (flags[1] >> 5), ~(1u << (flags[1] & 31)));
   MB2_GC(2)
-  for (int L = 0; L < S.numLevels; ++L) {
-    for (int ci = S.levelColStart[L] + warp; ci < S.levelColStart[L + 1]; ci += kGramThreads / 32) {
-      const int K = S.levelCols[ci];
-      cholDiagTile(tiles + size_t(S.diagTile[K]) * 256, y + 16 * K, lane, c.regularization, flags);
+  for (int Lv = 0; Lv < S.numLevels; ++Lv) {
+    const int4 l0 = tableRecord4(tab + L.level + 4 * Lv), l1 = tableRecord4(tab + L.level + 4 * (Lv + 1));
+    for (int ci = l0.x + warp; ci < l1.x; ci += kWarps) {
+      const int4 d = tableRecord4(tab + L.diag + 4 * ci);
+      cholDiagTile(tiles + size_t(d.y) * 256, y + 16 * d.x, lane, c.regularization, flags);
     }
     __syncthreads();
     MB2_GC(3)
-    for (int pi = S.levelPanelStart[L] + warp; pi < S.levelPanelStart[L + 1]; pi += kGramThreads / 32) {
-      float* ptile = tiles + size_t(S.panelTile[pi]) * 256;
+    for (int pi = l0.y + warp; pi < l1.y; pi += kWarps) {
+      const int2 pe = tableRecord2(tab + L.panel + 2 * pi);
+      float* ptile = tiles + size_t(pe.x) * 256;
       float x[2][4];
-      cholPanelProduct(ptile, tiles + size_t(S.panelDiag[pi]) * 256, lane, x);
+      cholPanelProduct(ptile, tiles + size_t(pe.y) * 256, lane, x);
       cholPanelStore(ptile, lane, x);
     }
     __syncthreads();
     MB2_GC(4)
-    for (int oi = S.levelOrderStart8[L] + warp; oi < S.levelOrderStart8[L + 1]; oi += kGramThreads / 32) { const int ti = S.taskOrder8[oi]; if (ti >= 0) cholUpdateTask(tiles, S, ti, lane); }
-    for (int vi = S.levelVTaskStart[L] + hw; vi < S.levelVTaskStart[L + 1]; vi += kGramThreads / 16) cholVectorTask(tiles, y, S, vi, hl);
+    for (int oi = l0.z + warp; oi < l1.z; oi += kWarps) {
+      const int4 o = tableRecord4(tab + L.order + 4 * oi);
+      if (o.x != 0xFFFF) cholUpdateTile(tiles, tab + L.pair, tab + L.pair + 1, 2, o.y, o.z, o.x, lane);
+    }
+    for (int vi = l0.w + hw; vi < l1.w; vi += kGramThreads / 16) {
+      const int4 v = tableRecord4(tab + L.vtask + 4 * vi);
+      cholVectorRows(tiles, y, tab + L.vsrc, tab + L.vsrc + 1, 2, v.y, v.z, v.x, hl);
+    }
     __syncthreads();
     MB2_GC(5)
   }
-  for (int L = S.numLevels - 1; L >= 0; --L) {
-    for (int ci = S.levelColStart[L] + warp; ci < S.levelColStart[L + 1]; ci += kGramThreads / 32) cholBackwardColumn(tiles, y, S, S.levelCols[ci], lane);
+  for (int Lv = S.numLevels - 1; Lv >= 0; --Lv) {
+    const int c0 = tab[L.level + 4 * Lv], c1 = tab[L.level + 4 * (Lv + 1)];
+    for (int ci = c0 + warp; ci < c1; ci += kWarps) {
+      const int4 d = tableRecord4(tab + L.diag + 4 * ci);
+      cholBackwardPanels(tiles, y, tab + L.colPanel, tab + L.colPanel + 1, 2, d.z, d.w, d.x, d.y, lane);
+    }
     __syncthreads();
   }
   MB2_GC(6)
@@ -742,18 +762,40 @@
 #undef MB2_GC
 }
 
-cudaError_t launchGramCholesky(const GramCholArgs& a, const CholSchedDev& sched, bool profile, cudaStream_t stream) {
+template <bool kProfile, class Tables>
+static cudaError_t prepareGramCholesky(size_t smem) {
+  cudaError_t e = cudaFuncSetAttribute(gramCholeskyKernel<kProfile, Tables>, cudaFuncAttributeMaxDynamicSharedMemorySize, int(smem));
+  if (e != cudaSuccess) return e;
+  return cudaFuncSetAttribute(gramCholeskyKernel<kProfile, Tables>, cudaFuncAttributePreferredSharedMemoryCarveout, int(cudaSharedmemCarveoutMaxShared));
+}
+
+int gramCholeskyParkSlots(const GramCholArgs& a, const CholSchedDev& sched, bool paramTables) {
+  const size_t smem = gramCholeskySmemBytes(a.g.stripStride, a.g.blobInts, a.c.ns, sched.nPad, sched.numTiles, sched.blobInts);
+  cudaError_t e = paramTables ? prepareGramCholesky<false, GramCholParamTables>(smem) : prepareGramCholesky<false, GramCholGlobalTables>(smem);
+  int perSm = 0;
+  if (e == cudaSuccess)
+    e = paramTables ? cudaOccupancyMaxActiveBlocksPerMultiprocessor(&perSm, gramCholeskyKernel<false, GramCholParamTables>, kGramThreads, smem)
+                    : cudaOccupancyMaxActiveBlocksPerMultiprocessor(&perSm, gramCholeskyKernel<false, GramCholGlobalTables>, kGramThreads, smem);
+  if (e != cudaSuccess || perSm < 1) return -1;
+  return (g_numSms * perSm + 31) / 32 * 32;
+}
+
+cudaError_t launchGramCholesky(const GramCholArgs& a, const CholSchedDev& sched, const GramCholParamTables* inParams, const GramCholGlobalTables& inGlobal, bool profile,
+                               cudaStream_t stream) {
   const size_t smem = gramCholeskySmemBytes(a.g.stripStride, a.g.blobInts, a.c.ns, sched.nPad, sched.numTiles, sched.blobInts);
   if (smem > size_t(g_maxSmemOptin) || (a.g.stripStride & 3) != 0) return cudaErrorInvalidConfiguration;
-  if (a.g.numOrder > kGramCholMaxRounds * (kGramThreads / 32)) return cudaErrorInvalidConfiguration;
-  cudaError_t e = profile ? cudaFuncSetAttribute(gramCholeskyKernel<true>, cudaFuncAttributeMaxDynamicSharedMemorySize, int(smem))
-                          : cudaFuncSetAttribute(gramCholeskyKernel<false>, cudaFuncAttributeMaxDynamicSharedMemorySize, int(smem));
+  if (a.parkTiles > 0 && (a.park == nullptr || a.parkSlots == nullptr || a.parkSlotWords < 1)) return cudaErrorInvalidValue;
+  cudaError_t e;
+  if (inParams != nullptr) e = profile ? prepareGramCholesky<true, GramCholParamTables>(smem) : prepareGramCholesky<false, GramCholParamTables>(smem);
+  else e = profile ? prepareGramCholesky<true, GramCholGlobalTables>(smem) : prepareGramCholesky<false, GramCholGlobalTables>(smem);
   if (e != cudaSuccess) return e;
-  e = profile ? cudaFuncSetAttribute(gramCholeskyKernel<true>, cudaFuncAttributePreferredSharedMemoryCarveout, int(cudaSharedmemCarveoutMaxShared))
-              : cudaFuncSetAttribute(gramCholeskyKernel<false>, cudaFuncAttributePreferredSharedMemoryCarveout, int(cudaSharedmemCarveoutMaxShared));
-  if (e != cudaSuccess) return e;
-  if (profile) gramCholeskyKernel<true><<<a.c.batch, kGramThreads, smem, stream>>>(a, sched);
-  else gramCholeskyKernel<false><<<a.c.batch, kGramThreads, smem, stream>>>(a, sched);
+  if (inParams != nullptr) {
+    if (profile) gramCholeskyKernel<true, GramCholParamTables><<<a.c.batch, kGramThreads, smem, stream>>>(a, sched, *inParams);
+    else gramCholeskyKernel<false, GramCholParamTables><<<a.c.batch, kGramThreads, smem, stream>>>(a, sched, *inParams);
+  } else {
+    if (profile) gramCholeskyKernel<true, GramCholGlobalTables><<<a.c.batch, kGramThreads, smem, stream>>>(a, sched, inGlobal);
+    else gramCholeskyKernel<false, GramCholGlobalTables><<<a.c.batch, kGramThreads, smem, stream>>>(a, sched, inGlobal);
+  }
   return cudaGetLastError();
 }
 
diff --git a/momentum_b200/csrc/ik_kernels.cuh b/momentum_b200/csrc/ik_kernels.cuh
--- a/momentum_b200/csrc/ik_kernels.cuh
+++ b/momentum_b200/csrc/ik_kernels.cuh
@@ -3,6 +3,7 @@
 #include <cuda_runtime.h>
 
 #include "ik_chol_sched.cuh"
+#include "ik_chol_sched.h"
 #include "ik_types.h"
 
 namespace mb2 {
@@ -86,9 +87,23 @@
   GramArgs g;
   CholArgs c;
   unsigned long long* phaseCycles;
+  float* park;
+  uint32_t* parkSlots;
+  int32_t parkSlotWords, parkTiles;
+};
+constexpr int kGramCholParamEntries = 8192;
+struct alignas(16) GramCholParamTables {
+  GramCholLayout L;
+  uint16_t tab[kGramCholParamEntries];
+};
+struct GramCholGlobalTables {
+  GramCholLayout L;
+  const uint16_t* tab;
 };
 size_t gramCholeskySmemBytes(size_t stripStride, int gramBlobInts, int n, int nPad, int numTiles, int schedBlobInts);
-cudaError_t launchGramCholesky(const GramCholArgs& a, const CholSchedDev& sched, bool profile, cudaStream_t stream);
+int gramCholeskyParkSlots(const GramCholArgs& a, const CholSchedDev& sched, bool paramTables);
+cudaError_t launchGramCholesky(const GramCholArgs& a, const CholSchedDev& sched, const GramCholParamTables* inParams, const GramCholGlobalTables& inGlobal, bool profile,
+                               cudaStream_t stream);
 
 struct QrArgs {
   CholArgs c;
```

Result: faster. 9.170 million (median of 6 runs) (+13.0%).
